# Alxaline/BraTS21

Measured on AMD Instinct MI355X. Metric: train patches/sec (4x128^3, width-48), higher is better.
Workload: dtype bf16; 1 GPU; equiunet width=48, batch=2/GPU of 4x128^3 synthetic patches, fwd + deep-supervision Dice + bwd + ranger (BASELINE.json configs[1]); global_batch=2, parallelism=dp1

## Files before the change

brats21_amd/csrc/conv_wgrad.hip:

```cpp
#include <stdlib.h>
#include "twin_begin.hpp"
#include "common.hpp"

typedef __attribute__((ext_vector_type(4))) short s16x4;

struct WgradParams {
  const void* x1; const void* x2; int c1, c2, p1, p2;
  const void* dy; int dyp;
  float* ws;
  int N, D, H, W, cin, cout;
  int tz, ty, tx, ntiles, nsplit;
  int nlane;
  int ntaps, dil;
  int seglen, nsegz;
};

constexpr int WG_TZ = 4, WG_TY = 4, WG_TX = 16, WG_VOX = 256;

template <typename T, int DIL, int COF, int CIF, int KS = 3>
struct WgGeom {
  static constexpr bool BF = std::is_same<T, bf16_t>::value;
  static constexpr int ESZ = sizeof(T);
  static constexpr int EPL = 16 / ESZ;
  static constexpr int R = KS == 3 ? DIL : 0;
  static constexpr int HY = WG_TY + 2 * R, HX = WG_TX + 2 * R;
  static constexpr int HVOX = WG_TZ * HY * HX;
  static constexpr int CI_T = 16 * CIF, CO_T = 16 * COF;
  static constexpr int XROWB = CI_T * ESZ, YROWB = CO_T * ESZ;
  static constexpr int SX = BF ? (CIF == 1 ? 32 : 96) : XROWB + 16;
  static constexpr int SY = BF ? (COF == 1 ? 32 : 96) : YROWB + 16;
  static constexpr int XPPV = XROWB / 16, YPPV = YROWB / 16;
  static constexpr int XPPR = HX * XPPV, XIPR = (XPPR + 63) / 64, XROWS = WG_TZ * HY, XRPW = (XROWS + 3) / 4;
  static constexpr int YPPR = WG_TX * YPPV, YIPR = (YPPR + 63) / 64, YROWS = WG_TZ * WG_TY, YRPW = YROWS / 4;
  static constexpr int LDS_X = HVOX * SX, LDS_Y = WG_VOX * SY;
  static constexpr int LDS = LDS_X + LDS_Y;
  static constexpr int PAIRS = (KS == 3 ? 9 : 1) * CIF;
  static constexpr int PPW = (PAIRS + 3) / 4;
  static constexpr int NB = BF ? 32 : 64;
};

DEVI bf16x8 tr_pair(const char* p0, const char* p1) {
  const s16x4 lo = __builtin_amdgcn_ds_read_tr16_b64_v4i16((__attribute__((address_space(3))) s16x4*)p0);
  const s16x4 hi = __builtin_amdgcn_ds_read_tr16_b64_v4i16((__attribute__((address_space(3))) s16x4*)p1);
  typedef __attribute__((ext_vector_type(8))) short s16x8;
  const s16x8 v = {lo[0], lo[1], lo[2], lo[3], hi[0], hi[1], hi[2], hi[3]};
  return __builtin_bit_cast(bf16x8, v);
}

template <typename T, int DIL, int COF, int CIF, int KS = 3>
__global__ __launch_bounds__(256, 2) void conv_wgrad_kernel(const WgradParams p) {
  using G = WgGeom<T, DIL, COF, CIF, KS>;
  extern __shared__ __attribute__((aligned(16))) char lds[];
  char* ldx = lds;
  char* ldy = lds + G::LDS_X;
  const int tid = threadIdx.x, lane = tid & 63;
  const int wave = __builtin_amdgcn_readfirstlane(tid >> 6);
  const int q = lane >> 4, v = lane & 15;
  const int NP = KS == 3 ? 3 : p.ntaps;
  const int lane8 = blockIdx.x % p.nlane, rr = blockIdx.x / p.nlane;
  const int tzg = rr % NP, gsub = rr / NP, g8 = gridDim.x / (NP * p.nlane);
  const int shz = (KS == 3 || p.ntaps == 1) ? 0 : (tzg / 9 - 1) * p.dil;
  const int shy = (KS == 3 || p.ntaps == 1) ? 0 : ((tzg / 3) % 3 - 1) * p.dil;
  const int shx = (KS == 3 || p.ntaps == 1) ? 0 : (tzg % 3 - 1) * p.dil;
  const int split = lane8 + p.nlane * gsub;
  const int tpx = (p.ntiles + p.nlane - 1) / p.nlane;
  const int tile_end = min(p.ntiles, (lane8 + 1) * tpx);
  const int cot = blockIdx.y, cit = blockIdx.z;
  const int co0 = cot * G::CO_T, ci0 = cit * G::CI_T;
  const T* xsrc;
  int xpitch;
  if (ci0 < p.c1) { xsrc = (const T*)p.x1 + ci0; xpitch = p.p1; }
  else { xsrc = (const T*)p.x2 + (ci0 - p.c1); xpitch = p.p2; }
  const int ci_lim = (ci0 < p.c1 ? p.c1 : p.c1 + p.c2) - ci0;
  const int co_lim = p.cout - co0;

  int xhx[G::XIPR], xlo[G::XIPR];
  int xvo[G::XRPW][G::XIPR];
#pragma unroll
  for (int j = 0; j < G::XIPR; ++j) {
    const int pc = lane + 64 * j;
    const int hx = pc / G::XPPV, part = pc % G::XPPV;
    const bool ok = pc < G::XPPR && part * G::EPL < ci_lim;
    xhx[j] = ok ? hx : -100000;
    xlo[j] = pc < G::XPPR ? wave * (G::HX * G::SX) + hx * G::SX + part * 16 : -1;
#pragma unroll
    for (int k = 0; k < G::XRPW; ++k) {
      const int row = wave + 4 * k;
      xvo[k][j] = (((row / G::HY) * p.H + row % G::HY) * p.W + hx) * xpitch * G::ESZ + part * 16;
    }
  }
  int yvx[G::YIPR], ylo[G::YIPR];
  int yvo[G::YRPW][G::YIPR];
#pragma unroll
  for (int j = 0; j < G::YIPR; ++j) {
    const int pc = lane + 64 * j;
    const int vx = pc / G::YPPV, part = pc % G::YPPV;
    const bool ok = pc < G::YPPR && part * G::EPL < co_lim;
    yvx[j] = ok ? vx : 100000;
    ylo[j] = pc < G::YPPR ? wave * (WG_TX * G::SY) + vx * G::SY + part * 16 : -1;
#pragma unroll
    for (int k = 0; k < G::YRPW; ++k) {
      const int row = wave + 4 * k;
      yvo[k][j] = (((row / WG_TY) * p.H + row % WG_TY) * p.W + vx) * p.dyp * G::ESZ + part * 16;
    }
  }
  const unsigned xsample_bytes = (unsigned)p.D * p.H * p.W * xpitch * G::ESZ;
  const unsigned ysample_bytes = (unsigned)p.D * p.H * p.W * p.dyp * G::ESZ;

  int poff[G::PPW];
#pragma unroll
  for (int jj = 0; jj < G::PPW; ++jj) {
    const int pid = wave + 4 * jj;
    const int t9 = pid / CIF, nn = pid % CIF;
    poff[jj] = pid < G::PAIRS ? (((t9 / 3) * G::R) * G::HX + (t9 % 3) * G::R) * G::SX + nn * G::NB : 0;
  }
  f32x4 acc[G::PPW][COF];
#pragma unroll
  for (int jj = 0; jj < G::PPW; ++jj)
#pragma unroll
    for (int m = 0; m < COF; ++m) acc[jj][m] = f32x4{0.f, 0.f, 0.f, 0.f};

  u32x4 rx[G::XRPW][G::XIPR], ry[G::YRPW][G::YIPR];
  auto issue_loads = [&](int tile) {
    int bt = tile;
    const int x0 = (bt % p.tx) * WG_TX; bt /= p.tx;
    const int y0 = (bt % p.ty) * WG_TY; bt /= p.ty;
    const int z0 = (bt % p.tz) * WG_TZ;
    const int n = bt / p.tz;
    const int gz0 = KS == 3 ? z0 + (tzg - 1) * DIL : z0 + shz;
    const int gy0 = KS == 3 ? y0 - DIL : y0 + shy, gx0 = KS == 3 ? x0 - DIL : x0 + shx;
    const size_t sample_vox = (size_t)n * p.D * p.H * p.W;
    const __amdgpu_buffer_rsrc_t xrs = __builtin_amdgcn_make_buffer_rsrc((void*)(xsrc + sample_vox * xpitch), (short)0,
                                                                          (int)xsample_bytes, 0x00020000);
    const __amdgpu_buffer_rsrc_t yrs = __builtin_amdgcn_make_buffer_rsrc((void*)((const T*)p.dy + sample_vox * p.dyp + co0),
                                                                          (short)0, (int)ysample_bytes, 0x00020000);
    const int xorg = ((gz0 * p.H + gy0) * p.W + gx0) * xpitch * G::ESZ;
    const int yorg = ((z0 * p.H + y0) * p.W + x0) * p.dyp * G::ESZ;
    bool xok[G::XIPR], yok[G::YIPR];
#pragma unroll
    for (int j = 0; j < G::XIPR; ++j) xok[j] = (unsigned)(gx0 + xhx[j]) < (unsigned)p.W;
#pragma unroll
    for (int j = 0; j < G::YIPR; ++j) yok[j] = x0 + yvx[j] < p.W;
#pragma unroll
    for (int k = 0; k < G::XRPW; ++k) {
      const int row = wave + 4 * k;
      const int gz = gz0 + row / G::HY, gy = gy0 + row % G::HY;
      const bool row_ok = row < G::XROWS && (unsigned)gz < (unsigned)p.D && (unsigned)gy < (unsigned)p.H;
#pragma unroll
      for (int j = 0; j < G::XIPR; ++j) {
        const int vo = (row_ok && xok[j]) ? xorg + xvo[k][j] : -1;
        rx[k][j] = __builtin_bit_cast(u32x4, __builtin_amdgcn_raw_buffer_load_b128(xrs, vo, 0, 0));
      }
    }
#pragma unroll
    for (int k = 0; k < G::YRPW; ++k) {
      const int row = wave + 4 * k;
      const bool row_ok = z0 + row / WG_TY < p.D && y0 + row % WG_TY < p.H;
#pragma unroll
      for (int j = 0; j < G::YIPR; ++j) {
        const int vo = (row_ok && yok[j]) ? yorg + yvo[k][j] : -1;
        ry[k][j] = __builtin_bit_cast(u32x4, __builtin_amdgcn_raw_buffer_load_b128(yrs, vo, 0, 0));
      }
    }
  };
  constexpr bool PREFETCH = !(G::BF && KS == 3 && DIL == 2 && COF * CIF == 9);
  const int tile_first = lane8 * tpx + gsub;
  if (PREFETCH && tile_first < tile_end) issue_loads(tile_first);
// ... 120 lines not shown
  if (ci0 < p.c1) { xsrc = (const T*)p.x1 + ci0; xpitch = p.p1; }
  else { xsrc = (const T*)p.x2 + (ci0 - p.c1); xpitch = p.p2; }

  int xcode[G::XI], ycode[G::YI];
#pragma unroll
  for (int i = 0; i < G::XI; ++i) {
    const int P = tid + 512 * i;
    const int vox = P / G::XPPV, part = P % G::XPPV;
    const int hx = vox % G::HX, hy = (vox / G::HX) % G::HY, hz = vox / (G::HX * G::HY);
    xcode[i] = (P < G::XPIECES && part * 8 < ci_lim) ? (hz | hy << 3 | hx << 6 | part << 11 | 1 << 14) : 0;
  }
#pragma unroll
  for (int i = 0; i < G::YI; ++i) {
    const int P = tid + 512 * i;
    const int vox = P / G::YPPV, part = P % G::YPPV;
    ycode[i] = (vox >> 6) | ((vox >> 4) & 3) << 3 | (vox & 15) << 6 | part << 11 | 1 << 14;
  }
  const unsigned xsample_bytes = (unsigned)p.D * p.H * p.W * xpitch * 2;
  const unsigned ysample_bytes = (unsigned)p.D * p.H * p.W * p.dyp * 2;

  int poff[G::PPW];
#pragma unroll
  for (int jj = 0; jj < G::PPW; ++jj) {
    const int pid = wave + 8 * jj;
    const int t = pid / CIF, nn = pid % CIF;
    poff[jj] = pid < G::PAIRS ? (((t / 9) * G::HY + (t / 3) % 3) * G::HX + t % 3) * G::SX + nn * 32 : 0;
  }
  f32x4 acc[G::PPW][COF];
#pragma unroll
  for (int jj = 0; jj < G::PPW; ++jj)
#pragma unroll
    for (int m = 0; m < COF; ++m) acc[jj][m] = f32x4{0.f, 0.f, 0.f, 0.f};

  u32x4 rx[G::XI], ry[G::YI];
  auto issue_loads = [&](int tile) {
    int bt = tile;
    const int x0 = (bt % p.tx) * WG_TX; bt /= p.tx;
    const int y0 = (bt % p.ty) * WG_TY; bt /= p.ty;
    const int z0 = (bt % p.tz) * WG_TZ;
    const int n = bt / p.tz;
    const size_t sample_vox = (size_t)n * p.D * p.H * p.W;
    const __amdgpu_buffer_rsrc_t xrs = __builtin_amdgcn_make_buffer_rsrc((void*)(xsrc + sample_vox * xpitch), (short)0,
                                                                          (int)xsample_bytes, 0x00020000);
    const __amdgpu_buffer_rsrc_t yrs = __builtin_amdgcn_make_buffer_rsrc((void*)((const T*)p.dy + sample_vox * p.dyp + co0),
                                                                          (short)0, (int)ysample_bytes, 0x00020000);
    unsigned zm = 0, ym = 0, xm = 0, zy = 0, yy = 0, xy = 0;
#pragma unroll
    for (int h = 0; h < G::HZ; ++h) zm |= ((unsigned)(z0 - 1 + h) < (unsigned)p.D ? 1u : 0u) << h;
#pragma unroll
    for (int h = 0; h < G::HY; ++h) ym |= ((unsigned)(y0 - 1 + h) < (unsigned)p.H ? 1u : 0u) << h;
#pragma unroll
    for (int h = 0; h < G::HX; ++h) xm |= ((unsigned)(x0 - 1 + h) < (unsigned)p.W ? 1u : 0u) << h;
    zy = zm >> 1; yy = ym >> 1; xy = xm >> 1;
    const int xorg = ((z0 - 1) * p.H + (y0 - 1)) * p.W + (x0 - 1);
    const int yorg = (z0 * p.H + y0) * p.W + x0;
    const int xpb = xpitch * 2, ypb = p.dyp * 2;
#pragma unroll
    for (int i = 0; i < G::XI; ++i) {
      int c = xcode[i];
      asm volatile("" : "+v"(c));
      const unsigned ok = (unsigned)(c >> 14) & (zm >> (c & 7)) & (ym >> ((c >> 3) & 7)) & (xm >> ((c >> 6) & 31)) & 1u;
      const int pv = ((c & 7) * p.H + ((c >> 3) & 7)) * p.W + ((c >> 6) & 31);
      const int vo = ok ? (xorg + pv) * xpb + ((c >> 11) & 7) * 16 : -1;
      rx[i] = __builtin_bit_cast(u32x4, __builtin_amdgcn_raw_buffer_load_b128(xrs, vo, 0, 0));
    }
#pragma unroll
    for (int i = 0; i < G::YI; ++i) {
      int c = ycode[i];
      asm volatile("" : "+v"(c));
      const unsigned ok = (zy >> (c & 7)) & (yy >> ((c >> 3) & 7)) & (xy >> ((c >> 6) & 31)) & 1u;
      const int pv = ((c & 7) * p.H + ((c >> 3) & 7)) * p.W + ((c >> 6) & 31);
      const int vo = ok ? (yorg + pv) * ypb + ((c >> 11) & 7) * 16 : -1;
      ry[i] = __builtin_bit_cast(u32x4, __builtin_amdgcn_raw_buffer_load_b128(yrs, vo, 0, 0));
    }
  };

  const int tile_first = lane8 * tpx + gsub;
  if (tile_first < tile_end) issue_loads(tile_first);
  for (int tile = tile_first; tile < tile_end; tile += g8) {
    __syncthreads();
#pragma unroll
    for (int i = 0; i < G::XI; ++i)
      if (tid + 512 * i < G::XPIECES) *(u32x4*)(ldx + (tid + 512 * i) * 16) = rx[i];
#pragma unroll
    for (int i = 0; i < G::YI; ++i) {
      const int P = tid + 512 * i;
      *(u32x4*)(ldy + (P / G::YPPV) * G::SY + (P % G::YPPV) * 16) = ry[i];
    }
    __syncthreads();
    if (tile + g8 < tile_end) issue_loads(tile + g8);
    __builtin_amdgcn_sched_barrier(0);
    const int qq = v >> 2, pp = v & 3;
    const int ybase = (4 * q + qq) * G::SY + pp * 8;
    const int xbase = (4 * q + qq) * G::SX + pp * 8;
    constexpr int PD = 2;
    bf16x8 a[2][COF], b[PD + 1];
    auto read_a = [&](auto s_) {
      constexpr int s = s_;
      const int yoff = ybase + (32 * s) * G::SY;
#pragma unroll
      for (int m = 0; m < COF; ++m) a[s & 1][m] = tr_pair(ldy + yoff + m * 32, ldy + yoff + 16 * G::SY + m * 32);
    };
    auto read_b = [&](auto u_) {
      constexpr int u = u_;
      constexpr int s = u / G::PPW, jj = u % G::PPW;
      const int xoff = xbase + (((s >> 1) * G::HY + 2 * (s & 1)) * G::HX) * G::SX + poff[jj];
      b[u % (PD + 1)] = tr_pair(ldx + xoff, ldx + xoff + G::HX * G::SX);
    };
    constexpr int NU = 8 * G::PPW;
    read_a(std::integral_constant<int, 0>{});
    static_for<0, PD>([&](auto u_) { read_b(u_); });
    static_for<0, NU>([&](auto u_) {
      constexpr int u = u_;
      constexpr int s = u / G::PPW, jj = u % G::PPW;
      if constexpr (u + PD < NU) read_b(std::integral_constant<int, u + PD>{});
      if constexpr (jj == 0 && s + 1 < 8) read_a(std::integral_constant<int, s + 1>{});
      __builtin_amdgcn_sched_barrier(0);
#pragma unroll
      for (int m = 0; m < COF; ++m)
        acc[jj][m] = MFMA16_16x16x32(a[s & 1][m], b[u % (PD + 1)], acc[jj][m]);
      __builtin_amdgcn_sched_barrier(0);
    });
  }

#pragma unroll
  for (int jj = 0; jj < G::PPW; ++jj) {
    const int pid = wave + 8 * jj;
    if (pid < G::PAIRS) {
      const int t = pid / CIF, nn = pid % CIF;
      float* base = p.ws + ((size_t)split * 27 + t) * p.cout * p.cin;
      const int ci = ci0 + nn * 16 + v;
      if (nn * 16 + v < ci_lim) {
#pragma unroll
        for (int m = 0; m < COF; ++m)
#pragma unroll
          for (int r = 0; r < 4; ++r) base[(size_t)(co0 + m * 16 + 4 * q + r) * p.cin + ci] = acc[jj][m][r];
      }
    }
  }
}

template <int COF, int CIF> struct Wg3b {
  static constexpr int HZ = WG_TZ + 2, HY = WG_TY + 2, HX = WG_TX + 2, HVOX = HZ * HY * HX;
  static constexpr int CO = 16 * COF, CI = 16 * CIF;
  static constexpr int SX = 2 * CI, SY = 2 * CO, XPPV = CI / 8, YPPV = CO / 8;
  static constexpr int XPIECES = HVOX * XPPV, YPIECES = WG_VOX * YPPV;
  static constexpr int XI = (XPIECES + 511) / 512, YI = YPIECES / 512;
  static constexpr int XB = XI * 512 * 16;
  static constexpr int LDS = 2 * XB + WG_VOX * SY;
  static constexpr int PAIRS = 27 * CIF, PPW = (PAIRS + 7) / 8;
  static_assert(YPIECES % 512 == 0, "");
};

template <int COF, int CIF>
__global__ __launch_bounds__(512, 1) void conv_wgrad_alltaps2_kernel(const WgradParams p) {
  typedef bf16_t T;
  using G = Wg3b<COF, CIF>;
  extern __shared__ __attribute__((aligned(16))) char lds[];
  char* ldy = lds + 2 * G::XB;
  const int tid = threadIdx.x, lane = tid & 63;
  const int wave = __builtin_amdgcn_readfirstlane(tid >> 6);
  const int q = lane >> 4, v = lane & 15;
  const int lane8 = blockIdx.x % p.nlane, gsub = blockIdx.x / p.nlane, g8 = gridDim.x / p.nlane;
  const int split = blockIdx.x;
  const int tpx = (p.ntiles + p.nlane - 1) / p.nlane;
  const int tile_end = min(p.ntiles, (lane8 + 1) * tpx);
  const int co0 = blockIdx.y * G::CO, ci0 = blockIdx.z * G::CI;
  const T* xsrc;
  int xpitch;
  if (ci0 < p.c1) { xsrc = (const T*)p.x1 + ci0; xpitch = p.p1; }
  else { xsrc = (const T*)p.x2 + (ci0 - p.c1); xpitch = p.p2; }
  const int xpb = xpitch * 2, ypb = p.dyp * 2;

  int xoffs[G::XI], xcode[G::XI];
#pragma unroll
  for (int i = 0; i < G::XI; ++i) {
    const int P = tid + 512 * i;
    const int vox = P / G::XPPV, part = P % G::XPPV;
    const int hx = vox % G::HX, hy = (vox / G::HX) % G::HY, hz = vox / (G::HX * G::HY);
    const bool ok = P < G::XPIECES && (CIF > 1 || part * 8 < p.c1);
    xoffs[i] = ok ? ((hz * p.H + hy) * p.W + hx) * xpb + part * 16 : (int)0x80000000;
    xcode[i] = ok ? (hz | hy << 3 | hx << 6 | 1 << 14) : 0;
  }
  const unsigned xsample_bytes = (unsigned)p.D * p.H * p.W * xpitch * 2;
  const unsigned ysample_bytes = (unsigned)p.D * p.H * p.W * p.dyp * 2;

  int poff[G::PPW];
#pragma unroll
  for (int jj = 0; jj < G::PPW; ++jj) {
    const int pid = wave + 8 * jj;
    const int t = pid / CIF, nn = pid % CIF;
    poff[jj] = pid < G::PAIRS ? (((t / 9) * G::HY + (t / 3) % 3) * G::HX + t % 3) * G::SX + nn * 32 : 0;
  }
  f32x4 acc[G::PPW][COF];
#pragma unroll
  for (int jj = 0; jj < G::PPW; ++jj)
#pragma unroll
    for (int m = 0; m < COF; ++m) acc[jj][m] = f32x4{0.f, 0.f, 0.f, 0.f};

  u32x4 ry[G::YI];
  struct TileLoads {
    rsrc4_t xrs;
    __amdgpu_buffer_rsrc_t yrs;
    int xorg, yorg;
    unsigned zm, ym, xm, inter;
    char* xdst;
  };
  auto setup_loads = [&](int tile, int buf) {
    TileLoads L;
    int bt = tile;
    const int x0 = (bt % p.tx) * WG_TX; bt /= p.tx;
    const int y0 = (bt % p.ty) * WG_TY; bt /= p.ty;
    const int z0 = (bt % p.tz) * WG_TZ;
    const int n = bt / p.tz;
    const size_t sample_vox = (size_t)n * p.D * p.H * p.W;
    L.xrs = make_rsrc4(xsrc + sample_vox * xpitch, xsample_bytes);
    L.yrs = __builtin_amdgcn_make_buffer_rsrc((void*)((const T*)p.dy + sample_vox * p.dyp + co0), (short)0, (int)ysample_bytes, 0x00020000);
    L.xorg = (((z0 - 1) * p.H + (y0 - 1)) * p.W + (x0 - 1)) * xpb;
    L.yorg = ((z0 * p.H + y0) * p.W + x0) * ypb;
    L.xdst = lds + buf * G::XB + wave * 1024;
    auto inside = [](int o, int size, int hn) {
      const int lo = o >= 1 ? 0 : 1 - o, hi = size - o + 1 < hn ? size - o + 1 : hn;
      return hi > lo ? ((1u << hi) - 1u) & ~((1u << lo) - 1u) : 0u;
    };
    L.zm = inside(z0, p.D, G::HZ); L.ym = inside(y0, p.H, G::HY); L.xm = inside(x0, p.W, G::HX);
    L.inter = (L.zm == (1u << G::HZ) - 1 && L.ym == (1u << G::HY) - 1 && L.xm == (1u << G::HX) - 1) ? 1u : 0u;
    return L;
  };
  auto issue_x = [&](const TileLoads& L, auto i_) {
    constexpr int i = i_;
    const int c = xcode[i];
    const unsigned ok = (unsigned)(c >> 14) & (L.inter | ((L.zm >> (c & 7)) & (L.ym >> ((c >> 3) & 7)) & (L.xm >> ((c >> 6) & 31)))) & 1u;
    lds_dma16_async(L.xrs, L.xdst + i * 8192, (L.xorg + xoffs[i]) | ((int)ok - 1));
  };
  auto issue_y = [&](const TileLoads& L, auto i_) {
    constexpr int i = i_;
    const int P = tid + 512 * i;
    const int vox = P / G::YPPV, part = P % G::YPPV;
    const int z = vox >> 6, y = (vox >> 4) & 3, x = vox & 15;
    const int yo = ((z * p.H + y) * p.W + x) * ypb + part * 16;
    const unsigned ok = (L.inter | ((L.zm >> (z + 1)) & (L.ym >> (y + 1)) & (L.xm >> (x + 1)))) & 1u;
    ry[i] = __builtin_bit_cast(u32x4, __builtin_amdgcn_raw_buffer_load_b128(L.yrs, (L.yorg + yo) | ((int)ok - 1), 0, 0));
  };

  const int tile_first = lane8 * tpx + gsub;
  const int qq = v >> 2, pp = v & 3;
  const int ybase = (4 * q + qq) * G::SY + pp * 8;
  const int xbase = (4 * q + qq) * G::SX + pp * 8;
  int cur = 0;
#ifdef BRATS_WGRAD_STAMPS
  long long tacc[5] = {0, 0, 0, 0, 0}, tlast = __builtin_amdgcn_s_memtime();
#define WG_STAMP(i) do { const long long t_ = __builtin_amdgcn_s_memtime(); tacc[i] += t_ - tlast; tlast = t_; } while (0)
#else
#define WG_STAMP(i) do { } while (0)
#endif
  if (tile_first < tile_end) {
    const TileLoads L = setup_loads(tile_first, 0);
    static_for<0, G::XI>([&](auto i_) { issue_x(L, i_); });
    static_for<0, G::YI>([&](auto i_) { issue_y(L, i_); });
  }
  for (int tile = tile_first; tile < tile_end; tile += g8, cur ^= 1) {
    WG_STAMP(4);
    asm volatile("s_waitcnt vmcnt(0)" ::: "memory");
    WG_STAMP(0);
    __syncthreads();
    WG_STAMP(1);
#pragma unroll
    for (int i = 0; i < G::YI; ++i) *(u32x4*)(ldy + (tid + 512 * i) * 16) = ry[i];
    __syncthreads();
    WG_STAMP(2);
    const bool more = tile + g8 < tile_end;
    TileLoads L = setup_loads(more ? tile + g8 : tile, cur ^ 1);
    if (!more) L.zm = L.inter = 0;
    __builtin_amdgcn_sched_barrier(0);
    WG_STAMP(3);
    const char* ldx = lds + cur * G::XB;
    constexpr int PD = 3;
    bf16x8 a[2][COF], b[PD + 1];
    auto read_a = [&](auto s_) {
      constexpr int s = s_;
      const int yoff = ybase + (32 * s) * G::SY;
#pragma unroll
      for (int m = 0; m < COF; ++m) a[s & 1][m] = tr_pair(ldy + yoff + m * 32, ldy + yoff + 16 * G::SY + m * 32);
    };
    auto read_b = [&](auto u_) {
      constexpr int u = u_;
      constexpr int s = u / G::PPW, jj = u % G::PPW;
      const int xoff = xbase + (((s >> 1) * G::HY + 2 * (s & 1)) * G::HX) * G::SX + poff[jj];
      b[u % (PD + 1)] = tr_pair(ldx + xoff, ldx + xoff + G::HX * G::SX);
    };
    constexpr int NU = 8 * G::PPW;
    static_for<0, G::XI>([&](auto i_) { issue_x(L, i_); });
    static_for<0, G::YI>([&](auto i_) { issue_y(L, i_); });
    __builtin_amdgcn_sched_barrier(0);
    read_a(std::integral_constant<int, 0>{});
    static_for<0, PD>([&](auto u_) { read_b(u_); });
    static_for<0, NU>([&](auto u_) {
      constexpr int u = u_;
      constexpr int s = u / G::PPW, jj = u % G::PPW;
      if constexpr (u + PD < NU) read_b(std::integral_constant<int, u + PD>{});
      if constexpr (jj == 0 && s + 1 < 8) read_a(std::integral_constant<int, s + 1>{});
      __builtin_amdgcn_sched_barrier(0);
#pragma unroll
      for (int m = 0; m < COF; ++m)
        acc[jj][m] = MFMA16_16x16x32(a[s & 1][m], b[u % (PD + 1)], acc[jj][m]);
      __builtin_amdgcn_sched_barrier(0);
    });
  }

#ifdef BRATS_WGRAD_STAMPS
  WG_STAMP(4);
  if (lane == 0 && blockIdx.y == 0 && blockIdx.z == 0) {
    long long* st = (long long*)(p.ws + (size_t)gridDim.x * 27 * p.cout * p.cin) + ((size_t)blockIdx.x * 8 + wave) * 5;
    for (int i = 0; i < 5; ++i) st[i] = tacc[i];
  }
#endif
#pragma unroll
  for (int jj = 0; jj < G::PPW; ++jj) {
    const int pid = wave + 8 * jj;
    if (pid < G::PAIRS) {
      const int t = pid / CIF, nn = pid % CIF;
      float* base = p.ws + ((size_t)split * 27 + t) * p.cout * p.cin;
      const int ci = ci0 + nn * 16 + v;
      if (CIF > 1 || ci < p.cin) {
#pragma unroll
        for (int m = 0; m < COF; ++m)
#pragma unroll
          for (int r = 0; r < 4; ++r) base[(size_t)(co0 + m * 16 + 4 * q + r) * p.cin + ci] = acc[jj][m][r];
      }
    }
  }
}

template <int DIL> struct Wg3n {
  static constexpr int HZ = WG_TZ + 2 * DIL, HY = WG_TY + 2 * DIL, HX = WG_TX + 2 * DIL, HVOX = HZ * HY * HX;
  static constexpr int COF = 3, CO = 48, CI = 16;
  static constexpr int SX = 2 * CI, SY = 2 * CO, XPPV = CI / 8, YPPV = CO / 8;
  static constexpr int MMA_WAVES = 8, LOAD_WAVES = 4, THREADS = 64 * (MMA_WAVES + LOAD_WAVES), LT = 64 * LOAD_WAVES;
  static constexpr int XPIECES = HVOX * XPPV, YPIECES = WG_VOX * YPPV;
  static constexpr int XI = (XPIECES + LT - 1) / LT, YI = YPIECES / LT;
  static constexpr int XB = XI * LT * 16, YB = YI * LT * 16;
  static constexpr int BUF = XB + YB;
  static constexpr int PAIRS = 27, PPW = 4;
  static constexpr int OUT_ROW = CI * 27, OUT_B = CO * OUT_ROW * 4;
  static constexpr int LDS = 2 * BUF > OUT_B ? 2 * BUF : OUT_B;
  static_assert(HZ <= 8 && HY <= 8 && HX <= 32, "packed halo coordinates: 3 + 3 + 5 bits");
  static_assert(YPIECES % LT == 0, "");
};

struct WgNoslabWalk {
  int nlane, nsplit, g8, tpx, ntiles;
  int split, tile, end;
  DEVI void enter() {
    for (;; ++split) {
      const int lane8 = split % nlane;
      tile = lane8 * tpx + split / nlane;
      end = min(ntiles, (lane8 + 1) * tpx);
      if (tile < end || split + 1 >= nsplit) return;
    }
  }
  DEVI WgNoslabWalk(const WgradParams& p) : nlane(p.nlane), nsplit(p.nsplit), g8(p.nsplit / p.nlane),
                                            tpx((p.ntiles + p.nlane - 1) / p.nlane), ntiles(p.ntiles), split(0) { enter(); }
  DEVI bool done() const { return tile >= end; }
  DEVI bool next() {
    tile += g8;
    if (tile < end) return false;
    if (split + 1 < nsplit) { ++split; enter(); }
    return true;
  }
};

template <int DIL>
__global__ __launch_bounds__(768, 1) void conv_wgrad_noslab_kernel(const WgradParams p) {
  typedef bf16_t T;
  using G = Wg3n<DIL>;
  extern __shared__ __attribute__((aligned(16))) char lds[];
  const int tid = threadIdx.x, lane = tid & 63;
  const int wave = __builtin_amdgcn_readfirstlane(tid >> 6);
  const int co0 = blockIdx.y * G::CO, ci0 = blockIdx.z * G::CI;
  f32x4 tot[G::PPW][G::COF];
#pragma unroll
  for (int jj = 0; jj < G::PPW; ++jj)
#pragma unroll
    for (int m = 0; m < G::COF; ++m) tot[jj][m] = f32x4{0.f, 0.f, 0.f, 0.f};

  WgNoslabWalk walk(p);
  if (wave >= G::MMA_WAVES) {
    const int lt = tid - 64 * G::MMA_WAVES, lw = wave - G::MMA_WAVES;
    const T* xsrc;
    int xpitch;
    if (ci0 < p.c1) { xsrc = (const T*)p.x1 + ci0; xpitch = p.p1; }
    else { xsrc = (const T*)p.x2 + (ci0 - p.c1); xpitch = p.p2; }
    const int xpb = xpitch * 2, ypb = p.dyp * 2;
    int xoffs[G::XI], xcode[G::XI], yoffs[G::YI], ycode[G::YI];
#pragma unroll
    for (int i = 0; i < G::XI; ++i) {
      const int P = lt + G::LT * i;
      const int vox = P / G::XPPV, part = P % G::XPPV;
      const int hx = vox % G::HX, hy = (vox / G::HX) % G::HY, hz = vox / (G::HX * G::HY);
      const bool ok = P < G::XPIECES;
      xoffs[i] = ok ? ((hz * p.H + hy) * p.W + hx) * xpb + part * 16 : (int)0x80000000;
      xcode[i] = ok ? (hz | hy << 3 | hx << 6 | 1 << 14) : 0;
    }
#pragma unroll
    for (int i = 0; i < G::YI; ++i) {
      const int P = lt + G::LT * i;
      const int vox = P / G::YPPV, part = P % G::YPPV;
      const int z = vox >> 6, y = (vox >> 4) & 3, x = vox & 15;
      yoffs[i] = ((z * p.H + y) * p.W + x) * ypb + part * 16;
      ycode[i] = (z + DIL) | (y + DIL) << 3 | (x + DIL) << 6;
    }
    const unsigned xsample_bytes = (unsigned)p.D * p.H * p.W * xpitch * 2;
    const unsigned ysample_bytes = (unsigned)p.D * p.H * p.W * p.dyp * 2;
    auto issue_tile = [&](int tile, int buf) {
      int bt = tile;
      const int x0 = (bt % p.tx) * WG_TX; bt /= p.tx;
      const int y0 = (bt % p.ty) * WG_TY; bt /= p.ty;
      const int z0 = (bt % p.tz) * WG_TZ;
      const int n = bt / p.tz;
      const size_t sample_vox = (size_t)n * p.D * p.H * p.W;
      const rsrc4_t xrs = make_rsrc4(xsrc + sample_vox * xpitch, xsample_bytes);
      const rsrc4_t yrs = make_rsrc4((const T*)p.dy + sample_vox * p.dyp + co0, ysample_bytes);
      const int xorg = (((z0 - DIL) * p.H + (y0 - DIL)) * p.W + (x0 - DIL)) * xpb;
      const int yorg = ((z0 * p.H + y0) * p.W + x0) * ypb;
      char* const dst = lds + buf * G::BUF + lw * 1024;
      auto inside = [](int o, int size, int hn) {
        const int lo = o >= DIL ? 0 : DIL - o, hi = size - o + DIL < hn ? size - o + DIL : hn;
        return hi > lo ? ((1u << hi) - 1u) & ~((1u << lo) - 1u) : 0u;
      };
      const unsigned zm = inside(z0, p.D, G::HZ), ym = inside(y0, p.H, G::HY), xm = inside(x0, p.W, G::HX);
      static_for<0, G::XI>([&](auto i_) {
        constexpr int i = i_;
        const int c = xcode[i];
        const unsigned ok = (unsigned)(c >> 14) & (zm >> (c & 7)) & (ym >> ((c >> 3) & 7)) & (xm >> ((c >> 6) & 31)) & 1u;
        lds_dma16_async(xrs, dst + i * (G::LT * 16), (xorg + xoffs[i]) | ((int)ok - 1));
      });
      static_for<0, G::YI>([&](auto i_) {
        constexpr int i = i_;
        const int c = ycode[i];
        const unsigned ok = (zm >> (c & 7)) & (ym >> ((c >> 3) & 7)) & (xm >> ((c >> 6) & 31)) & 1u;
        lds_dma16_async(yrs, dst + G::XB + i * (G::LT * 16), (yorg + yoffs[i]) | ((int)ok - 1));
      });
    };
    issue_tile(walk.tile, 0);
    asm volatile("s_waitcnt vmcnt(0)" ::: "memory");
    __syncthreads();
    for (int buf = 1; !walk.done(); buf ^= 1) {
      walk.next();
      if (!walk.done()) issue_tile(walk.tile, buf);
      asm volatile("s_waitcnt vmcnt(0)" ::: "memory");
      __syncthreads();
    }
  } else {
    const int q = lane >> 4, v = lane & 15;
    const bool four = wave + 24 < G::PAIRS;
    int poff[G::PPW];
#pragma unroll
    for (int jj = 0; jj < G::PPW; ++jj) {
      const int t = wave + 8 * jj;
      poff[jj] = t < G::PAIRS ? ((((t / 9) * G::HY + (t / 3) % 3) * G::HX + t % 3) * DIL) * G::SX : 0;
    }
    f32x4 acc[G::PPW][G::COF];
#pragma unroll
    for (int jj = 0; jj < G::PPW; ++jj)
#pragma unroll
      for (int m = 0; m < G::COF; ++m) acc[jj][m] = f32x4{0.f, 0.f, 0.f, 0.f};
    const int qq = v >> 2, pp = v & 3;
    const int ybase = (4 * q + qq) * G::SY + pp * 8;
    const int xbase = (4 * q + qq) * G::SX + pp * 8;
    __syncthreads();
    for (int buf = 0; !walk.done(); buf ^= 1) {
      const char* ldx = lds + buf * G::BUF;
      const char* ldy = ldx + G::XB;
      constexpr int PD = 3;
      bf16x8 a[2][G::COF], b[PD + 1];
      auto read_a = [&](auto s_) {
        constexpr int s = s_;
        const int yoff = ybase + (32 * s) * G::SY;
#pragma unroll
        for (int m = 0; m < G::COF; ++m) a[s & 1][m] = tr_pair(ldy + yoff + m * 32, ldy + yoff + 16 * G::SY + m * 32);
      };
      auto read_b = [&](auto u_) {
        constexpr int u = u_;
        constexpr int s = u / G::PPW, jj = u % G::PPW;
// ... 302 lines not shown
    f32x4 s[4];
#pragma unroll
    for (int t = 0; t < 4; ++t) s[t] = f32x4{0.f, 0.f, 0.f, 0.f};
    for (int k0 = 0; k0 < nsplit; k0 += 8) {
      f32x4 v[4][8];
#pragma unroll
      for (int t = 0; t < 4; ++t) {
        const int tap = g + 8 * t;
        const float* src = ws + ((size_t)(tap < taps ? tap : 0) * cout * cin + p4 * 4);
#pragma unroll
        for (int u = 0; u < 8; ++u)
          v[t][u] = (tap < taps && k0 + u < nsplit) ? *(const f32x4*)(src + (size_t)(k0 + u) * per) : f32x4{0.f, 0.f, 0.f, 0.f};
      }
#pragma unroll
      for (int t = 0; t < 4; ++t)
#pragma unroll
        for (int u = 0; u < 8; ++u)
          if (k0 + u < nsplit) s[t] += v[t][u];
    }
#pragma unroll
    for (int t = 0; t < 4; ++t)
      if (g + 8 * t < taps) *(f32x4*)(red_tile + (g + 8 * t) * 128 + e * 4) = s[t];
  }
  __syncthreads();
  const size_t pair0 = (size_t)blockIdx.x * 128, npairs = (size_t)cout * cin;
  float* dst = dw + pair0 * taps;
  const float isc = amax ? x3_inv_scale(x3_scale_from_amax(*amax)) : 1.f;
  for (int i = threadIdx.x; i < 128 * taps; i += blockDim.x) {
    const int pr = i / taps, tap = i % taps;
    if (pair0 + pr < npairs) dst[i] = red_tile[tap * 128 + pr] * isc;
  }
}

static void wgrad_reduce_launch(const float* ws, float* dw, int nsplit, int cout, int cin, int taps, hipStream_t st,
                                const float* amax = nullptr) {
  const size_t per = (size_t)taps * cout * cin;
  const size_t tblocks = ((size_t)cout * cin / 4 + 31) / 32;
  if (taps > 1 && taps <= 32 && tblocks >= 256)
    hipLaunchKernelGGL(wgrad_reduce_taps_kernel, dim3((unsigned)tblocks), dim3(256), (size_t)taps * 128 * sizeof(float), st, ws, dw,
                       nsplit, cout, cin, taps, amax);
  else
    hipLaunchKernelGGL(wgrad_reduce_kernel, dim3((unsigned)((per / 4 + 31) / 32)), dim3(256), 0, st, ws, dw, nsplit, cout, cin, taps, amax);
}

template <typename T>
__global__ void dbias_kernel(const T* __restrict__ dy, int pitch, float* __restrict__ db, size_t voxels, int C) {
  __shared__ float red[256];
  const int c = blockIdx.x;
  float s = 0.f;
  for (size_t v = threadIdx.x; v < voxels; v += blockDim.x) s += to_f<T>(dy[v * pitch + c]);
  red[threadIdx.x] = s;
  __syncthreads();
  for (int m = 128; m > 0; m >>= 1) {
    if ((int)threadIdx.x < m) red[threadIdx.x] += red[threadIdx.x + m];
    __syncthreads();
  }
  if (threadIdx.x == 0) db[c] = red[0];
}
static void wgrad_dbias_launch(int dtype, const void* dy, int dypitch, float* dbias, size_t vox, int cout, hipStream_t st) {
  with_storage(dtype, [&](auto t) {
    using T = typename decltype(t)::type;
    hipLaunchKernelGGL(dbias_kernel<T>, dim3(cout), dim3(256), 0, st, (const T*)dy, dypitch, dbias, vox, cout);
  });
}

struct WgradArgs {
  const void* x1; int c1, p1;
  const void* x2; int c2, p2;
  const void* dy; int dyp;
  int N, D, H, W, cout;
  int cin() const { return c1 + c2; }
  size_t vox() const { return (size_t)N * D * H * W; }
};
static WgradArgs wgrad_shape(int N, int D, int H, int W, int c1, int c2, int cout) {
  return WgradArgs{nullptr, c1, 0, nullptr, c2 > 0 ? c2 : 0, 0, nullptr, 0, N, D, H, W, cout};
}
static int wgrad_sample_overflow(const WgradArgs& a, int esize) {
  const int mp = a.p1 > a.p2 ? (a.p1 > a.dyp ? a.p1 : a.dyp) : (a.p2 > a.dyp ? a.p2 : a.dyp);
  return (double)a.D * a.H * a.W * mp * esize >= 2147483648.0 ? mp : 0;
}

struct WgradTileGrid { int tz, ty, tx, ntiles; };
static WgradTileGrid wgrad_tile_grid(const WgradArgs& a, int TZ = WG_TZ, int TY = WG_TY, int TX = WG_TX) {
  WgradTileGrid t{ceil_div(a.D, TZ), ceil_div(a.H, TY), ceil_div(a.W, TX), 0};
  t.ntiles = a.N * t.tz * t.ty * t.tx;
  return t;
}
static WgradParams wgrad_params(const WgradArgs& a, float* ws, const WgradTileGrid& t, int nlane, int nsplit, int ntaps, int dil) {
  WgradParams p{};
  p.x1 = a.x1; p.x2 = a.x2; p.c1 = a.c1; p.c2 = a.c2; p.p1 = a.p1; p.p2 = a.p2;
  p.dy = a.dy; p.dyp = a.dyp; p.ws = ws;
  p.N = a.N; p.D = a.D; p.H = a.H; p.W = a.W; p.cin = a.cin(); p.cout = a.cout;
  p.tz = t.tz; p.ty = t.ty; p.tx = t.tx; p.ntiles = t.ntiles;
  p.nlane = nlane; p.nsplit = nsplit; p.ntaps = ntaps; p.dil = dil;
  return p;
}

static int wgrad_nlane(int ntiles) {
  int nl = 8;
  while (nl > 1 && ntiles / nl < 16) nl >>= 1;
  return nl;
}
static int wgrad_split_g8(int ntiles, int nlane, int groups, int cot, int cit) {
  int g8 = ceil_div(512, groups * nlane * cot * cit);
  const int cap = ceil_div(ntiles, nlane);
  if (g8 > cap) g8 = cap;
  return g8 < 1 ? 1 : g8;
}
static bool wgrad_blocks_g8(int ntiles, int blocks, int* nlane, int* g8) {
  *nlane = wgrad_nlane(ntiles);
  *g8 = ceil_div(device_cus(), *nlane * blocks);
  if (*g8 < 1) *g8 = 1;
  return ntiles >= 4 * *nlane * *g8;
}
static void wgrad_tiles(int dtype, int c1, int c2, int cout, int* cof, int* cif) {
  const int co16 = ceil_div(cout, 16);
  *cof = co16 % 3 == 0 ? 3 : (co16 % 2 == 0 ? 2 : 1);
  if (dtype == BRATS_F32) { *cif = 1; return; }
  const int a = ceil_div(c1, 16), b = c2 > 0 ? ceil_div(c2, 16) : 0;
  auto ok = [&](int f) { return a % f == 0 && (b == 0 || b % f == 0); };
  *cif = ok(3) ? 3 : (ok(2) ? 2 : 1);
}

int g_wgrad_alltaps_mode = -1;
extern "C" int BRATS_API(brats_conv3d_set_wgrad_alltaps)(int mode) {
  const int old = g_wgrad_alltaps_mode;
  g_wgrad_alltaps_mode = mode < 0 ? -1 : (mode ? 1 : 0);
  return old;
}
static int wgrad_alltaps_mode() {
  static int env_mode = -1;
  if (env_mode < 0) {
    const char* e = getenv("BRATS_WGRAD_ALLTAPS");
    env_mode = e ? atoi(e) : 1;
  }
  return g_wgrad_alltaps_mode >= 0 ? g_wgrad_alltaps_mode : env_mode;
}

int g_wgrad_noslab_mode = -1;
extern "C" int BRATS_API(brats_conv3d_set_wgrad_noslab)(int mode) {
  const int old = g_wgrad_noslab_mode;
  g_wgrad_noslab_mode = mode < 0 ? -1 : (mode ? 1 : 0);
  return old;
}
static int wgrad_noslab_mode() {
  static int env_mode = -2;
  if (env_mode < -1) {
    const char* e = getenv("BRATS_WGRAD_NOSLAB");
    const int m = e ? atoi(e) : -1;
    env_mode = m < 0 ? -1 : (m ? 1 : 0);
  }
  return g_wgrad_noslab_mode >= 0 ? g_wgrad_noslab_mode : env_mode;
}
static bool wgrad_noslab_built(int dtype, bool shifted, int ksize, int dil, const WgradArgs& a) {
  return !shifted && ksize == 3 && dtype == BRATS_BF16 && (dil == 1 || dil == 2) && a.cout > 0 && a.cout % 48 == 0 && a.c1 > 0 &&
         a.c1 % 16 == 0 && a.c2 % 16 == 0 && a.N > 0 && a.D > 0 && a.H > 0 && a.W > 0;
}
static bool wgrad_noslab_rule(const WgradArgs& a, int dil, int ntiles) {
  const int wgs = (a.cout / 48) * (a.cin() / 16);
  return 4 * wgs >= 3 * device_cus() && ntiles <= (dil == 2 ? 64 : 32);
}

enum WgradForm {
  WG_TAP_PLANE, WG_SHIFTED_TAP,
  WG_ALLTAPS2_33, WG_ALLTAPS2_42, WG_ALLTAPS2_31,
  WG_NOSLAB,
  WG_ALLTAPS_1, WG_ALLTAPS_1_4,
  WG_F8_33, WG_F8_42
};
struct WgradPlan {
  WgradForm form;
  int cof, cif;
  int cot, cit;
  int nlane, g8, nsplit;
  int ntaps, groups;
  bool clear;
  WgradTileGrid tiles;
  size_t per;
  size_t slab_bytes() const { return nsplit * per * sizeof(float); }
};

static WgradPlan wgrad_plan(int dtype, bool shifted, int ksize, int dil, const WgradArgs& a, bool noslab = false) {
  WgradPlan pl;
  const int c1 = a.c1, c2 = a.c2, cin = a.cin(), cout = a.cout;
  pl.tiles = wgrad_tile_grid(a);
  pl.ntaps = ksize == 3 ? 27 : 1;
  pl.per = (size_t)pl.ntaps * cout * cin;
  if (noslab && wgrad_alltaps_mode() && wgrad_noslab_mode() != 0 && wgrad_noslab_built(dtype, shifted, ksize, dil, a) &&
      (wgrad_noslab_mode() == 1 || wgrad_noslab_rule(a, dil, pl.tiles.ntiles))) {
    pl.form = WG_NOSLAB;
    pl.cof = 3; pl.cif = 1;
    pl.cot = cout / 48; pl.cit = cin / 16;
    const WgradPlan slab = wgrad_plan(dtype, shifted, ksize, dil, a);
    pl.nlane = slab.nlane; pl.g8 = slab.g8; pl.nsplit = 0; pl.groups = 1;
    pl.clear = false;
    return pl;
  }
  const bool narrow = c2 == 0 && c1 <= 16;
  auto blocks_of = [&](int co, int ci) { return cout % co == 0 && (narrow || (c1 % ci == 0 && c2 % ci == 0)); };
  if (!shifted && wgrad_alltaps_mode() && dtype == BRATS_BF16 && dil == 1 && (blocks_of(48, 48) || blocks_of(64, 32))) {
    const bool wide = !blocks_of(48, 48);
    pl.cof = wide ? 4 : 3; pl.cif = narrow ? 1 : (wide ? 2 : 3);
    pl.cot = cout / (16 * pl.cof); pl.cit = narrow ? 1 : cin / (16 * pl.cif);
    if (wgrad_blocks_g8(pl.tiles.ntiles, pl.cot * pl.cit, &pl.nlane, &pl.g8)) {
      pl.form = wide ? (narrow ? WG_ALLTAPS_1_4 : WG_ALLTAPS2_42) : narrow ? (c1 % 8 == 0 ? WG_ALLTAPS2_31 : WG_ALLTAPS_1) : WG_ALLTAPS2_33;
      pl.groups = 1;
      pl.clear = false;
      pl.nsplit = pl.nlane * pl.g8;
      return pl;
    }
  }
  pl.form = shifted ? WG_SHIFTED_TAP : WG_TAP_PLANE;
  wgrad_tiles(dtype, c1, c2, cout, &pl.cof, &pl.cif);
  pl.cot = ceil_div(cout, 16 * pl.cof);
  pl.cit = ceil_div(c1, 16 * pl.cif) + (c2 > 0 ? ceil_div(c2, 16 * pl.cif) : 0);
  pl.groups = shifted ? pl.ntaps : 3;
  pl.nlane = wgrad_nlane(pl.tiles.ntiles);
  pl.g8 = wgrad_split_g8(pl.tiles.ntiles, pl.nlane, pl.groups, pl.cot, pl.cit);
  pl.nsplit = pl.nlane * pl.g8;
  pl.clear = cin % 16 || cout % 16;
  return pl;
}
static size_t wgrad_slab_room(int dtype, bool shifted, int ksize, const WgradArgs& a) {
  const size_t d1 = wgrad_plan(dtype, shifted, ksize, 1, a).slab_bytes();
  const size_t d2 = shifted ? 0 : wgrad_plan(dtype, shifted, ksize, 2, a).slab_bytes();
  return d1 > d2 ? d1 : d2;
}

template <typename T, int DIL, int COF, int CIF, int KS = 3>
static int wgrad_launch(const WgradParams& p, dim3 grid, hipStream_t st) {
  using G = WgGeom<T, DIL, COF, CIF, KS>;
  auto kern = conv_wgrad_kernel<T, DIL, COF, CIF, KS>;
  static std::atomic<uint64_t> attr_done{0};
  BRATS_ENSURE_LDS_ATTR(kern, G::LDS, attr_done);
  hipLaunchKernelGGL(kern, grid, dim3(256), G::LDS, st, p);
  BRATS_CHECK_LAUNCH();
  return 0;
}

template <typename T, int DIL, int KS = 3>
static int wgrad_dispatch(const WgradParams& p, int cof, int cif, dim3 grid, hipStream_t st) {
#define WG_CASE(A, B) if (cof == A && cif == B) return wgrad_launch<T, DIL, A, B, KS>(p, grid, st);
  WG_CASE(3, 1) WG_CASE(2, 1) WG_CASE(1, 1)
  if constexpr (std::is_same<T, bf16_t>::value) {
    WG_CASE(3, 3) WG_CASE(3, 2) WG_CASE(2, 3) WG_CASE(2, 2) WG_CASE(1, 3) WG_CASE(1, 2)
  }
#undef WG_CASE
  BRATS_FAIL(BRATS_E_UNSUPPORTED, "wgrad: unsupported tile %dx%d", cof, cif);
}

template <auto KERN, int LDS, int THREADS = 512>
static int wgrad_alltaps_launch(const WgradParams& p, dim3 grid, hipStream_t st) {
  static std::atomic<uint64_t> attr_done{0};
  BRATS_ENSURE_LDS_ATTR(KERN, LDS, attr_done);
  hipLaunchKernelGGL(KERN, grid, dim3(THREADS), LDS, st, p);
  BRATS_CHECK_LAUNCH();
  return 0;
}

static int wgrad_run(const WgradPlan& pl, int dtype, int dil, const WgradArgs& a, float* ws, size_t room, hipStream_t st) {
  const char* who = pl.form == WG_SHIFTED_TAP ? "wgrad_shift" : "wgrad";
  if (a.c2 > 0 && a.c1 % (16 * pl.cif)) BRATS_FAIL(BRATS_E_UNSUPPORTED, "wgrad: c1=%d must be a multiple of the ci tile %d", a.c1, 16 * pl.cif);
  if (pl.slab_bytes() > room) BRATS_FAIL(BRATS_E_ARG, "%s: the plan's %zu bytes of slabs exceed the workspace size %zu", who, pl.slab_bytes(), room);
  const WgradParams p = wgrad_params(a, ws, pl.tiles, pl.nlane, pl.nsplit, pl.ntaps, dil);
  if (pl.clear) {
    hipError_t e = hipMemsetAsync(ws, 0, pl.slab_bytes(), st);
    if (e != hipSuccess) BRATS_FAIL(BRATS_E_HIP, "%s: memset: %s", who, hipGetErrorString(e));
  }
  const dim3 grid(pl.groups * pl.nsplit, pl.cot, pl.cit);
  const bool bf = dtype == BRATS_BF16;
  switch (pl.form) {
    case WG_NOSLAB: {
      const dim3 g1(1, pl.cot, pl.cit);
      WgradParams pn = p;
      pn.nsplit = pl.nlane * pl.g8;
      return dil == 1 ? wgrad_alltaps_launch<conv_wgrad_noslab_kernel<1>, Wg3n<1>::LDS, Wg3n<1>::THREADS>(pn, g1, st)
                      : wgrad_alltaps_launch<conv_wgrad_noslab_kernel<2>, Wg3n<2>::LDS, Wg3n<2>::THREADS>(pn, g1, st);
    }
    case WG_TAP_PLANE:
      if (bf) return dil == 1 ? wgrad_dispatch<bf16_t, 1>(p, pl.cof, pl.cif, grid, st) : wgrad_dispatch<bf16_t, 2>(p, pl.cof, pl.cif, grid, st);
      return dil == 1 ? wgrad_dispatch<float, 1>(p, pl.cof, pl.cif, grid, st) : wgrad_dispatch<float, 2>(p, pl.cof, pl.cif, grid, st);
    case WG_SHIFTED_TAP:
      return bf ? wgrad_dispatch<bf16_t, 1, 1>(p, pl.cof, pl.cif, grid, st) : wgrad_dispatch<float, 1, 1>(p, pl.cof, pl.cif, grid, st);
    case WG_ALLTAPS2_33: return wgrad_alltaps_launch<conv_wgrad_alltaps2_kernel<3, 3>, Wg3b<3, 3>::LDS>(p, grid, st);
    case WG_ALLTAPS2_42: return wgrad_alltaps_launch<conv_wgrad_alltaps2_kernel<4, 2>, Wg3b<4, 2>::LDS>(p, grid, st);
    case WG_ALLTAPS2_31: return wgrad_alltaps_launch<conv_wgrad_alltaps2_kernel<3, 1>, Wg3b<3, 1>::LDS>(p, grid, st);
    case WG_ALLTAPS_1: return wgrad_alltaps_launch<conv_wgrad_alltaps_kernel<1>, Wg3<1>::LDS>(p, grid, st);
    case WG_ALLTAPS_1_4: return wgrad_alltaps_launch<conv_wgrad_alltaps_kernel<1, 4>, Wg3<1, 4>::LDS>(p, grid, st);
    default: BRATS_FAIL(BRATS_E_UNSUPPORTED, "wgrad: form %d is not a 16-bit / f32 kernel", (int)pl.form);
  }
}

template <int V>
__global__ void __launch_bounds__(256) x3_split_kernel(const float* __restrict__ src, int pitch, bf16_t* __restrict__ hi,
                                                       bf16_t* __restrict__ lo, size_t voxels, int C, const float* __restrict__ amax) {
  const float sc = amax ? x3_scale_from_amax(*amax) : 1.f;
  const int cv = C / 8;
  const size_t total = voxels * cv;
  const size_t stride = (size_t)gridDim.x * 256;
  auto load = [&](size_t i, u32x4& a, u32x4& b) {
    const float* p = src + (i / cv) * pitch + (i % cv) * 8;
    a = __builtin_nontemporal_load((const u32x4*)p);
    b = __builtin_nontemporal_load((const u32x4*)(p + 4));
  };
  auto emit = [&](size_t i, const u32x4& a, const u32x4& b) {
    const uint32_t w[8] = {a[0], a[1], a[2], a[3], b[0], b[1], b[2], b[3]};
    uint32_t h[4], l[4];
#pragma unroll
    for (int e = 0; e < 4; ++e) {
      const float x0 = __uint_as_float(w[2 * e]) * sc, x1 = __uint_as_float(w[2 * e + 1]) * sc;
      x3_split2(x0, x1, h[e], l[e]);
    }
    const size_t o = (i / cv) * C + (i % cv) * 8;
    __builtin_nontemporal_store(u32x4{h[0], h[1], h[2], h[3]}, (u32x4*)(hi + o));
    __builtin_nontemporal_store(u32x4{l[0], l[1], l[2], l[3]}, (u32x4*)(lo + o));
  };
  size_t i = (size_t)blockIdx.x * 256 + threadIdx.x;
  for (; i + stride < total; i += 2 * stride) {
    u32x4 a0, b0, a1, b1;
    load(i, a0, b0);
    load(i + stride, a1, b1);
    emit(i, a0, b0);
    emit(i + stride, a1, b1);
  }
  if (i < total) {
    u32x4 a0, b0;
    load(i, a0, b0);
    emit(i, a0, b0);
  }
}
static size_t x3_align(size_t b) { return (b + 255) / 256 * 256; }
static void x3_split_launch(const float* src, int pitch, bf16_t* hi, bf16_t* lo, size_t vox, int c, const float* amax, hipStream_t st) {
  const size_t total = vox * (c / 8);
  size_t nb = (total + 511) / 512;
  const unsigned blocks = (unsigned)(nb < 1 ? 1 : (nb > 262144 ? 262144 : nb));
  hipLaunchKernelGGL(x3_split_kernel<0>, dim3(blocks), dim3(256), 0, st, src, pitch, hi, lo, vox, c, amax);
}

struct X3Carve {
  size_t off[7];
  X3Carve(size_t room16, const WgradArgs& a) {
    const int c[3] = {a.c1, a.c2, a.cout};
    size_t b = x3_align(3 * room16);
    for (int i = 0; i < 6; ++i) {
      off[i] = b;
      b += c[i / 2] > 0 ? x3_align(a.vox() * c[i / 2] * 2) : 0;
    }
    off[6] = b;
  }
  size_t bytes() const { return off[6]; }
  bf16_t* at(float* ws, int i) const { return (bf16_t*)((char*)ws + off[i]); }
};

static int wgrad_x3(const WgradPlan& pl, int dil, const WgradArgs& a, const float* amax_dy, float* ws, float* dw, size_t room16,
                          hipStream_t st) {
  const X3Carve cv(room16, a);
  bf16_t *h1 = cv.at(ws, 0), *l1 = cv.at(ws, 1), *h2 = cv.at(ws, 2), *l2 = cv.at(ws, 3), *hy = cv.at(ws, 4), *ly = cv.at(ws, 5);
  x3_split_launch((const float*)a.x1, a.p1, h1, l1, a.vox(), a.c1, nullptr, st);
  if (a.c2 > 0) x3_split_launch((const float*)a.x2, a.p2, h2, l2, a.vox(), a.c2, nullptr, st);
  x3_split_launch((const float*)a.dy, a.dyp, hy, ly, a.vox(), a.cout, amax_dy, st);
  BRATS_CHECK_LAUNCH();
  WgradArgs t = a;
  t.p1 = a.c1; t.p2 = a.c2; t.dyp = a.cout;
  const bool xlo[3] = {true, false, false}, ylo[3] = {false, true, false};
  for (int k = 0; k < 3; ++k) {
    t.x1 = xlo[k] ? l1 : h1;
    t.x2 = a.c2 > 0 ? (xlo[k] ? l2 : h2) : nullptr;
    t.dy = ylo[k] ? ly : hy;
    const int rc = wgrad_run(pl, BRATS_BF16, dil, t, ws + (size_t)k * pl.nsplit * pl.per, room16, st);
    if (rc) return rc;
  }
  wgrad_reduce_launch((const float*)ws, dw, 3 * pl.nsplit, a.cout, a.cin(), pl.ntaps, st, amax_dy);
  return 0;
}

#include "conv_wgrad_x3.hpp"
extern "C" int BRATS_API(brats_conv3d_set_x3_wgrad_fused)(int mode) {
  const int old = g_x3_wgrad_fused_mode;
  g_x3_wgrad_fused_mode = mode < 0 ? -1 : (mode > 2 ? 2 : mode);
  return old;
}

static size_t wgrad_ws_bytes(int dtype, bool shifted, int ksize, const WgradArgs& a) {
  if (dtype != BRATS_X3_BF16) return wgrad_slab_room(dtype, shifted, ksize, a);
  const size_t three = X3Carve(wgrad_slab_room(BRATS_BF16, shifted, ksize, a), a).bytes();
  const size_t fused = shifted ? 0 : wgrad_x3_fused_ws_bytes(a);
  return three > fused ? three : fused;
}
extern "C" size_t BRATS_API(brats_conv3d_wgrad_ws_bytes)(int dtype, int ksize, int N, int D, int H, int W, int c1, int c2, int cout) {
  return ksize == 3 ? wgrad_ws_bytes(dtype, false, 3, wgrad_shape(N, D, H, W, c1, c2, cout)) : 0;
}
extern "C" size_t BRATS_API(brats_conv3d_wgrad_shift_ws_bytes)(int dtype, int ksize, int N, int D, int H, int W, int cin, int cout) {
  return ksize == 1 || ksize == 3 ? wgrad_ws_bytes(dtype, true, ksize, wgrad_shape(N, D, H, W, cin, 0, cout)) : 0;
}

extern "C" int BRATS_API(brats_conv3d_wgrad_noslab_taken)(int dtype, int dil, int N, int D, int H, int W, int c1, int c2, int cout) {
  if (dtype != BRATS_BF16 || c1 <= 0 || cout <= 0 || N <= 0 || D <= 0 || H <= 0 || W <= 0) return 0;
  return wgrad_plan(dtype, false, 3, dil, wgrad_shape(N, D, H, W, c1, c2, cout), true).form == WG_NOSLAB ? 1 : 0;
}

static int wgrad_impl(bool shifted, WgradArgs a, const float* amax_dy, float* ws, float* dw, float* dbias, int dtype, int ksize, int dil,
                      brats_stream_t s) {
  const char* who = shifted ? "wgrad_shift" : "wgrad";
  if (!a.x1 || !a.dy || !ws || !dw || a.c1 <= 0 || a.cout <= 0 || (shifted && (a.N <= 0 || a.D <= 0 || a.H <= 0 || a.W <= 0)))
    BRATS_FAIL(BRATS_E_ARG, "%s: null pointer / bad size", who);
  if (shifted ? (ksize != 1 && ksize != 3) || dil < 1 : ksize != 3 || (dil != 1 && dil != 2))
    BRATS_FAIL(BRATS_E_UNSUPPORTED, "%s: ksize=%d dil=%d unsupported", who, ksize, dil);
  if (shifted && dtype != BRATS_BF16 && dtype != BRATS_F32 && dtype != BRATS_X3_BF16) BRATS_FAIL(BRATS_E_UNSUPPORTED, "wgrad_shift: dtype %d", dtype);
  if (a.c2 < 0) a.c2 = 0;
  if (a.c2 > 0 && !a.x2) BRATS_FAIL(BRATS_E_ARG, "wgrad: c2 > 0 but x2 NULL");
  const bool x3 = dtype == BRATS_X3_BF16;
  const int epl = vec_width(dtype);
  if (a.p1 % epl || (a.c2 && a.p2 % epl) || a.dyp % epl || a.c1 % epl || a.c2 % epl || a.cout % epl)
    BRATS_FAIL(BRATS_E_ARG, "%s: channel counts / pitches must be multiples of %d", who, epl);
  if (x3 && (a.c1 % 8 || a.c2 % 8 || a.cout % 8)) BRATS_FAIL(BRATS_E_ARG, "%s (split precision): channel counts must be multiples of 8", who);
  if (const int mp = wgrad_sample_overflow(a, dtype == BRATS_BF16 ? 2 : 4))
    BRATS_FAIL(BRATS_E_UNSUPPORTED, "%s: one sample of %dx%dx%d x pitch %d exceeds the 2 GiB buffer-offset range", who, a.D, a.H, a.W, mp);
  hipStream_t st = (hipStream_t)s;
  int rc = x3 && !shifted ? wgrad_x3_fused(a, amax_dy, ws, dw, dil, st) : 1;
  if (rc == 1) {
    const int dt = x3 ? BRATS_BF16 : dtype;
    const WgradPlan pl = wgrad_plan(dt, shifted, ksize, dil, a, !x3);
    const size_t room = wgrad_slab_room(dt, shifted, ksize, a);
    if (x3) rc = wgrad_x3(pl, dil, a, amax_dy, ws, dw, room, st);
    else if (pl.form == WG_NOSLAB) rc = wgrad_run(pl, dtype, dil, a, dw, room, st);
    else if (!(rc = wgrad_run(pl, dtype, dil, a, ws, room, st))) wgrad_reduce_launch((const float*)ws, dw, pl.nsplit, a.cout, a.cin(), pl.ntaps, st);
  }
  if (rc) return rc;
  if (dbias) wgrad_dbias_launch(dtype, a.dy, a.dyp, dbias, a.vox(), a.cout, st);
  BRATS_CHECK_LAUNCH();
  return 0;
}

extern "C" int BRATS_API(brats_conv3d_wgrad)(const void* x1, int c1, int pitch1, const void* x2, int c2, int pitch2, const void* dy,
                                  int dypitch, float* ws, float* dw, float* dbias, int dtype, int ksize, int dil, int N,
                                  int D, int H, int W, int cout, brats_stream_t s) {
  return wgrad_impl(false, WgradArgs{x1, c1, pitch1, x2, c2, pitch2, dy, dypitch, N, D, H, W, cout}, nullptr, ws, dw, dbias, dtype, ksize, dil, s);
}
extern "C" int BRATS_API(brats_conv3d_x3_wgrad)(const void* x1, int c1, int pitch1, const void* x2, int c2, int pitch2, const void* dy,
                                     int dypitch, const float* amax_dy, float* ws, float* dw, float* dbias, int dtype, int dil,
                                     int N, int D, int H, int W, int cout, brats_stream_t s) {
  if (dtype != BRATS_X3_BF16) BRATS_FAIL(BRATS_E_ARG, "conv3d_x3_wgrad: dtype must be BRATS_X3_F16 or BRATS_X3_BF16");
  return wgrad_impl(false, WgradArgs{x1, c1, pitch1, x2, c2, pitch2, dy, dypitch, N, D, H, W, cout}, amax_dy, ws, dw, dbias, dtype, 3, dil, s);
}
extern "C" int BRATS_API(brats_conv3d_wgrad_shift)(const void* x, int cin, int xpitch, const void* dy, int dypitch, float* ws, float* dw,
                                        float* dbias, int dtype, int ksize, int dil, int N, int D, int H, int W, int cout,
                                        brats_stream_t s) {
  return wgrad_impl(true, WgradArgs{x, cin, xpitch, nullptr, 0, 0, dy, dypitch, N, D, H, W, cout}, nullptr, ws, dw, dbias, dtype, ksize, dil, s);
}
extern "C" int BRATS_API(brats_conv3d_x3_wgrad_shift)(const void* x, int cin, int xpitch, const void* dy, int dypitch, const float* amax_dy,
                                           float* ws, float* dw, float* dbias, int dtype, int ksize, int dil, int N, int D, int H,
                                           int W, int cout, brats_stream_t s) {
  if (dtype != BRATS_X3_BF16) BRATS_FAIL(BRATS_E_ARG, "conv3d_x3_wgrad_shift: dtype must be BRATS_X3_F16 or BRATS_X3_BF16");
  return wgrad_impl(true, WgradArgs{x, cin, xpitch, nullptr, 0, 0, dy, dypitch, N, D, H, W, cout}, amax_dy, ws, dw, dbias, dtype, ksize, dil, s);
}

static bool wgrad_f8_plan(const WgradArgs& a, WgradPlan* pl) {
  const int c1 = a.c1, c2 = a.c2, cout = a.cout;
  if (c1 <= 0 || cout <= 0) return false;
  if (cout % 48 == 0 && c1 % 48 == 0 && c2 % 48 == 0) { pl->form = WG_F8_33; pl->cof = 3; pl->cif = 3; }
  else if (cout % 64 == 0 && c1 % 32 == 0 && c2 % 32 == 0) { pl->form = WG_F8_42; pl->cof = 4; pl->cif = 2; }
  else return false;
  pl->tiles = wgrad_tile_grid(a);
  pl->cot = cout / (16 * pl->cof); pl->cit = a.cin() / (16 * pl->cif);
  if (!wgrad_blocks_g8(pl->tiles.ntiles, pl->cot * pl->cit, &pl->nlane, &pl->g8)) return false;
  pl->nsplit = pl->nlane * pl->g8;
  pl->ntaps = 27; pl->groups = 1; pl->clear = false;
  pl->per = (size_t)27 * cout * a.cin();
  return true;
}

extern "C" size_t BRATS_API(brats_conv3d_wgrad_f8_ws_bytes)(int N, int D, int H, int W, int c1, int c2, int cout) {
  WgradPlan pl;
  return wgrad_f8_plan(wgrad_shape(N, D, H, W, c1, c2, cout), &pl) ? pl.slab_bytes() : 0;
}

template <int COF, int CIF>
static int wgrad_f8_launch(const WgradF8Params& pp, dim3 grid, hipStream_t st) {
  using G = Wg3f<COF, CIF>;
  auto kern = conv_wgrad_alltaps_f8_kernel<COF, CIF>;
  static std::atomic<uint64_t> attr_done{0};
  BRATS_ENSURE_LDS_ATTR(kern, G::LDS, attr_done);
  hipLaunchKernelGGL(kern, grid, dim3(512), G::LDS, st, pp);
  BRATS_CHECK_LAUNCH();
  return 0;
}

extern "C" int BRATS_API(brats_conv3d_wgrad_f8)(const void* x1, int c1, int pitch1, const float* amax1, const void* x2, int c2, int pitch2,
                                     const float* amax2, const void* dy, int dypitch, const float* amax_dy, float* ws, float* dw,
                                     int N, int D, int H, int W, int cout, brats_stream_t s) {
  if (!x1 || !dy || !ws || !dw || !amax1 || !amax_dy || c1 <= 0 || cout <= 0) BRATS_FAIL(BRATS_E_ARG, "wgrad_f8: null pointer / bad size");
  if (c2 < 0) c2 = 0;
  if (c2 > 0 && (!x2 || !amax2)) BRATS_FAIL(BRATS_E_ARG, "wgrad_f8: c2 > 0 needs x2 and its |max|");
  const WgradArgs a{x1, c1, pitch1, x2, c2, pitch2, dy, dypitch, N, D, H, W, cout};
  WgradPlan pl;
  if (!wgrad_f8_plan(a, &pl))
    BRATS_FAIL(BRATS_E_UNSUPPORTED, "wgrad_f8: built for 48 x 48 / 64 x 32 channel blocks of layers with enough tiles "
               "(brats_conv3d_wgrad_f8_ws_bytes() == 0 otherwise): use brats_conv3d_wgrad");
  if (pitch1 % 8 || (c2 && pitch2 % 8) || dypitch % 8) BRATS_FAIL(BRATS_E_ARG, "wgrad_f8: pitches must be multiples of 8");
  if (wgrad_sample_overflow(a, 2)) BRATS_FAIL(BRATS_E_UNSUPPORTED, "wgrad_f8: sample exceeds the 2 GiB buffer-offset range");
  const WgradF8Params pp{wgrad_params(a, ws, pl.tiles, pl.nlane, pl.nsplit, 27, 1), amax1, c2 ? amax2 : nullptr, amax_dy};
  hipStream_t st = (hipStream_t)s;
  const dim3 grid(pl.nsplit, pl.cot, pl.cit);
  const int rc = pl.form == WG_F8_33 ? wgrad_f8_launch<3, 3>(pp, grid, st) : wgrad_f8_launch<4, 2>(pp, grid, st);
  if (rc) return rc;
  wgrad_reduce_launch((const float*)ws, dw, pl.nsplit, cout, a.cin(), 27, st);
  BRATS_CHECK_LAUNCH();
  return 0;
}
#include "twin_end.hpp"
```

brats21_amd/csrc/gen_twin_dispatch.py:

```python
#!/usr/bin/env python3
import re
import sys

BOTH = {"brats_conv3d_set_vs8", "brats_conv3d_set_kp", "brats_conv3d_set_wgrad_alltaps", "brats_conv3d_set_wgrad_noslab",
        "brats_conv3d_set_x3_wgrad_fused", "brats_upsample_bwd_set_fused"}
DATA = {"brats_conv3d_f8_fwd", "brats_conv3d_wgrad_f8", "brats_conv3d_pack_weights_multi"}

txt = re.sub(r"/\*.*?\*/", " ", open(sys.argv[1]).read(), flags=re.S)
protos = {}
for m in re.finditer(r"(const char\s*\*|size_t|int)\s+(brats_[a-z0-9_]+)\s*\(([^)]*)\)\s*;", txt):
    protos[m.group(2)] = (" ".join(m.group(1).split()), " ".join(m.group(3).split()))
names = []
for path in sys.argv[2:]:
    for m in re.finditer(r'extern "C" [a-z_ \*]+?BRATS_API\((brats_[a-z0-9_]+)\)\(', open(path).read()):
        names.append(m.group(1))
print("// GENERATED by gen_twin_dispatch.py from include/brats_hip.h -- do not edit")
print('#include "../../include/brats_hip.h"')
print('extern "C" {')
for n in names:
    if n not in protos:
        raise SystemExit(f"{n} is defined in a twinned translation unit but not declared in brats_hip.h")
    ret, args = protos[n]
    arglist = [] if args in ("", "void") else [a.strip() for a in args.split(",")]
    argnames = [re.search(r"([A-Za-z_][A-Za-z0-9_]*)$", a).group(1) for a in arglist]
    call = ", ".join(argnames)
    sig = args if arglist else "void"
    print(f"{ret} {n}_bf16({sig});")
    print(f"{ret} {n}_f16({sig});")
    if n in DATA:
        if n + "_f16" not in protos:
            raise SystemExit(f"{n}_f16 must be declared in brats_hip.h (16-bit data, no dtype argument)")
        print(f"{ret} {n}({sig}) {{ return {n}_bf16({call}); }}")
    elif n in BOTH:
        print(f"{ret} {n}({sig}) {{ {n}_f16({call}); return {n}_bf16({call}); }}")
    elif "dtype" in argnames:
        call16 = ", ".join("BRATS_BF16" if a == "dtype" else a for a in argnames)
        callx3 = ", ".join("BRATS_X3_BF16" if a == "dtype" else a for a in argnames)
        print(f"{ret} {n}({sig}) {{ return dtype == BRATS_F16 ? {n}_f16({call16}) : dtype == BRATS_X3_F16 ? {n}_f16({callx3}) : {n}_bf16({call}); }}")
    else:
        print(f"{ret} {n}({sig}) {{ return {n}_bf16({call}); }}")
print("}")
```

brats21_amd/csrc/norm.hip:

```cpp
#include "twin_begin.hpp"
#include "common.hpp"

#include "act.hpp"
#include "se.hpp"

constexpr int GN_MAX_SPLITS = 64;
__global__ void gn_chan_reduce_kernel(const float* __restrict__ stats, int tps, int C, double* __restrict__ part) {
  const int n = blockIdx.y, c0 = blockIdx.x * 16;
  const int cl = threadIdx.x & 15, tl = threadIdx.x >> 4;
  const int c = c0 + cl;
  const int per = (tps + gridDim.z - 1) / gridDim.z;
  const int t0 = blockIdx.z * per, t1 = min(tps, t0 + per);
  double s1 = 0.0, s2 = 0.0;
  if (c < C) {
    for (int t = t0 + tl; t < t1; t += 16) {
      const f32x2 v = *(const f32x2*)(stats + (((size_t)n * tps + t) * C + c) * 2);
      s1 += v[0];
      s2 += v[1];
    }
  }
  __shared__ double r1[256], r2[256];
  r1[threadIdx.x] = s1;
  r2[threadIdx.x] = s2;
  __syncthreads();
  for (int m = 128; m >= 16; m >>= 1) {
    if ((int)threadIdx.x < m) { r1[threadIdx.x] += r1[threadIdx.x + m]; r2[threadIdx.x] += r2[threadIdx.x + m]; }
    __syncthreads();
  }
  if (threadIdx.x < 16 && c < C) {
    double* dst = part + (((size_t)blockIdx.z * gridDim.y + n) * C + c) * 2;
    dst[0] = r1[threadIdx.x];
    dst[1] = r2[threadIdx.x];
  }
}

static int gn_splits(int tps) {
  int splits = tps / 64;
  return splits < 1 ? 1 : (splits > GN_MAX_SPLITS ? GN_MAX_SPLITS : splits);
}

static int chan_reduce_launch(const float* stats, int tps, int N, int C, double* chan_ws, hipStream_t st) {
  hipLaunchKernelGGL(gn_chan_reduce_kernel, dim3((C + 15) / 16, N, gn_splits(tps)), dim3(256), 0, st, stats, tps, C,
                     chan_ws + (size_t)N * C * 2);
  return 0;
}

__global__ void gn_finalize_kernel(double* __restrict__ chan, int splits, int N, int C, int groups, double count_per_channel,
                                   float eps, int unbiased, const float* __restrict__ gamma, const float* __restrict__ beta,
                                   float* __restrict__ mean_rstd, float* __restrict__ scale_shift) {
  const int n = blockIdx.x / groups, g = blockIdx.x % groups;
  const int cpg = C / groups;
  __shared__ double r1[256], r2[256];
  double s1 = 0.0, s2 = 0.0;
  {
    const int ZL = 256 / cpg;
    const int cl = threadIdx.x % cpg, zl = threadIdx.x / cpg;
    const double* part = chan + (size_t)N * C * 2;
    double p1 = 0.0, p2 = 0.0;
    if (zl < ZL) {
      const int c = g * cpg + cl;
      for (int z = zl; z < splits; z += ZL) {
        p1 += part[(((size_t)z * N + n) * C + c) * 2];
        p2 += part[(((size_t)z * N + n) * C + c) * 2 + 1];
      }
    }
    r1[threadIdx.x] = p1;
    r2[threadIdx.x] = p2;
    __syncthreads();
    if ((int)threadIdx.x < cpg) {
      for (int z = 0; z < ZL; ++z) { s1 += r1[z * cpg + threadIdx.x]; s2 += r2[z * cpg + threadIdx.x]; }
      const int c = g * cpg + threadIdx.x;
      chan[((size_t)n * C + c) * 2] = s1;
      chan[((size_t)n * C + c) * 2 + 1] = s2;
    }
    __syncthreads();
  }
  r1[threadIdx.x] = s1;
  r2[threadIdx.x] = s2;
  __syncthreads();
  for (int m = blockDim.x / 2; m > 0; m >>= 1) {
    if ((int)threadIdx.x < m) { r1[threadIdx.x] += r1[threadIdx.x + m]; r2[threadIdx.x] += r2[threadIdx.x + m]; }
    __syncthreads();
  }
  const double M = count_per_channel * cpg;
  const double mean = r1[0] / M;
  double var = r2[0] / M - mean * mean;
  if (unbiased) var = var * M / (M - 1.0);
  if (var < 0.0) var = 0.0;
  const float rstd = (float)(1.0 / sqrt(var + (double)eps));
  if (threadIdx.x == 0) {
    mean_rstd[(n * groups + g) * 2] = (float)mean;
    mean_rstd[(n * groups + g) * 2 + 1] = rstd;
  }
  if (scale_shift && (int)threadIdx.x < cpg) {
    const int c = g * cpg + threadIdx.x;
    const float sc = rstd * gamma[c];
    scale_shift[((size_t)n * C + c) * 2] = sc;
    scale_shift[((size_t)n * C + c) * 2 + 1] = beta[c] - (float)mean * sc;
  }
}

__global__ void __launch_bounds__(1024) gn_finalize_direct_kernel(const float* __restrict__ stats, int tps, double* __restrict__ chan,
                                                                  int N, int C, int groups, double count_per_channel, float eps,
                                                                  int unbiased, const float* __restrict__ gamma,
                                                                  const float* __restrict__ beta, float* __restrict__ mean_rstd,
                                                                  float* __restrict__ scale_shift) {
  const int n = blockIdx.x / groups, g = blockIdx.x % groups;
  const int cpg = C / groups;
  __shared__ double r1[1024], r2[1024];
  const int TL = 1024 / cpg;
  const int cl = threadIdx.x % cpg, tl = threadIdx.x / cpg;
  double p1 = 0.0, p2 = 0.0;
  if (tl < TL) {
    const float* src = stats + (((size_t)n * tps) * C + g * cpg + cl) * 2;
    int t = tl;
    for (; t + 7 * TL < tps; t += 8 * TL) {
      f32x2 v[8];
#pragma unroll
      for (int u = 0; u < 8; ++u) v[u] = *(const f32x2*)(src + (size_t)(t + u * TL) * C * 2);
#pragma unroll
      for (int u = 0; u < 8; ++u) { p1 += v[u][0]; p2 += v[u][1]; }
    }
    for (; t < tps; t += TL) {
      const f32x2 v = *(const f32x2*)(src + (size_t)t * C * 2);
      p1 += v[0];
      p2 += v[1];
    }
  }
  r1[threadIdx.x] = p1;
  r2[threadIdx.x] = p2;
  __syncthreads();
  double s1 = 0.0, s2 = 0.0;
  if ((int)threadIdx.x < cpg) {
    for (int z = 0; z < TL; ++z) { s1 += r1[z * cpg + threadIdx.x]; s2 += r2[z * cpg + threadIdx.x]; }
    const int c = g * cpg + threadIdx.x;
    chan[((size_t)n * C + c) * 2] = s1;
    chan[((size_t)n * C + c) * 2 + 1] = s2;
  }
  __syncthreads();
  r1[threadIdx.x] = s1;
  r2[threadIdx.x] = s2;
  __syncthreads();
  for (int m = 128; m > 0; m >>= 1) {
    if ((int)threadIdx.x < m) { r1[threadIdx.x] += r1[threadIdx.x + m]; r2[threadIdx.x] += r2[threadIdx.x + m]; }
    __syncthreads();
  }
  const double M = count_per_channel * cpg;
  const double mean = r1[0] / M;
  double var = r2[0] / M - mean * mean;
  if (unbiased) var = var * M / (M - 1.0);
  if (var < 0.0) var = 0.0;
  const float rstd = (float)(1.0 / sqrt(var + (double)eps));
  if (threadIdx.x == 0) {
    mean_rstd[(n * groups + g) * 2] = (float)mean;
    mean_rstd[(n * groups + g) * 2 + 1] = rstd;
  }
// ... 593 lines not shown
#pragma unroll
      for (int k = 0; k < HK; ++k)
#pragma unroll
        for (int j = 0; j < VW; ++j) wr[k][j] = hf.w[k * C + c0 + j];
      const float* dl = hf.dl + (size_t)n * HK * voxels;
      const float nslope = act == BRATS_ACT_RELU ? 0.f : slope;
      auto hbody = [&](const float* g, const float* yy) {
#pragma unroll
        for (int j = 0; j < VW; ++j) {
          float d = 0.f;
#pragma unroll
          for (int k = 0; k < HK; ++k) d += g[k] * wr[k][j];
          const float pre = yy[j] * sc[j] + sh[j];
          const bool pos = pre > 0.f;
          const float u = d * (pos ? 1.f : nslope);
          a1[j] += u;
          a2[j] += u * yy[j];
          const float z = pos ? pre : pre * nslope;
#pragma unroll
          for (int k = 0; k < HK; ++k) aw[k][j] += g[k] * z;
        }
#pragma unroll
        for (int k = 0; k < HK; ++k) ab[k] += g[k];
      };
      auto step = [&](size_t v0, auto cnt) {
        constexpr int NV = decltype(cnt)::value;
        typename Raw16<T>::type yr[NV];
        float gq[NV][HKA];
#pragma unroll
        for (int i = 0; i < NV; ++i) yr[i] = Raw16<T>::template load<NT>(yb + (v0 + i * stride) * ypitch);
#pragma unroll
        for (int i = 0; i < NV; ++i)
#pragma unroll
          for (int k = 0; k < HK; ++k) gq[i][k] = dl[(size_t)k * voxels + v0 + i * stride];
#pragma unroll
        for (int i = 0; i < NV; ++i) {
          float yy[VW];
          Raw16<T>::unpack(yr[i], yy);
          hbody(gq[i], yy);
        }
      };
      for (; vox + 3 * stride < (size_t)voxels; vox += 4 * stride) step(vox, std::integral_constant<int, 4>{});
      for (; vox < (size_t)voxels; vox += stride) step(vox, std::integral_constant<int, 1>{});
#pragma unroll
      for (int j = 0; j < VW; ++j) a2[j] = a2[j] * rs[j] + mo[j] * a1[j];
    } else {
    auto body = [&](const float* g, const float* yy) {
#pragma unroll
      for (int j = 0; j < VW; ++j) {
        const float u = g[j] * act_grad<HEAVY>(yy[j] * sc[j] + sh[j], act, slope);
        a1[j] += u;
        a2[j] += u * (yy[j] * rs[j] + mo[j]);
      }
    };
    for (; vox + 3 * stride < (size_t)voxels; vox += 4 * stride) {
      float g0[VW], y0[VW], g1[VW], y1[VW], g2[VW], y2[VW], g3[VW], y3[VW];
      vload<T, VW, NT>(dzb + vox * dzpitch, g0);
      vload<T, VW, NT>(yb + vox * ypitch, y0);
      vload<T, VW, NT>(dzb + (vox + stride) * dzpitch, g1);
      vload<T, VW, NT>(yb + (vox + stride) * ypitch, y1);
      vload<T, VW, NT>(dzb + (vox + 2 * stride) * dzpitch, g2);
      vload<T, VW, NT>(yb + (vox + 2 * stride) * ypitch, y2);
      vload<T, VW, NT>(dzb + (vox + 3 * stride) * dzpitch, g3);
      vload<T, VW, NT>(yb + (vox + 3 * stride) * ypitch, y3);
      body(g0, y0);
      body(g1, y1);
      body(g2, y2);
      body(g3, y3);
    }
    for (; vox < (size_t)voxels; vox += stride) {
      float g0[VW], y0[VW];
      vload<T, VW, NT>(dzb + vox * dzpitch, g0);
      vload<T, VW, NT>(yb + vox * ypitch, y0);
      body(g0, y0);
    }
    }
  }
  float* scr = sm;
  if (myvl < vl_n) {
#pragma unroll
    for (int j = 0; j < VW; ++j) {
      scr[(myvl * C + c0 + j) * 2] = a1[j];
      scr[(myvl * C + c0 + j) * 2 + 1] = a2[j];
    }
  }
  __syncthreads();
  float* part = red + (size_t)gridDim.y * C * 2 + ((size_t)blockIdx.x * gridDim.y + n) * C * 2;
  for (int i = threadIdx.x; i < 2 * C; i += blockDim.x) {
    float t = 0.f;
    for (int l = 0; l < vl_n; ++l) t += scr[l * C * 2 + i];
    part[i] = t;
  }
  if constexpr (HK > 0) {
    const bool live = myvl < vl_n;
    float* hb = sm + vl_n * C * 2;
    if (live && mycv == 0) {
#pragma unroll
      for (int k = 0; k < HK; ++k) hb[myvl * HK + k] = ab[k];
    }
    float* hp = hf.hpart + ((size_t)n * gridDim.x + blockIdx.x) * (HK * C + HK);
#pragma unroll
    for (int k = 0; k < HK; ++k)
      lane_reduce_plane<VW>(sm, aw[k], live, myvl, vl_n, C, c0, [&](int c, float t) { hp[k * C + c] = t; });
    if ((int)threadIdx.x < HK) {
      float t = 0.f;
      for (int l = 0; l < vl_n; ++l) t += hb[l * HK + threadIdx.x];
      hp[HK * C + threadIdx.x] = t;
    }
  }
}

__global__ void __launch_bounds__(256) gn_bwd_finish_kernel(float* __restrict__ red, int nb, int total ) {
  const int e = threadIdx.x & 7, g = threadIdx.x >> 3;
  const int i = blockIdx.x * 8 + e;
  const float* part = red + total;
  float s = 0.f;
  if (i < total) {
    const float* src = part + i;
    int b = g;
    for (; b + 7 * 32 < nb; b += 8 * 32) {
      float v[8];
#pragma unroll
      for (int u = 0; u < 8; ++u) v[u] = src[(size_t)(b + 32 * u) * total];
#pragma unroll
      for (int u = 0; u < 8; ++u) s += v[u];
    }
    for (; b < nb; b += 32) s += src[(size_t)b * total];
  }
  __shared__ float sm[32][8];
  sm[g][e] = s;
  __syncthreads();
  if (g == 0 && i < total) {
#pragma unroll
    for (int k = 1; k < 32; ++k) s += sm[k][e];
    red[i] = s;
  }
}

template <typename T, bool HEAVY, bool NT = false, int HK = 0>
__global__ void __launch_bounds__(256) gn_bwd_apply_kernel(const T* __restrict__ dz, int dzpitch, const T* __restrict__ y,
                                                           int ypitch, const float* __restrict__ scale_shift,
                                                           const float* __restrict__ mean_rstd, const float* __restrict__ gamma,
                                                           const float* __restrict__ red, T* __restrict__ dy, int dypitch,
                                                           float* __restrict__ dgamma, float* __restrict__ dbeta, int act,
                                                           SlopeArg sl, int N, int voxels, int C, int groups,
                                                           uint32_t* __restrict__ amax, HeadFold hf) {
  constexpr int VW = 16 / sizeof(T);
  constexpr int HKA = HK > 0 ? HK : 1;
  const float slope = sl.p ? *sl.p : sl.v;
  extern __shared__ float sm[];
  float* m12 = sm;
  const int n = blockIdx.y;
  const int cpg = C / groups;
  const float invM = 1.f / ((float)cpg * (float)voxels);
  for (int g = threadIdx.x; g < groups; g += blockDim.x) {
    float t1 = 0.f, t2 = 0.f;
    for (int j = 0; j < cpg; ++j) {
      const int c = g * cpg + j;
      t1 += gamma[c] * red[((size_t)n * C + c) * 2];
      t2 += gamma[c] * red[((size_t)n * C + c) * 2 + 1];
    }
    m12[g * 2] = t1 * invM;
    m12[g * 2 + 1] = t2 * invM;
  }
  if (blockIdx.x == 0 && blockIdx.y == 0 && dgamma) {
    for (int c = threadIdx.x; c < C; c += blockDim.x) {
      float b = 0.f, g = 0.f;
      for (int m = 0; m < N; ++m) { b += red[((size_t)m * C + c) * 2]; g += red[((size_t)m * C + c) * 2 + 1]; }
      dbeta[c] = b;
      dgamma[c] = g;
    }
  }
  __syncthreads();
  const int cv = C / VW;
  const int vl_n = blockDim.x / cv;
  const int mycv = threadIdx.x % cv, myvl = threadIdx.x / cv;
  const bool live = myvl < vl_n;
  const int c0 = mycv * VW;
  float sc[VW], sh[VW], ca[VW], cb[VW], ck[VW];
#pragma unroll
  for (int j = 0; j < VW; ++j) {
    const int c = c0 + j, g = c / cpg;
    sc[j] = scale_shift[((size_t)n * C + c) * 2];
    sh[j] = scale_shift[((size_t)n * C + c) * 2 + 1];
    const float mean = mean_rstd[(n * groups + g) * 2], rstd = mean_rstd[(n * groups + g) * 2 + 1];
    const float m1 = m12[g * 2], m2 = m12[g * 2 + 1];
    ca[j] = rstd * gamma[c];
    cb[j] = -rstd * rstd * m2;
    ck[j] = rstd * (mean * rstd * m2 - m1);
  }
  const T* dzb = dz + (size_t)n * voxels * dzpitch + c0;
  const T* yb = y + (size_t)n * voxels * ypitch + c0;
  T* dyb = dy + (size_t)n * voxels * dypitch + c0;
  const size_t stride = (size_t)gridDim.x * vl_n;
  size_t vox = live ? (size_t)blockIdx.x * vl_n + myvl : (size_t)voxels;
  float mx = 0.f;
  auto body = [&](const float* g, const float* yy, float* o) {
#pragma unroll
    for (int j = 0; j < VW; ++j) {
      const float u = g[j] * act_grad<HEAVY>(yy[j] * sc[j] + sh[j], act, slope);
      o[j] = u * ca[j] + (yy[j] * cb[j] + ck[j]);
    }
    if (amax) {
#pragma unroll
      for (int j = 0; j < VW; j += 2) mx = __builtin_fmaxf(__builtin_fmaxf(mx, __builtin_fabsf(o[j])), __builtin_fabsf(o[j + 1]));
    }
  };
  if constexpr (HK < 0) {
    const float nslope = act == BRATS_ACT_RELU ? 0.f : slope;
    auto step = [&](size_t v0, auto cnt) {
      constexpr int NVX = decltype(cnt)::value;
      typename Raw16<T>::type yr[NVX], skr[NVX], dpr[NVX], avr[NVX];
      uint32_t aw[NVX][VW / 4];
      int kk[NVX];
#pragma unroll
      for (int i = 0; i < NVX; ++i) {
        yr[i] = Raw16<T>::template load<NT>(yb + (v0 + i * stride) * ypitch);
        pool_dz<T, VW>(hf, n, v0 + i * stride, c0, C, skr[i], dpr[i], avr[i], aw[i], kk[i]);
      }
#pragma unroll
      for (int i = 0; i < NVX; ++i) {
        float yy[VW], g[VW], o[VW];
        Raw16<T>::unpack(yr[i], yy);
        pool_dz_finish<T, VW>(skr[i], dpr[i], avr[i], hf.with_avg, aw[i], kk[i], g);
#pragma unroll
        for (int j = 0; j < VW; ++j) {
          const float u = g[j] * (yy[j] * sc[j] + sh[j] > 0.f ? 1.f : nslope);
          o[j] = u * ca[j] + (yy[j] * cb[j] + ck[j]);
        }
        if (amax) {
#pragma unroll
          for (int j = 0; j < VW; j += 2) mx = __builtin_fmaxf(__builtin_fmaxf(mx, __builtin_fabsf(o[j])), __builtin_fabsf(o[j + 1]));
        }
        vstore<T, VW, NT>(dyb + (v0 + i * stride) * dypitch, o);
      }
    };
    for (; vox + stride < (size_t)voxels; vox += 2 * stride) step(vox, std::integral_constant<int, 2>{});
    for (; vox < (size_t)voxels; vox += stride) step(vox, std::integral_constant<int, 1>{});
  } else if constexpr (HK > 0) {
    float wr[HKA][VW];
#pragma unroll
    for (int k = 0; k < HK; ++k)
#pragma unroll
      for (int j = 0; j < VW; ++j) wr[k][j] = hf.w[k * C + c0 + j];
    const float* dl = hf.dl + (size_t)n * HK * voxels;
    const float nslope = act == BRATS_ACT_RELU ? 0.f : slope;
    auto step = [&](size_t v0, auto cnt) {
      constexpr int NV = decltype(cnt)::value;
      typename Raw16<T>::type yr[NV];
      float gq[NV][HKA];
#pragma unroll
      for (int i = 0; i < NV; ++i) yr[i] = Raw16<T>::template load<NT>(yb + (v0 + i * stride) * ypitch);
#pragma unroll
      for (int i = 0; i < NV; ++i)
#pragma unroll
        for (int k = 0; k < HK; ++k) gq[i][k] = dl[(size_t)k * voxels + v0 + i * stride];
#pragma unroll
      for (int i = 0; i < NV; ++i) {
        float yy[VW], o[VW];
        Raw16<T>::unpack(yr[i], yy);
#pragma unroll
        for (int j = 0; j < VW; ++j) {
          float d = 0.f;
#pragma unroll
          for (int k = 0; k < HK; ++k) d += gq[i][k] * wr[k][j];
          const float u = d * (yy[j] * sc[j] + sh[j] > 0.f ? 1.f : nslope);
          o[j] = u * ca[j] + (yy[j] * cb[j] + ck[j]);
        }
        if (amax) {
#pragma unroll
          for (int j = 0; j < VW; j += 2) mx = __builtin_fmaxf(__builtin_fmaxf(mx, __builtin_fabsf(o[j])), __builtin_fabsf(o[j + 1]));
        }
        vstore<T, VW, NT>(dyb + (v0 + i * stride) * dypitch, o);
      }
    };
    for (; vox + 3 * stride < (size_t)voxels; vox += 4 * stride) step(vox, std::integral_constant<int, 4>{});
    for (; vox < (size_t)voxels; vox += stride) step(vox, std::integral_constant<int, 1>{});
  } else {
  for (; vox + stride < (size_t)voxels; vox += 2 * stride) {
    float g0[VW], y0[VW], g1[VW], y1[VW], o0[VW], o1[VW];
    vload<T, VW, NT>(dzb + vox * dzpitch, g0);
    vload<T, VW, NT>(yb + vox * ypitch, y0);
    vload<T, VW, NT>(dzb + (vox + stride) * dzpitch, g1);
    vload<T, VW, NT>(yb + (vox + stride) * ypitch, y1);
    body(g0, y0, o0);
    body(g1, y1, o1);
    vstore<T, VW, NT>(dyb + vox * dypitch, o0);
    vstore<T, VW, NT>(dyb + (vox + stride) * dypitch, o1);
  }
  if (vox < (size_t)voxels) {
    float g0[VW], y0[VW], o0[VW];
    vload<T, VW, NT>(dzb + vox * dzpitch, g0);
    vload<T, VW, NT>(yb + vox * ypitch, y0);
    body(g0, y0, o0);
    vstore<T, VW, NT>(dyb + vox * dypitch, o0);
  }
  }
  if (amax) record_absmax<T>(mx, amax);
}

constexpr int GN_BWD_MAX_BLOCKS = 2048;
extern "C" size_t BRATS_API(brats_gn_bwd_ws_floats)(int N, int C) { return (size_t)(1 + GN_BWD_MAX_BLOCKS) * N * C * 2; }

template <typename F> static inline void with_fold(int fold, F&& f) {
  if (fold > 0) f(std::integral_constant<int, 3>{});
  else if (fold < 0) f(std::integral_constant<int, -1>{});
  else f(std::integral_constant<int, 0>{});
}

static int gn_act_bwd_impl(const void* dz, int dzpitch, const void* y, int ypitch, const float* scale_shift, const float* mean_rstd,
                           const float* gamma, void* dy, int dypitch, float* red, float* dgamma, float* dbeta, int dtype, int act,
                           SlopeArg slope, int N, int voxels, int C, int groups, float* amax, HeadFold hf, int K, hipStream_t st) {
  const int vw = vec_width(dtype);
  if (C % vw || C % groups || dzpitch % vw || ypitch % vw || dypitch % vw || C / vw > 256)
    BRATS_FAIL(BRATS_E_ARG, "gn_act_bwd: C=%d / pitches must be multiples of %d", C, vw);
  const Walk w = voxel_walk(vw, voxels, C);
  const bool big = big_tensor(dtype, (size_t)N * voxels * C);
  dim3 g1(w.grid(big ? GN_BWD_MAX_BLOCKS : 512), N), g2(w.grid(big ? 8192 : 2048), N);
  const size_t lds1 = (size_t)(w.vl * C * 2 + (K > 0 ? w.vl * K : 0)) * sizeof(float);
  const size_t lds2 = (size_t)2 * groups * sizeof(float);
  auto go = [&](auto t, auto heavy, auto nt, auto hk) {
    using T = typename decltype(t)::type;
    constexpr bool HEAVY = decltype(heavy)::value, NT = decltype(nt)::value;
    constexpr int HK = decltype(hk)::value;
    hipLaunchKernelGGL((gn_bwd_reduce_kernel<T, HEAVY, NT, HK>), g1, dim3(256), lds1, st, (const T*)dz, dzpitch, (const T*)y, ypitch,
                       scale_shift, mean_rstd, red, act, slope, voxels, C, groups, hf);
    hipLaunchKernelGGL(gn_bwd_finish_kernel, dim3((N * C * 2 + 7) / 8), dim3(256), 0, st, red, (int)g1.x, N * C * 2);
    hipLaunchKernelGGL((gn_bwd_apply_kernel<T, HEAVY, NT, HK>), g2, dim3(256), lds2, st, (const T*)dz, dzpitch, (const T*)y, ypitch,
                       scale_shift, mean_rstd, gamma, red, (T*)dy, dypitch, dgamma, dbeta, act, slope, N, voxels, C, groups,
                       (uint32_t*)amax, hf);
  };
  with_fold(K, [&](auto hk) {
    if constexpr (decltype(hk)::value != 0)
      with_stream(dtype, big, [&](auto t, auto nt) { go(t, std::false_type{}, nt, hk); });
    else
      with_act_stream(dtype, act > BRATS_ACT_LEAKY, big, [&](auto t, auto heavy, auto nt) { go(t, heavy, nt, hk); });
  });
  BRATS_CHECK_LAUNCH();
  return (int)g1.x;
}

extern "C" int BRATS_API(brats_gn_act_bwd)(const void* dz, int dzpitch, const void* y, int ypitch, const float* scale_shift,
                                const float* mean_rstd, const float* gamma, void* dy, int dypitch, float* red,
                                float* dgamma, float* dbeta, int dtype, int act, float slope_value, const float* slope_dev,
                                int N, int voxels, int C, int groups, float* amax, brats_stream_t s) {
  if (!dz || !y || !dy || !red || !scale_shift || !mean_rstd || !gamma) BRATS_FAIL(BRATS_E_ARG, "gn_act_bwd: null pointer");
  const int rc = gn_act_bwd_impl(dz, dzpitch, y, ypitch, scale_shift, mean_rstd, gamma, dy, dypitch, red, dgamma, dbeta, dtype, act,
                                 SlopeArg{slope_value, slope_dev}, N, voxels, C, groups, amax, HeadFold{}, 0, (hipStream_t)s);
  return rc < 0 ? rc : 0;
}

__global__ void __launch_bounds__(256) gn_bwd_tiles_finish_kernel(const double* __restrict__ part, int splits, int N, int C, int groups,
                                                                  const float* __restrict__ mean_rstd, float* __restrict__ red) {
  const int i = blockIdx.x * blockDim.x + threadIdx.x;
  if (i >= N * C) return;
  const int n = i / C, c = i % C;
  double s1 = 0.0, s2 = 0.0;
  const double* src = part + ((size_t)n * C + c) * 2;
  const size_t zs = (size_t)N * C * 2;
  int z = 0;
  for (; z + 8 <= splits; z += 8) {
    double v1[8], v2[8];
#pragma unroll
    for (int u = 0; u < 8; ++u) { v1[u] = src[(z + u) * zs]; v2[u] = src[(z + u) * zs + 1]; }
#pragma unroll
    for (int u = 0; u < 8; ++u) { s1 += v1[u]; s2 += v2[u]; }
  }
  for (; z < splits; ++z) { s1 += src[z * zs]; s2 += src[z * zs + 1]; }
  const int g = c / (C / groups);
  const double mean = mean_rstd[(n * groups + g) * 2], rstd = mean_rstd[(n * groups + g) * 2 + 1];
  red[(size_t)i * 2] = (float)s1;
  red[(size_t)i * 2 + 1] = (float)(rstd * (s2 - mean * s1));
}

extern "C" int BRATS_API(brats_gn_act_bwd_tiles)(const float* tile_stats, int tiles_per_sample, const void* dz, int dzpitch, const void* y,
                                      int ypitch, const float* scale_shift, const float* mean_rstd, const float* gamma, void* dy,
                                      int dypitch, float* red, float* dgamma, float* dbeta, int dtype, int act, float slope,
                                      int N, int voxels, int C, int groups, float* amax, brats_stream_t s) {
  if (!tile_stats || !dz || !y || !dy || !red || !scale_shift || !mean_rstd || !gamma || tiles_per_sample <= 0)
    BRATS_FAIL(BRATS_E_ARG, "gn_act_bwd_tiles: null pointer");
  if (dtype != BRATS_BF16 && dtype != BRATS_F32) BRATS_FAIL(BRATS_E_UNSUPPORTED, "gn_act_bwd_tiles: 16-bit or f32 (split-precision mode) activations");
  if (act != BRATS_ACT_RELU && act != BRATS_ACT_LEAKY) BRATS_FAIL(BRATS_E_UNSUPPORTED, "gn_act_bwd_tiles: relu / leakyrelu only (act %d)", act);
  const int vw = vec_width(dtype);
  if (C % vw || C % groups || dzpitch % vw || ypitch % vw || dypitch % vw || C / vw > 256)
    BRATS_FAIL(BRATS_E_ARG, "gn_act_bwd_tiles: C=%d / pitches must be multiples of %d", C, vw);
  hipStream_t st = (hipStream_t)s;
  double* part = (double*)(red + (((size_t)N * C * 2 + 1) / 2) * 2);
  const int splits = gn_splits(tiles_per_sample);
  hipLaunchKernelGGL(gn_chan_reduce_kernel, dim3((C + 15) / 16, N, splits), dim3(256), 0, st, tile_stats, tiles_per_sample, C, part);
  hipLaunchKernelGGL(gn_bwd_tiles_finish_kernel, dim3((N * C + 255) / 256), dim3(256), 0, st, part, splits, N, C, groups, mean_rstd, red);
  const bool big = big_tensor(dtype, (size_t)N * voxels * C);
  dim3 g2(voxel_walk(vw, voxels, C).grid(big ? 8192 : 2048), N);
  const size_t lds2 = (size_t)2 * groups * sizeof(float);
  with_stream(dtype, big, [&](auto t, auto nt) {
    using T = typename decltype(t)::type;
    hipLaunchKernelGGL((gn_bwd_apply_kernel<T, false, decltype(nt)::value, 0>), g2, dim3(256), lds2, st, (const T*)dz, dzpitch, (const T*)y,
                       ypitch, scale_shift, mean_rstd, gamma, red, (T*)dy, dypitch, dgamma, dbeta, act, SlopeArg{slope, nullptr}, N, voxels,
                       C, groups, (uint32_t*)amax, HeadFold{});
  });
  BRATS_CHECK_LAUNCH();
  return 0;
}

extern "C" size_t BRATS_API(brats_gn_bwd_head_ws_floats)(int N, int C, int K) { return (size_t)N * GN_BWD_MAX_BLOCKS * (K * C + K); }
extern "C" int BRATS_API(brats_gn_act_bwd_head)(const float* dlogits, const float* hw, int K, const void* y, int ypitch,
                                     const float* scale_shift, const float* mean_rstd, const float* gamma, void* dy, int dypitch,
                                     float* red, float* hws, float* dgamma, float* dbeta, float* dhw, float* dhb, int dtype,
                                     int act, float slope_value, int N, int voxels, int C, int groups, float* amax,
                                     brats_stream_t s) {
  if (!dlogits || !hw || !y || !dy || !red || !hws || !scale_shift || !mean_rstd || !gamma || !dhw || !dhb)
    BRATS_FAIL(BRATS_E_ARG, "gn_act_bwd_head: null pointer");
  if (K != 3 || act > BRATS_ACT_LEAKY)
    BRATS_FAIL(BRATS_E_UNSUPPORTED, "gn_act_bwd_head: built for K = 3 logit planes and relu / leakyrelu (K=%d, act=%d)", K, act);
  HeadFold hf;
  hf.dl = dlogits; hf.w = hw; hf.hpart = hws;
  const int nb = gn_act_bwd_impl(nullptr, 8, y, ypitch, scale_shift, mean_rstd, gamma, dy, dypitch, red, dgamma, dbeta, dtype, act,
                                 SlopeArg{slope_value, nullptr}, N, voxels, C, groups, amax, hf, K, (hipStream_t)s);
  if (nb < 0) return nb;
  return brats_ordered_sum2(hws, dhw, K * C, dhb, N * nb, K * C + K, (hipStream_t)s);
}

extern "C" int BRATS_API(brats_gn_act_bwd_pool)(const void* dskip, int dskip_pitch, const void* dpool, int dpool_pitch,
                                     const unsigned char* argmax, const void* y, int ypitch, const float* scale_shift,
                                     const float* mean_rstd, const float* gamma, void* dy, int dypitch, float* red, float* dgamma,
                                     float* dbeta, int dtype, int act, float slope_value, int N, int D, int H, int W, int C,
                                     int groups, float* amax, brats_stream_t s) {
  const int vw = vec_width(dtype);
  if (!dskip || !dpool || !argmax || !y || !dy || !red || !scale_shift || !mean_rstd || !gamma)
    BRATS_FAIL(BRATS_E_ARG, "gn_act_bwd_pool: null pointer");
  if (act > BRATS_ACT_LEAKY || ((D | H | W) & 1) || dskip_pitch % vw || dpool_pitch % vw)
    BRATS_FAIL(BRATS_E_UNSUPPORTED, "gn_act_bwd_pool: relu / leakyrelu, even spatial dims, pitches multiples of %d (act=%d)", vw, act);
  HeadFold hf;
  hf.dskip = dskip; hf.dpool = dpool; hf.argmax = argmax; hf.dskip_pitch = dskip_pitch; hf.dpool_pitch = dpool_pitch;
  hf.D = D; hf.H = H; hf.W = W;
  const int rc = gn_act_bwd_impl(nullptr, vw, y, ypitch, scale_shift, mean_rstd, gamma, dy, dypitch, red, dgamma, dbeta, dtype, act,
                                 SlopeArg{slope_value, nullptr}, N, D * H * W, C, groups, amax, hf, -1, (hipStream_t)s);
  return rc < 0 ? rc : 0;
}

template <typename T>
__global__ void __launch_bounds__(256) prelu_slope_grad_kernel(const T* __restrict__ dz, int dzpitch, const T* __restrict__ y, int ypitch,
                                                               const float* __restrict__ scale_shift, float* __restrict__ part,
                                                               int voxels, int C) {
  constexpr int VW = 16 / sizeof(T);
  const int n = blockIdx.y;
  const int cv = C / VW, vl_n = blockDim.x / cv;
  const int mycv = threadIdx.x % cv, myvl = threadIdx.x / cv, c0 = mycv * VW;
  float acc = 0.f;
  if (myvl < vl_n) {
    float sc[VW], sh[VW];
#pragma unroll
    for (int j = 0; j < VW; ++j) { sc[j] = scale_shift[((size_t)n * C + c0 + j) * 2]; sh[j] = scale_shift[((size_t)n * C + c0 + j) * 2 + 1]; }
    const T* dzb = dz + (size_t)n * voxels * dzpitch + c0;
    const T* yb = y + (size_t)n * voxels * ypitch + c0;
    for (size_t vox = (size_t)blockIdx.x * vl_n + myvl; vox < (size_t)voxels; vox += (size_t)gridDim.x * vl_n) {
      float g[VW], yy[VW];
      Vec<T, VW>::load(dzb + vox * dzpitch, g);
      Vec<T, VW>::load(yb + vox * ypitch, yy);
#pragma unroll
      for (int j = 0; j < VW; ++j) acc += g[j] * fminf(yy[j] * sc[j] + sh[j], 0.f);
    }
  }
  __shared__ float r[256];
  r[threadIdx.x] = acc;
  __syncthreads();
  for (int m = 128; m > 0; m >>= 1) {
    if ((int)threadIdx.x < m) r[threadIdx.x] += r[threadIdx.x + m];
    __syncthreads();
  }
  if (threadIdx.x == 0) part[(size_t)n * gridDim.x + blockIdx.x] = r[0];
}

constexpr int PRELU_MAX_BLOCKS = 1024;
extern "C" size_t BRATS_API(brats_prelu_ws_floats)(int N) { return (size_t)N * PRELU_MAX_BLOCKS; }
extern "C" int BRATS_API(brats_prelu_slope_grad)(const void* dz, int dzpitch, const void* y, int ypitch, const float* scale_shift, float* ws,
                                      float* dslope, int dtype, int N, int voxels, int C, brats_stream_t s) {
  const int vw = vec_width(dtype);
  if (!dz || !y || !scale_shift || !ws || !dslope || C % vw || dzpitch % vw || ypitch % vw || C / vw > 256)
    BRATS_FAIL(BRATS_E_ARG, "prelu_slope_grad: bad argument");
  hipStream_t st = (hipStream_t)s;
  const unsigned gx = voxel_walk(vw, voxels, C).grid(PRELU_MAX_BLOCKS);
  with_storage(dtype, [&](auto t) {
    using T = typename decltype(t)::type;
    hipLaunchKernelGGL(prelu_slope_grad_kernel<T>, dim3(gx, N), dim3(256), 0, st, (const T*)dz, dzpitch, (const T*)y, ypitch, scale_shift,
                       ws, voxels, C);
  });
  BRATS_CHECK_LAUNCH();
  return brats_ordered_sum(ws, dslope, N * (int)gx, 1, st);
}

extern "C" int BRATS_API(brats_evonorm_finalize)(const float* stats, int tiles_per_sample, int N, int C, int groups,
                                      double count_per_channel, float eps, float* mean_rstd, double* chan_ws,
                                      brats_stream_t s) {
  if (!stats || !mean_rstd || !chan_ws || C % groups || C / groups > 256) BRATS_FAIL(BRATS_E_ARG, "evonorm_finalize: bad argument");
  return gn_finalize_launch(stats, tiles_per_sample, N, C, groups, count_per_channel, eps, 1, nullptr, nullptr, mean_rstd, nullptr, chan_ws,
                            (hipStream_t)s);
}

DEVI float sigmoidf_(float x) { return __builtin_amdgcn_rcpf(1.f + __expf(-x)); }

template <typename T, bool NT = false>
__global__ void __launch_bounds__(256) evonorm_fwd_kernel(const T* __restrict__ x, int xpitch, const float* __restrict__ mean_rstd,
                                   const float* __restrict__ gamma, const float* __restrict__ beta, T* __restrict__ z,
                                   int zpitch, float* __restrict__ chansum, int voxels, int C, int groups,
                                   uint32_t* __restrict__ amax, const float* __restrict__ gscale) {
  constexpr int VW = 16 / sizeof(T);
  extern __shared__ float sm[];
  float* sc = sm;
  float* be = sm + C;
  const int n = blockIdx.y, cpg = C / groups;
  for (int c = threadIdx.x; c < C; c += blockDim.x) {
    const float gs = gscale ? gscale[(size_t)n * C + c] : 1.f;
    sc[c] = mean_rstd[(n * groups + c / cpg) * 2 + 1] * gamma[c] * gs;
    be[c] = beta[c] * gs;
  }
  __syncthreads();
  const int cv = C / VW, vl_n = blockDim.x / cv;
  const int mycv = threadIdx.x % cv, myvl = threadIdx.x / cv, c0 = mycv * VW;
  float acc[VW];
  float mx = 0.f;
#pragma unroll
  for (int j = 0; j < VW; ++j) acc[j] = 0.f;
  if (myvl < vl_n) {
    const T* xb = x + (size_t)n * voxels * xpitch;
    T* zb = z + (size_t)n * voxels * zpitch;
    for (size_t vox = (size_t)blockIdx.x * vl_n + myvl; vox < (size_t)voxels; vox += (size_t)gridDim.x * vl_n) {
      float a[VW];
      vload<T, VW, NT>(xb + vox * xpitch + c0, a);
#pragma unroll
      for (int j = 0; j < VW; ++j) {
        a[j] = a[j] * sigmoidf_(a[j]) * sc[c0 + j] + be[c0 + j];
        acc[j] += a[j];
      }
      if (amax) {
#pragma unroll
        for (int j = 0; j < VW; j += 2) mx = __builtin_fmaxf(__builtin_fmaxf(mx, __builtin_fabsf(a[j])), __builtin_fabsf(a[j + 1]));
      }
      vstore<T, VW, NT>(zb + vox * zpitch + c0, a);
    }
  }
  if (amax) record_absmax<T>(mx, amax);
  if (chansum) {
    float* scr = sm + 2 * C;
// ... 858 lines not shown
```

brats21_amd/networks/_program.py:

```python
import os

import torch
import torch.nn as nn

from .. import ops
from .._lib import BratsHipError


class _PackedWeightsModule(nn.Module):

    PRECISIONS = ("auto", "bf16", "fp16", "fp32", "x3", "fp16x3", "bf16x3", "x3fwd", "x3bwd")
    _cpu_hint = ""

    @property
    def precision(self):
        return self._precision

    @precision.setter
    def precision(self, value):
        if value not in self.PRECISIONS:
            raise ValueError(f"model.precision / BRATS_PRECISION must be one of {self.PRECISIONS}, got {value!r}")
        self._precision = value

    def train(self, mode=True):
        if mode != self.training:
            ops.invalidate_packed_weights()
        return super().train(mode)

    def _init_switches(self, pack_plan):
        self.precision = os.environ.get("BRATS_PRECISION", "auto")
        self.conv_fp8 = None
        self.skip_deep_heads_in_eval = False
        self._grad_sink = None
        self._grad_dest = None
        self.pack_plan = os.environ.get("BRATS_PACK_PLAN", pack_plan) != "0"
        self.fold_head_bwd = os.environ.get("BRATS_FOLD_HEAD", "1") != "0"
        self.fold_pool_bwd = os.environ.get("BRATS_FOLD_POOL", "1") != "0"
        self.fold_bwd_stats = os.environ.get("BRATS_FOLD_BWD_STATS", "1") != "0"
        self.fold_head_fwd = os.environ.get("BRATS_FOLD_HEAD_FWD", os.environ.get("BRATS_FOLD_HEAD", "1")) != "0"

    def _init_dropout(self, p):
        if not 0.0 <= float(p) < 1.0:
            raise ValueError(f"dropout probability has to be in [0, 1), got {p}")
        self.dropout_p = float(p)
        seed = 0
        if self.dropout_p > 0.0:
            seed = int(torch.randint(0, 2 ** 62, (1,), generator=torch.Generator().manual_seed(torch.initial_seed())))
        self._dropout_seed_base, self._dropout_rank_mixed = seed, self.dropout_p == 0.0
        self.register_buffer("_dropout_state", torch.tensor([seed, 0], dtype=torch.int64), persistent=False)

    def _advance_dropout(self, device):
        if self._dropout_state.device != device:
            raise BratsHipError("brats21_amd: module and input are on different devices")
        if not self._dropout_rank_mixed:
            rank = os.environ.get("RANK")
            if rank is None:
                import torch.distributed as dist
                rank = dist.get_rank() if dist.is_available() and dist.is_initialized() else 0
            self._dropout_state[0] = (self._dropout_seed_base + 0x9E3779B97F4A7C15 * int(rank)) % (2 ** 63)
            self._dropout_rank_mixed = True
        self._dropout_state[1] += 1
        return self._dropout_state.clone()

    def _weights_may_have_changed(self):
        if torch.is_grad_enabled():
            ops.invalidate_packed_weights()

    def _dtype(self):
        if self.precision == "bf16":
            return torch.bfloat16
        if self.precision == "fp16":
            return torch.float16
        if self.precision in ("fp32", "x3", "fp16x3", "bf16x3", "x3fwd", "x3bwd"):
            return torch.float32
        if torch.is_autocast_enabled():
            return torch.float16 if torch.get_autocast_dtype("cuda") == torch.float16 else torch.bfloat16
        return torch.float32

    def _x3_modes(self):
        if self.precision in ("x3", "fp16x3"):
            return ops.X3F, ops.X3F
        if self.precision == "bf16x3":
            return ops.X3B, ops.X3B
        if self.precision in ("x3fwd", "x3bwd"):
            return (ops.X3F, None) if self.precision == "x3fwd" else (None, ops.X3F)
        return None, None

    MAX_INPLANES = MAX_CLASSES = 16

    def _check_shape_limits(self, inplanes, num_classes, features, width_multiple):
        if int(inplanes) != inplanes or int(num_classes) != num_classes or inplanes < 1 or num_classes < 1:
            raise ValueError(f"{self.name}: inplanes and num_classes must be positive integers (got {inplanes!r}, {num_classes!r})")
        if inplanes > self.MAX_INPLANES:
            raise NotImplementedError(f"{self.name}: the input layer is built for inplanes <= {self.MAX_INPLANES} (got {inplanes})")
        if num_classes > self.MAX_CLASSES:
            raise NotImplementedError(f"{self.name}: the head kernels are built for num_classes <= {self.MAX_CLASSES} (got {num_classes})")
        if any(c % width_multiple for c in features):
            raise NotImplementedError(f"{self.name}: the convolution kernels need widths that are multiples of {width_multiple} "
                                      f"(got {list(features)})")
        self.inplanes = int(inplanes)

    def _run(self, fn, x):
        if not x.is_cuda:
            raise BratsHipError(f"brats21_amd.{self.name} runs on the GPU only (no CPU fallback){self._cpu_hint}")
        if x.dim() != 5 or x.shape[1] != self.inplanes or any(s % 8 for s in x.shape[2:]):
            raise ValueError(f"expected input [N, {self.inplanes}, D, H, W] with D, H, W divisible by 8")
        refinement = getattr(self, "refinement", False)
        if refinement and any(s % 16 for s in x.shape[2:]):
            raise ValueError(f"refinement=True: expected input [N, {self.inplanes}, D, H, W] with D, H, W divisible by 16")
        if refinement and self.conv_fp8:
            raise NotImplementedError("refinement=True with the e4m3 convolution path (conv_fp8) is not implemented")
        self._fwd_grad = torch.is_grad_enabled()
        self._weights_may_have_changed()
        if self.training and self.pack_plan and torch.is_grad_enabled():
            ops.plan_for(self, x.device)
        outs = fn.apply(self, x.float(), self._dtype(), *self.parameters())
        if refinement:
            return ([outs[0], outs[1]], list(outs[2:])) if self.deep_supervision else [outs[0], outs[1]]
        if self.deep_supervision:
            return outs[0], list(outs[1:])
        return outs[0]


class _AmaxSlots:

    def __init__(self, n, device):
        self.buf = torch.zeros(n, dtype=torch.float32, device=device)
        self.i = 0

    def take(self):
        s = self.buf[self.i:self.i + 1]
        self.i += 1
        return s


def _inherit_amax(dst, src):
    a = getattr(src, "_amax", None)
    if a is not None:
        dst._amax = a
    return dst


def douts_device(douts):
    return next(d.device for d in douts if d is not None)


class _Ctx:

    def __init__(self, model, dtype, will_bwd=False):
        self.m, self.dtype = model, dtype
        self.fp8 = getattr(model, "conv_fp8", None) if ops.is16(dtype) else None
        self.x3s = ops.x3_mode() == ops.X3F and dtype == torch.float32
        self.slots = None
        self._names = None
        self.grads = {}
        self.recs = {}
        self.drop = None
        self.act, self.training = getattr(model, "act", None), model.training
        self.will_bwd = will_bwd
        self.lazy_ok = (not will_bwd and not torch.is_grad_enabled() and getattr(model, "norm_on_load", False)
                        and ops.is16(dtype))

    @property
    def names(self):
        if self._names is None:
            self._names = {p: i for i, p in enumerate(self.m.parameters())}
        return self._names

    def start_dropout(self, device):
        m = self.m
        if m.training and m.dropout_p > 0.0:
            if self.fp8:
                raise NotImplementedError("--dropout > 0 with the e4m3 convolution path is not implemented")
            self.drop = (m.dropout_p, m._advance_dropout(device))

    def drop_of(self, unit):
        return self.m._unit_ids[unit] if self.drop is not None else None

    def dropped(self, t, uid, out=None):
        if self.drop is None or uid is None:
            return t
        return ops.dropout(t, self.drop[0], self.drop[1], uid, out=out)

    def slot(self, device, force=False):
        if not self.fp8 and not force:
            return None
        if self.slots is None or self.slots.i >= self.slots.buf.numel():
            self.slots = _AmaxSlots(64, device)
        return self.slots.take()

    def identity_ss(self, n, c, device):
# ... 65 lines not shown
```

brats21_amd/networks/equiunet.py:

```python
import contextlib
import functools
import math
import os

import torch
import torch.nn as nn

from .. import ops
from .._lib import PACK_DGRAD, PACK_FWD, BratsHipError
from ._program import _PackedWeightsModule, _fn_backward, _fn_forward, _heads_bwd, _inherit_amax, input_cpad


class _ConvParams(nn.Module):

    def __init__(self, cin, cout, k, bias):
        super().__init__()
        self.weight = nn.Parameter(torch.empty(cout, cin, k, k, k))
        self.bias = nn.Parameter(torch.empty(cout)) if bias else None
        nn.init.kaiming_uniform_(self.weight, a=math.sqrt(5))
        if bias:
            bound = 1.0 / math.sqrt(cin * k * k * k)
            nn.init.uniform_(self.bias, -bound, bound)


# ... 93 lines not shown
        self.conv0 = _ConvParams(in_ch, inc_ch, 3, bias=True)
        for name in ("hx1", "hx2", "hx3", "hx4", "hx5"):
            setattr(self, name, ConvBnRelu(inc_ch, inc_ch, 1, norm, act))
        for name in ("d4", "d3", "d2", "d1"):
            setattr(self, name, ConvBnRelu(inc_ch * 2, inc_ch, 1, norm, act))
        self.conv_d0 = _ConvParams(inc_ch, in_ch, 3, bias=True)


def _head(cin, k):
    return nn.ModuleList([_ConvParams(cin, k, 1, bias=True)])


def _f8_ok(fp8, dtype, x, x2=None):
    return (bool(fp8) and ops.is16(dtype) and not getattr(x, "_net_input", False) and x.shape[1] >= ops.F8_MIN_SIZE and
            ops.conv_f8_chunk(x.shape[-1], x2.shape[-1] if x2 is not None else 0) > 0)


def _unit_act(unit, act):
    if act == "prelu":
        return "leakyrelu", unit.prelu.weight.detach()
    return act, None


def _one_sample(t):
    n, d, h, w, c = t.shape
    if not t.is_contiguous():
        raise BratsHipError("--norm batch needs dense activations")
    return t.view(1, n * d, h, w, c)


def _blk(b):
    return b.ConvBnRelu1, b.ConvBnRelu2


def _bn_fwd_tail(cx, unit, x, x2, y, stats, pool):
    n, d, h, wd, c = y.shape
    bn = unit.bn
    if cx.training:
        mean_rstd, scale_shift = ops.gn_finalize(stats.view(1, -1, c, 2), 1, c, c, n * d * h * wd, bn.weight.detach(), bn.bias.detach())
        with torch.no_grad():
            cnt = float(n * d * h * wd)
            mean = mean_rstd[0, :, 0]
            var = (1.0 / mean_rstd[0, :, 1].double() ** 2 - 1e-5).clamp_min(0).float()
            bn.running_mean.mul_(0.9).add_(mean, alpha=0.1)
            bn.running_var.mul_(0.9).add_(var, alpha=0.1 * cnt / max(cnt - 1.0, 1.0))
            bn.num_batches_tracked += 1
    else:
        mean_rstd = None
        scale = bn.weight.detach() * torch.rsqrt(bn.running_var + 1e-5)
        scale_shift = torch.stack([scale, bn.bias.detach() - bn.running_mean * scale], -1).reshape(1, c, 2).contiguous().float()
    kact, slope_t = _unit_act(unit, cx.act)
    z = ops.affine_act(_one_sample(y), scale_shift, kact, slope_t=slope_t).view(n, d, h, wd, c)
    cx.dropped(z, cx.drop_of(unit), out=z)
    cx.recs[unit] = (unit, x, x2, y, mean_rstd, scale_shift)
    if pool:
        return z, ops.maxpool2(z, want_argmax=pool == "argmax")
    return z


def _cgr_fwd(cx, unit, x, x2=None, *, no_act=False, pool=False, lazy=False):
    dtype, fp8 = cx.dtype, cx.fp8
    uid = cx.drop_of(unit)
    lazy = lazy and cx.lazy_ok and uid is None
    if pool:
        pool = "argmax" if cx.will_bwd else True
    w = unit.conv.weight
    cbias, gamma_c, beta_c = None, unit.bn.weight.detach(), unit.bn.bias.detach()
    if unit.bcn:
        if torch.is_grad_enabled():
            a_c, cbias, gamma_c, beta_c = unit.bn.tables()
            w = w.detach() * a_c.view(-1, 1, 1, 1, 1)
        else:
            srcs = (unit.conv.weight, unit.bn.weight, unit.bn.bias, unit.bn.bn.weight, unit.bn.bn.bias, unit.bn.bn.running_var,
                    unit.bn.bn.running_mean)
            key = (ops.pack_generation(),) + tuple((t._version, t.data_ptr()) for t in srcs)
            hit = getattr(unit, "_bcn_fold", None)
            if hit is None or hit[0] != key:
                a_c, cbias, gamma_c, beta_c = unit.bn.tables()
                hit = unit._bcn_fold = (key, (w.detach() * a_c.view(-1, 1, 1, 1, 1), cbias, gamma_c, beta_c))
            w, cbias, gamma_c, beta_c = hit[1]
        fp8, lazy = None, False
    elif unit.conv.bias is not None:
        cbias, fp8 = unit.conv.bias.detach(), None
    cout = w.shape[0]
    cin_pad = x.shape[-1] + (x2.shape[-1] if x2 is not None else 0)
    c1 = x.shape[-1] if x2 is not None else None
    if isinstance(x, ops.Pending) or isinstance(x2, ops.Pending):
        if fp8 or not ops.conv_pre_ok(dtype, 3, unit.dilation, x.shape[-1], x2.shape[-1] if x2 is not None else 0, cout):
            x = x.materialize() if isinstance(x, ops.Pending) else x
            x2 = x2.materialize() if isinstance(x2, ops.Pending) else x2
    if _f8_ok(fp8, dtype, x, x2):
        wpk = ops.pack_weights_f8(w, PACK_FWD, cin_pad=cin_pad, c1=c1)
        y, stats = ops.conv3d_f8(x, wpk, cout, unit.dilation, want_stats=True, x2=x2, amax=getattr(x, "_amax", None),
                                 amax2=getattr(x2, "_amax", None) if x2 is not None else None)
    else:
        with ops.use_plan(None) if unit.bcn else contextlib.nullcontext():
            wpk = ops.pack_weights(w, dtype, PACK_FWD, cin_pad=cin_pad, dil=unit.dilation, c1=c1)
        y, stats = ops.conv3d(x, wpk, cout, 3, unit.dilation, want_stats=True, x2=x2, amax=getattr(x, "_x3amax", None), bias=cbias)
    n, d, h, wd, _ = y.shape
    if unit.batch_norm:
        return _bn_fwd_tail(cx, unit, x, x2, y, stats, pool)
    mean_rstd, scale_shift = ops.gn_finalize(stats, n, cout, unit.groups, d * h * wd, gamma_c, beta_c)
    rec = (unit, x, x2, y, mean_rstd, scale_shift)
    if no_act:
        cx.recs[unit] = rec
        return y
    amax = cx.slot(y.device)
    kact, slope_t = _unit_act(unit, cx.act)
    if lazy and slope_t is None and kact in ("relu", "leakyrelu") and amax is None and not pool:
        return ops.Pending(y, scale_shift, kact)
    cx.recs[unit] = rec
    if pool and uid is None and kact in ("relu", "leakyrelu") and y.numel() * y.element_size() >= (256 << 20):
        z, pooled = ops.affine_act_pool(y, scale_shift, kact, amax=amax, slope_t=slope_t, want_argmax=pool == "argmax")
        if amax is not None:
            z._amax = pooled._amax = amax
        return z, pooled
    z = ops.affine_act(y, scale_shift, kact, amax=amax, slope_t=slope_t)
    if amax is not None:
        z._amax = amax
    cx.dropped(z, uid, out=z)
    if pool:
        return z, _inherit_amax(ops.maxpool2(z, want_argmax=pool == "argmax"), z)
    return z


def _cgr_bwd(cx, unit, dz, *, need_dx=True, head=None, pool=None, bst=None):
    _, x, x2, y, mean_rstd, scale_shift = cx.recs[unit]
    dtype, fp8 = cx.dtype, cx.fp8
    if bst is not None:
        bst = cx.recs[bst] if (cx.m.fold_bwd_stats and cx.drop is None) else None
    cin = unit.conv.weight.shape[1]
    gamma_c = unit.bn.weight.detach()
    w_bwd = unit.conv.weight
    if unit.bcn:
        a_c, _, gamma_c, _ = unit.bn.tables()
        w_bwd = unit.conv.weight.detach() * a_c.view(-1, 1, 1, 1, 1)
        fp8 = None
    elif unit.conv.bias is not None:
        fp8 = None
    tiles = None
    if isinstance(dz, tuple):
        dz, tiles = dz
    dz = cx.dropped(dz, cx.drop_of(unit))
    all8 = fp8 == "all" and ops.is16(dtype)
    f8 = all8 and need_dx and ops.conv_f8_chunk(y.shape[-1]) > 0
    ax, ax2 = getattr(x, "_amax", None), (getattr(x2, "_amax", None) if x2 is not None else None)
    w8 = (all8 and unit.dilation == 1 and ax is not None and (x2 is None or ax2 is not None) and ops.is16(y.dtype)
          and ops.conv3d_wgrad_f8_ok(x, y, x2))
    x3s = cx.x3s
    amax = cx.slot(y.device, True) if (f8 or w8 or x3s) else None
    kact, slope_t = _unit_act(unit, cx.act)
    if slope_t is not None:
        cx.put(unit.prelu.weight, ops.prelu_slope_grad(dz, y, scale_shift))
    if unit.batch_norm:
        if mean_rstd is None:
            raise NotImplementedError("--norm batch: backward through an eval-mode forward (running statistics) is not implemented")
        n_, d_, h_, w_, c_ = y.shape
        dy, dgamma, dbeta = ops.gn_act_bwd(_one_sample(dz), _one_sample(y), scale_shift, mean_rstd, gamma_c, c_, kact,
                                           amax=amax, slope_t=slope_t)
        dy = dy.view(n_, d_, h_, w_, c_)
        if amax is not None:
            dy._amax = amax
    elif head is not None:
        hd, dout = head
        dy, dgamma, dbeta, dhw, dhb = ops.gn_act_bwd_head(dout, hd.weight, y, scale_shift, mean_rstd, gamma_c,
                                                          unit.groups, kact, amax=amax)
        cx.put(hd.weight, dhw)
        cx.put(hd.bias, dhb)
    elif pool is not None:
        dy, dgamma, dbeta = ops.gn_act_bwd_pool(pool[0], pool[1], pool[2], y, scale_shift, mean_rstd, gamma_c,
                                                unit.groups, kact, amax=amax)
    elif tiles is not None:
        dy, dgamma, dbeta = ops.gn_act_bwd_tiles(tiles, dz, y, scale_shift, mean_rstd, gamma_c, unit.groups, kact,
                                                 amax=amax)
    else:
        dy, dgamma, dbeta = ops.gn_act_bwd(dz, y, scale_shift, mean_rstd, gamma_c, unit.groups, kact, amax=amax,
                                           slope_t=slope_t)
    wdst = cx.dest(unit.conv.weight)
    if w8 and amax is not None:
        dw = ops.conv3d_wgrad_f8(x, dy, ax, amax, x2=x2, amax2=ax2, out=wdst)
    elif x2 is not None and x.shape[-1] % 16:
        dw, db = ops.conv3d_wgrad(torch.cat([x, x2], -1), dy, 3, unit.dilation, amax_dy=amax if x3s else None, want_dbias=unit.bcn)
    else:
        dw, db = ops.conv3d_wgrad(x, dy, 3, unit.dilation, x2=x2, out=None if unit.bcn else wdst, amax_dy=amax if x3s else None,
                                  want_dbias=unit.bcn)
    dw = dw[:, :cin].contiguous() if dw.shape[1] != cin else dw
    if unit.bcn:
        pg = _bcn_param_grads(unit, dw, db, dgamma, dbeta)
    else:
        pg = {unit.conv.weight: dw, unit.bn.weight: dgamma, unit.bn.bias: dbeta}
        if unit.conv.bias is not None:
            pg[unit.conv.bias] = ops.channel_dot(dy).sum(0)
    for prm, g in pg.items():
        cx.put(prm, g)
    if not need_dx:
        return None
    if f8:
        wpk = ops.pack_weights_f8(unit.conv.weight, PACK_DGRAD)

        def dgrad(**kw):
            return ops.conv3d_f8(dy, wpk, cin, unit.dilation, amax=amax, **kw)
    else:
        with ops.use_plan(None) if unit.bcn else contextlib.nullcontext():
            wpk = ops.pack_weights(w_bwd, dtype, PACK_DGRAD, dil=unit.dilation)

        def dgrad(**kw):
            return ops.conv3d(dy, wpk, cin, 3, unit.dilation, amax=amax if x3s else None, **kw)
    if x2 is None:
        if bst is not None and not f8:
            u1, _, _, y1, mr1, ss1 = bst
            kact1, slope1 = _unit_act(u1, cx.act)
            if (not u1.batch_norm and not u1.bcn and not unit.bcn and mr1 is not None and y1.shape[-1] == cin and y1.dtype == dy.dtype
                    and ops.conv_bstats_ok(dtype, unit.dilation, dy.shape[-1], cin, kact1, slope1)):
                return ops.conv3d_bstats(dy, wpk, cin, unit.dilation, y1, ss1, kact1, amax=amax if x3s else None)
        dx, _ = dgrad()
        return dx
    c1 = x.shape[-1]
    if c1 % ops.split_granule(cin) == 0:
        dx, _ = dgrad(split=c1)
        return dx
    dx, _ = dgrad()
    return dx[..., :c1], dx[..., c1:]


def _level_bwd(cx, unit, down, d_pooled, d_skip, need_dx=True, bst=None):
    idx = getattr(down, "_pool_argmax", None)
    kact, slope_t = _unit_act(unit, cx.act)
    if (idx is not None and cx.m.fold_pool_bwd and cx.drop is None and not unit.batch_norm and slope_t is None
            and kact in ("relu", "leakyrelu")):
        return _cgr_bwd(cx, unit, None, need_dx=need_dx, pool=(d_skip, d_pooled, idx), bst=bst)
    return _cgr_bwd(cx, unit, ops.maxpool2_bwd(down, d_pooled, dx_skip=d_skip), need_dx=need_dx, bst=bst)


def _ref_cpad(k):
    return 8 if k <= 8 else 16


def _ref_amax(cx, t):
    return ops.absmax(t) if cx.x3s else None


def _ref_fwd(ctx, cx, out):
    r, dtype = cx.m.refunet, cx.dtype
    cgr = functools.partial(_cgr_fwd, cx)
    k, f0 = out.shape[1], r.conv0.weight.shape[0]
    x0 = ops.ncdhw_to_ndhwc(out, dtype, cpad=input_cpad(k, dtype))
    x0._net_input = True
    amax0 = ops.absmax(x0) if ops.x3_mode() == ops.X3F else None
    wpk = ops.pack_weights(r.conv0.weight, dtype, PACK_FWD, cin_pad=x0.shape[-1])
    hx, _ = ops.conv3d(x0, wpk, f0, 3, 1, bias=r.conv0.bias.detach(), amax=amax0)
    hx1, p = cgr(r.hx1, hx, pool=True)
    hx2, p = cgr(r.hx2, p, pool=True)
    hx3, p = cgr(r.hx3, p, pool=True)
    hx4, p = cgr(r.hx4, p, pool=True)
    d = cgr(r.hx5, p)
    for unit, skip in ((r.d4, hx4), (r.d3, hx3), (r.d2, hx2), (r.d1, hx1)):
        d = cgr(unit, ops.upsample(d, 2), x2=skip)
    ctx.ref = (x0, hx1, hx2, hx3, hx4, d)
    return ops.conv3d_narrow(d, ops.pack_weights_narrow(r.conv_d0.weight, PACK_FWD), k, bias=r.conv_d0.bias.detach(), add=out)


def _ref_bwd(ctx, cx, d_ref, d_out):
    r, dtype = cx.m.refunet, cx.dtype
    cbw = functools.partial(_cgr_bwd, cx)
    x0, hx1, hx2, hx3, hx4, d1 = ctx.ref
    ctx.ref = None
    if d_ref is None:
        d_ref = torch.zeros(ctx.out_shape, dtype=torch.float32, device=d1.device)
    d_ref = d_ref.contiguous().float()
    k, f0 = d_ref.shape[1], d1.shape[-1]
    dy = ops.ncdhw_to_ndhwc(d_ref, dtype, cpad=_ref_cpad(k))
    amax = _ref_amax(cx, dy)
    dw, _ = ops.conv3d_wgrad(d1, dy, 3, 1, amax_dy=amax)
    cx.put(r.conv_d0.weight, dw[:k].contiguous())
    cx.put(r.conv_d0.bias, ops.channel_dot(dy).sum(0)[:k].contiguous())
    wpad = torch.zeros((dy.shape[-1],) + tuple(r.conv_d0.weight.shape[1:]), dtype=torch.float32, device=d1.device)
    wpad[:k] = r.conv_d0.weight.detach()
    with ops.use_plan(None):
        wpk = ops.pack_weights(wpad, dtype, PACK_DGRAD)
    g, _ = ops.conv3d(dy, wpk, f0, 3, 1, amax=amax)
    skips = []
    for unit in (r.d1, r.d2, r.d3, r.d4):
        g_up, g_skip = cbw(unit, g)
        skips.append(g_skip)
        g = ops.upsample_bwd(g_up, 2)
    g = cbw(r.hx5, g)
    for unit, down in ((r.hx4, hx4), (r.hx3, hx3), (r.hx2, hx2), (r.hx1, hx1)):
        g = _level_bwd(cx, unit, down, g, skips.pop())
    dw0, _ = ops.conv3d_wgrad(x0, g, 3, 1, amax_dy=_ref_amax(cx, g))
    cx.put(r.conv0.weight, dw0[:, :k].contiguous())
    cx.put(r.conv0.bias, ops.channel_dot(g).sum(0))
    rest = d_ref if d_out is None else d_ref + d_out.float()
    return ops.conv3d_narrow(g, ops.pack_weights_narrow(r.conv0.weight, PACK_DGRAD), k, add=rest)


def _deep_heads_on(m):
    return m.deep_supervision and not (m.skip_deep_heads_in_eval and not m.training)


def _plus(a, b):
    return a if b is None else a + b


def _decoder_fwd(ctx, cx, down1, down2, down3, down4, bottom, bottom_2):
    m = cx.m
    cgr = functools.partial(_cgr_fwd, cx)

    def up(t):
        return _inherit_amax(ops.upsample(t, 2), t)

    up3 = cgr(m.decoder3.ConvBnRelu2, cgr(m.decoder3.ConvBnRelu1, down3, x2=up(bottom_2), lazy=True))
    up2 = cgr(m.decoder2.ConvBnRelu2, cgr(m.decoder2.ConvBnRelu1, down2, x2=up(up3), lazy=True))
    u1 = cgr(m.decoder1.ConvBnRelu1, down1, x2=up(up2), lazy=True)
    last = m.decoder1.ConvBnRelu2
    kact, slope_t = _unit_act(last, cx.act)
    nk = m.outconv.weight.shape[0]
    fuse_top = (m.fold_head_fwd and cx.drop is None and not last.batch_norm and slope_t is None and kact in ("relu", "leakyrelu")
                and nk <= 4 and (not cx.will_bwd or (m.fold_head_bwd and ops.head_fold_ok(m.outconv.weight, kact, slope_t))))
    if fuse_top:
        y1 = cgr(last, u1, no_act=True)
        up1 = None
        outs = [ops.gn_head(y1, cx.recs[last][5], m.outconv.weight, m.outconv.bias, kact)]
    else:
        up1 = cgr(last, u1)
        outs = [ops.head(up1, m.outconv.weight, m.outconv.bias, 1)]
    ctx.top_fused = fuse_top
    ctx.out_shape = tuple(outs[0].shape)
    ctx.heads = [(m.outconv, up1, 1)]
    if _deep_heads_on(m):
        for hd, src, sc in ((m.deep_bottom[0], bottom, 8), (m.deep_bottom2[0], bottom_2, 8), (m.deep3[0], up3, 4),
                            (m.deep2[0], up2, 2)):
            outs.append(ops.head(src, hd.weight, hd.bias, sc))
# ... 129 lines not shown
```

brats21_amd/ops.py:

```python
import contextlib
import weakref

import numpy as np
import torch

from . import _lib
from ._lib import ACT_LEAKY, ACT_NONE, ACT_RELU, BF16, F16, F32, PACK_DGRAD, PACK_FWD, X3_BF16, X3_F16

from ._tensors import (X3B, X3F, _NO_ACT, _SIZES, _act, _act2, _code, _conv_packed, _desc, _desc2, _even, _f32, _finalize_in,
                       _groups, _head_weight, _out, _packed, _planes, _tile_stats, _vec)

ACTS = {"none": ACT_NONE, "relu": ACT_RELU, "leakyrelu": ACT_LEAKY, "elu": _lib.ACT_ELU, "swish": _lib.ACT_SWISH,
        "mish": _lib.ACT_MISH}


class KernelTimer:

    def __init__(self):
        self.records = {}

    def span(self, key):
        return _Span(self, key)

    def summary(self):
# ... 1563 lines not shown
POOL_FUSED_MIN_BYTES = 256 << 20


def rrcnn_fwd(x, x2, params, groups=8, act="relu", t=2, save=True, pool=False):
    if x3_active():
        raise NotImplementedError("rrcnn_fwd: the split-precision modes are not built for the recurrent block")
    a, a2 = _conv_sources(x, x2, "rrcnn_fwd")
    ps, c, cin = _rrcnn_params(params, a)
    if t < 1:
        raise _lib.BratsHipError(f"rrcnn_fwd: t = {t} (t >= 1)")
    if pool:
        _even(a, "rrcnn_fwd(pool=True)")
    (n, d, h, w, c1), c2 = a.shape, a2.c
    if (x2 is not None and c1 + c2 != cin) or (x2 is None and c1 < cin):
        raise _lib.BratsHipError(f"rrcnn_fwd: the block is built for {cin} input channels, the tensors have {c1} + {c2}")
    if c % groups:
        raise _lib.BratsHipError(f"rrcnn_fwd: {c} channels in {groups} groups")
    dtype, dev, vox = x.dtype, x.device, d * h * w
    sv = RrcnnSaved()
    sv.x, sv.x2, sv.groups, sv.act, sv.t, sv.n = x, x2, groups, act, t, n
    sv.S, sv.Y, sv.ss, sv.mr = [], [], [[], []], [[], []]
    if save:
        for _ in range(4):
            (sv.S if len(sv.S) < 2 else sv.Y).append(new_act((t + 1) * n, d, h, w, c, dtype, dev))
        x0 = sv.S[0][:n]
    else:
        x0 = new_act(n, d, h, w, c, dtype, dev)
        ybuf, ping = new_act(n, d, h, w, c, dtype, dev), [new_act(n, d, h, w, c, dtype, dev) for _ in range(2)]
    wpk = pack_weights(params[8], dtype, PACK_FWD, cin_pad=c1 + c2, c1=c1 if x2 is not None else None)
    conv3d(x, wpk, c, 1, 1, bias=ps[9], out=x0, x2=x2)
    xb = x0
    for b in (0, 1):
        _, bias, gamma, beta = ps[4 * b:4 * b + 4]
        wpk = pack_weights(params[4 * b], dtype, PACK_FWD)
        cur = xb
        for k in range(t + 1):
            yk = sv.Y[b][k * n:(k + 1) * n] if save else ybuf
            _, stats = conv3d(cur, wpk, c, 3, 1, bias=bias, out=yk, want_stats=True)
            mean_rstd, scale_shift = gn_finalize(stats, n, c, groups, vox, gamma, beta)
            if save:
                sv.ss[b].append(scale_shift)
                sv.mr[b].append(mean_rstd)
            if k < t:
                nxt = sv.S[b][(k + 1) * n:(k + 2) * n] if save else ping[b]
                cur = affine_act_add(yk, scale_shift, xb, act, out=nxt)
            elif b == 0:
                xb = affine_act(yk, scale_shift, act, out=sv.S[1][:n] if save else ping[0])
            elif not pool:
                out = affine_act_add(yk, scale_shift, x0, act, out=None if save else ping[1])
            elif yk.numel() * yk.element_size() >= POOL_FUSED_MIN_BYTES:
                out = affine_act_add(yk, scale_shift, x0, act, out=None if save else ping[1], pool=True, want_argmax=save)
            else:
                out = affine_act_add(yk, scale_shift, x0, act, out=None if save else ping[1])
                out = out, maxpool2(out, want_argmax=save)
    return out, (sv if save else None)


def rrcnn_bwd(dout, saved, params, need_dx=True):
    sv = saved
    if not isinstance(sv, RrcnnSaved):
        raise _lib.BratsHipError("rrcnn_bwd: saved must come from rrcnn_fwd(save=True)")
    if x3_active():
        raise NotImplementedError("rrcnn_bwd: the split-precision modes are not built for the recurrent block")
    ps, c, cin = _rrcnn_params(params, sv.x)
    _rrcnn_saved(sv, c, cin, dout)
    n, t, x, x2 = sv.n, sv.t, sv.x, sv.x2
    dtype = x.dtype
    grads = [None] * 10
    dz = dout
    for b in (1, 0):
        gamma = ps[4 * b + 2]
        S, Y = sv.S[b], sv.Y[b]
        DY = torch.empty_like(Y)
        wpk = pack_weights(params[4 * b], dtype, PACK_DGRAD)
        ds, small = [None] * (t + 1), []
        for k in range(t, -1, -1):
            sl = slice(k * n, (k + 1) * n)
            _, dgamma, dbeta = gn_act_bwd(dz, Y[sl], sv.ss[b][k], sv.mr[b][k], gamma, sv.groups, sv.act, out=DY[sl])
            small.append((dgamma, dbeta))
            ds[k], _ = conv3d(DY[sl], wpk, c, 3, 1)
            dz = ds[k]
        dz = grad_sum(*(ds + ([dout] if b == 0 else [])))
        grads[4 * b], _ = conv3d_wgrad(S, DY, 3, 1)
        grads[4 * b + 1] = channel_dot(DY).sum(0)
        gb = torch.stack([g for g, _ in small] + [g for _, g in small]).view(2, t + 1, c).sum(1)
        grads[4 * b + 2], grads[4 * b + 3] = gb[0], gb[1]
    d_x0 = dz
    c1 = x.shape[-1]
    dws = [conv3d_wgrad_shift(s, d_x0, 1)[0] for s in ((x,) if x2 is None else (x, x2))]
    dw1 = dws[0] if x2 is None else torch.cat(dws, 1)
    grads[8] = dw1[:, :cin].contiguous() if dw1.shape[1] != cin else dw1
    grads[9] = channel_dot(d_x0).sum(0)
    if not need_dx:
        return None, None, grads
    wpk = pack_weights(params[8], dtype, PACK_DGRAD, cin_pad=c1 if x2 is None else None)
    if x2 is None:
        dx, _ = conv3d(d_x0, wpk, c1, 1, 1)
        return dx, None, grads
    if c1 % split_granule(cin) == 0:
        (dx, dx2), _ = conv3d(d_x0, wpk, cin, 1, 1, split=c1)
        return dx, dx2, grads
    dx, _ = conv3d(d_x0, wpk, cin, 1, 1)
    return dx[..., :c1], dx[..., c1:], grads


def probe_box(device=None, mfma_ms=50.0, stream_bytes=403 << 20, modes=(0, 1)):
    dev = torch.device("cuda", torch.cuda.current_device()) if device is None else torch.device(device)
    l = _lib.lib()
    ncu = torch.cuda.get_device_properties(dev).multi_processor_count
    blocks = 2 * ncu
    out = torch.empty(blocks, dtype=torch.float32, device=dev)
    ev = [torch.cuda.Event(enable_timing=True) for _ in range(4)]

    def mfma(iters, mode):
        ev[0].record()
        _lib.check(l.brats_probe_mfma(out.data_ptr(), blocks, iters, mode, _stream()), "probe_mfma")
        ev[1].record()
        ev[1].synchronize()
        return ev[0].elapsed_time(ev[1])

    res = {}
    for mode in modes:
        mfma(2000, mode)
        t0 = mfma(20000, mode)
        iters = max(20000, int(20000 * mfma_ms / max(t0, 1e-3)))
        ms = mfma(iters, mode)
        tf = blocks * 4.0 * iters * 8 * 16384 / (ms * 1e-3) / 1e12
        res[mode] = (tf, ms, iters)
    src = torch.empty(stream_bytes, dtype=torch.uint8, device=dev)
    src.view(torch.int16).fill_(0x3c00)
    dst = torch.empty_like(src)
    for _ in range(2):
        _lib.check(l.brats_probe_stream(src.data_ptr(), dst.data_ptr(), stream_bytes, _stream()), "probe_stream")
    reps = 8
    ev[2].record()
    for _ in range(reps):
        _lib.check(l.brats_probe_stream(src.data_ptr(), dst.data_ptr(), stream_bytes, _stream()), "probe_stream")
    ev[3].record()
    ev[3].synchronize()
    sms = ev[2].elapsed_time(ev[3]) / reps
    rec = {"stream_TBps": round(2.0 * stream_bytes / (sms * 1e-3) / 1e12, 3)}
    names = {0: "mfma", 1: "mfma_zeros", 2: "mfma_duty_dense", 3: "mfma_duty"}
    for mode, (tf, ms, iters) in res.items():
        rec[names[mode] + "_TFLOPs"] = round(tf, 1)
    if 0 in res:
        rec["sclk_MHz"] = round(2.0 * res[0][2] * 8 * 16 / (res[0][1] * 1e-3) / 1e6, 0)
    rec["probe"] = (f"csrc/probe.hip: {blocks} x 4 waves issuing v_mfma_f32_16x16x32_bf16 back to back, ~{mfma_ms:.0f} ms per mode (mfma = dense "
                    f"random operands: the sustained matrix rate, sclk = the clock behind it at 16 cycles per MFMA and SIMD; mfma_zeros = "
                    f"every second value zero); bf16 read + write stream over {stream_bytes >> 20} MiB, {sms * 1e3:.0f} us per pass")
    return rec


from ._attgate import AttGateSaved, attgate_bwd, attgate_fwd
```

include/brats_hip.h:

```cpp
#ifndef BRATS_HIP_H
#define BRATS_HIP_H
#include <stddef.h>
#include <stdint.h>

#ifdef __cplusplus
extern "C" {
#endif

typedef void* brats_stream_t;

enum { BRATS_F32 = 0, BRATS_BF16 = 1, BRATS_F16 = 2, BRATS_X3_BF16 = 3, BRATS_X3_F16 = 4 };
enum { BRATS_E_ARG = -1, BRATS_E_UNSUPPORTED = -2, BRATS_E_HIP = -3 };
enum { BRATS_ACT_NONE = 0, BRATS_ACT_RELU = 1, BRATS_ACT_LEAKY = 2, BRATS_ACT_ELU = 3, BRATS_ACT_SWISH = 4, BRATS_ACT_MISH = 5 };

#define BRATS_ABI_VERSION 7
int brats_abi_version(void);
const char* brats_last_error(void);

int brats_dropout(const void* x, int xpitch, void* out, int opitch, int dtype, size_t voxels, int C, float p,
                  const void* state, int unit, brats_stream_t s);

int brats_ncdhw_to_ndhwc(const float* src, void* dst, int dtype, int N, int C, int cpad, int dst_pitch,
                         int D, int H, int W, brats_stream_t s);
int brats_ndhwc_to_ncdhw(const void* src, int src_pitch, float* dst, int dtype, int N, int C,
                         int D, int H, int W, brats_stream_t s);

enum { BRATS_PACK_FWD = 0, BRATS_PACK_DGRAD = 1 };
size_t brats_conv3d_packed_bytes(int dtype, int ksize, int cin, int cout, int ck);
int brats_conv3d_chunk(int dtype, int ksize, int dil, int c1, int c2, int cout);
int brats_conv3d_pack_weights(const float* w, void* packed, int dtype, int mode, int ksize,
                              int cout_w, int cin_w, int cin_off, int cin_cnt, int ck, brats_stream_t s);
typedef struct {
  const float* w;
  void* out;
  int dtype, mode, taps, cin_w, cin_real, cin_off, rows, rows16, kdim, ck, ms_n, reserved;
  unsigned long long total;
} brats_pack_job;
int brats_conv3d_pack_blocks(int kdim, int ck, int rows);
int brats_conv3d_pack_weights_multi(const brats_pack_job* jobs, const int* blocks , int nblocks,
                                    brats_stream_t s);
int brats_conv3d_pack_weights_multi_f16(const brats_pack_job* jobs, const int* blocks , int nblocks,
                                    brats_stream_t s);
int brats_conv3d_tiles_per_sample(int D, int H, int W);
int brats_conv3d_split_granule(int cout);
int brats_conv3d_set_vs8(int mode);
int brats_conv3d_set_kp(int mode);
int brats_conv3d_fwd(const void* x1, int c1, int pitch1, const void* x2, int c2, int pitch2,
                     const void* packed_w, const float* bias, void* y, int ypitch,
                     void* y2, int y2pitch, int ysplit, float* stats,
                     int dtype, int ksize, int dil, int N, int D, int H, int W, int cout,
                     brats_stream_t s);
int brats_conv3d_pre_ok(int dtype, int ksize, int dil, int c1, int c2, int cout);
int brats_conv3d_fwd_pre(const void* x1, int c1, int pitch1, const float* ss1, const void* x2, int c2, int pitch2,
                         const float* ss2, int act, float slope, const void* packed_w, const float* bias, void* y, int ypitch,
                         float* stats, int dtype, int dil, int N, int D, int H, int W, int cout, brats_stream_t s);
int brats_conv3d_bstats_ok(int dtype, int ksize, int dil, int c1, int cout);
int brats_conv3d_fwd_bstats(const void* x1, int c1, int pitch1, const void* packed_w, void* y, int ypitch,
                            const void* fwd_y, int fwd_pitch, const float* scale_shift, int act, float slope,
                            float* tile_stats, int dtype, int dil, int N, int D, int H, int W, int cout, brats_stream_t s);
int brats_conv3d_x3_fwd(const void* x1, int c1, int pitch1, const void* x2, int c2, int pitch2, const float* xamax,
                        const void* packed_w, const float* bias, void* y, int ypitch, void* y2, int y2pitch, int ysplit,
                        float* stats, int dtype, int dil, int N, int D, int H, int W, int cout, brats_stream_t s);
int brats_conv3d_x3_fwd_bstats(const void* x1, int c1, int pitch1, const float* xamax, const void* packed_w, void* y, int ypitch,
                               const void* fwd_y, int fwd_pitch, const float* scale_shift, int act, float slope,
                               float* tile_stats, int dtype, int dil, int N, int D, int H, int W, int cout, brats_stream_t s);
int brats_conv3d_f8_chunk(int c1, int c2);
size_t brats_conv3d_f8_packed_bytes(int cin, int cout, int ck);
int brats_conv3d_f8_pack_weights(const float* w, void* packed, int mode, int cout_w, int cin_w, int cin_off,
                                 int cin_cnt, int ck, brats_stream_t s);
int brats_conv3d_f8_fwd(const void* x1, int c1, int pitch1, const float* amax1, const void* x2, int c2, int pitch2,
                        const float* amax2, float xscale, const void* packed_w, const float* bias, void* y, int ypitch,
                        void* y2, int y2pitch, int ysplit, float* stats, int dil, int N, int D, int H, int W, int cout,
                        brats_stream_t s);
int brats_conv3d_f8_fwd_f16(const void* x1, int c1, int pitch1, const float* amax1, const void* x2, int c2, int pitch2,
                        const float* amax2, float xscale, const void* packed_w, const float* bias, void* y, int ypitch,
                        void* y2, int y2pitch, int ysplit, float* stats, int dil, int N, int D, int H, int W, int cout,
                        brats_stream_t s);
int brats_absmax(const void* x, int pitch, int dtype, size_t rows, int C, float* out, brats_stream_t s);
size_t brats_conv3d_wgrad_ws_bytes(int dtype, int ksize, int N, int D, int H, int W, int c1, int c2, int cout);
int brats_conv3d_set_wgrad_alltaps(int mode);
int brats_conv3d_set_wgrad_noslab(int mode);
int brats_conv3d_wgrad_noslab_taken(int dtype, int dil, int N, int D, int H, int W, int c1, int c2, int cout);
int brats_conv3d_set_x3_wgrad_fused(int mode);
int brats_conv3d_wgrad(const void* x1, int c1, int pitch1, const void* x2, int c2, int pitch2,
                       const void* dy, int dypitch, float* ws, float* dw, float* dbias,
                       int dtype, int ksize, int dil, int N, int D, int H, int W, int cout,
                       brats_stream_t s);
int brats_conv3d_x3_wgrad(const void* x1, int c1, int pitch1, const void* x2, int c2, int pitch2, const void* dy, int dypitch,
                          const float* amax_dy, float* ws, float* dw, float* dbias, int dtype, int dil, int N, int D, int H,
                          int W, int cout, brats_stream_t s);
size_t brats_conv3d_wgrad_f8_ws_bytes(int N, int D, int H, int W, int c1, int c2, int cout);
int brats_conv3d_wgrad_f8(const void* x1, int c1, int pitch1, const float* amax1, const void* x2, int c2, int pitch2,
                          const float* amax2, const void* dy, int dypitch, const float* amax_dy, float* ws, float* dw,
                          int N, int D, int H, int W, int cout, brats_stream_t s);
int brats_conv3d_wgrad_f8_f16(const void* x1, int c1, int pitch1, const float* amax1, const void* x2, int c2, int pitch2,
                          const float* amax2, const void* dy, int dypitch, const float* amax_dy, float* ws, float* dw,
                          int N, int D, int H, int W, int cout, brats_stream_t s);
size_t brats_conv3d_wgrad_shift_ws_bytes(int dtype, int ksize, int N, int D, int H, int W, int cin, int cout);
int brats_conv3d_wgrad_shift(const void* x, int cin, int xpitch, const void* dy, int dypitch, float* ws, float* dw,
                             float* dbias, int dtype, int ksize, int dil, int N, int D, int H, int W, int cout,
                             brats_stream_t s);
int brats_conv3d_x3_wgrad_shift(const void* x, int cin, int xpitch, const void* dy, int dypitch, const float* amax_dy,
                                float* ws, float* dw, float* dbias, int dtype, int ksize, int dil, int N, int D, int H, int W,
                                int cout, brats_stream_t s);

size_t brats_gn_ws_doubles(int N, int C);
int brats_gn_finalize(const float* stats, int tiles_per_sample, int N, int C, int groups,
                      double count_per_channel, float eps, const float* gamma, const float* beta,
                      float* mean_rstd , float* scale_shift ,
                      double* chan_ws , brats_stream_t s);
int brats_affine_act_fwd(const void* y, int ypitch, const float* scale_shift, void* z, int zpitch,
                         int dtype, int act, float slope, const float* slope_dev, int N, int voxels, int C, float* amax,
                         brats_stream_t s);
int brats_affine_act_add_fwd(const void* y, int ypitch, const float* scale_shift, const void* add, int addpitch, void* s,
                             int spitch, int dtype, int act, float slope, const float* slope_dev, int N, int voxels, int C,
                             brats_stream_t stream);
int brats_grad_sum(const void* src0, int pitch0, const void* src1, int pitch1, const void* src2, int pitch2, const void* src3,
                   int pitch3, int nsrc, void* dst, int dpitch, int dtype, int N, int voxels, int C, brats_stream_t stream);
int brats_affine_act_pool_fwd(const void* y, int ypitch, const float* scale_shift, void* z, int zpitch, void* pooled,
                              int ppitch, unsigned char* argmax ,
                              int dtype, int act, float slope, const float* slope_dev, int N, int D, int H, int W, int C,
                              int with_avg, float* amax, brats_stream_t s);
int brats_affine_act_add_pool_fwd(const void* y, int ypitch, const float* scale_shift, const void* add, int addpitch, void* s,
                                  int spitch, void* pooled, int ppitch, unsigned char* argmax, int dtype, int act, float slope,
                                  const float* slope_dev, int N, int D, int H, int W, int C, brats_stream_t stream);
size_t brats_gn_bwd_ws_floats(int N, int C);
int brats_gn_act_bwd(const void* dz, int dzpitch, const void* y, int ypitch, const float* scale_shift,
                     const float* mean_rstd, const float* gamma, void* dy, int dypitch,
                     float* red , float* dgamma, float* dbeta,
                     int dtype, int act, float slope, const float* slope_dev, int N, int voxels, int C, int groups,
                     float* amax , brats_stream_t s);
int brats_gn_act_bwd_tiles(const float* tile_stats, int tiles_per_sample, const void* dz, int dzpitch, const void* y,
                           int ypitch, const float* scale_shift, const float* mean_rstd, const float* gamma, void* dy,
                           int dypitch, float* red , float* dgamma, float* dbeta, int dtype, int act,
                           float slope, int N, int voxels, int C, int groups,
                           float* amax , brats_stream_t s);
size_t brats_gn_bwd_head_ws_floats(int N, int C, int K);
int brats_gn_act_bwd_head(const float* dlogits, const float* hw, int K, const void* y, int ypitch, const float* scale_shift,
                          const float* mean_rstd, const float* gamma, void* dy, int dypitch, float* red ,
                          float* hws, float* dgamma, float* dbeta, float* dhw, float* dhb, int dtype, int act, float slope,
                          int N, int voxels, int C, int groups, float* amax, brats_stream_t s);
int brats_gn_act_bwd_pool(const void* dskip, int dskip_pitch, const void* dpool, int dpool_pitch, const unsigned char* argmax,
                          const void* y, int ypitch, const float* scale_shift, const float* mean_rstd, const float* gamma,
                          void* dy, int dypitch, float* red, float* dgamma, float* dbeta, int dtype, int act, float slope,
                          int N, int D, int H, int W, int C, int groups, float* amax, brats_stream_t s);
size_t brats_prelu_ws_floats(int N);
int brats_prelu_slope_grad(const void* dz, int dzpitch, const void* y, int ypitch, const float* scale_shift, float* ws,
                           float* dslope, int dtype, int N, int voxels, int C, brats_stream_t s);

size_t brats_chan_ws_floats(int N, int C, int vals);
int brats_evonorm_finalize(const float* stats, int tiles_per_sample, int N, int C, int groups,
                           double count_per_channel, float eps, float* mean_rstd, double* chan_ws,
                           brats_stream_t s);
int brats_evonorm_fwd(const void* x, int xpitch, const float* mean_rstd, const float* gamma,
                      const float* beta, void* z, int zpitch, float* chansum, int dtype, int N,
                      int voxels, int C, int groups,
                      float* amax , brats_stream_t s);
int brats_evonorm_bwd(const void* dz, int dzpitch, const void* x, int xpitch, const float* mean_rstd,
                      const float* gamma, void* dx, int dxpitch, float* red ,
                      float* dgamma, float* dbeta, const double* chan_sums, float* dconvbias,
                      int dtype, int N, int voxels, int C, int groups,
                      float* amax ,
                      const float* gscale, const float* gadd ,
                      brats_stream_t s);
size_t brats_evonorm_bwd_tiles_ws_floats(int N, int C);
int brats_evonorm_bwd_tiles(const float* tile_stats, int tiles_per_sample, const void* dz, int dzpitch, const void* x,
                            int xpitch, const float* mean_rstd, const float* gamma, const float* beta, void* dx, int dxpitch,
                            float* red, float* dgamma, float* dbeta, const double* chan_sums, float* dconvbias, int dtype,
                            int N, int voxels, int C, int groups, float* amax, brats_stream_t s);
int brats_se_fwd(const float* chansum, float inv_vox, const float* w1, const float* b1, const float* w2, const float* b2,
                 float* gate1p , float* hidden , int N, int C, int Ch, brats_stream_t s);
int brats_se_bwd(const float* dgate, const float* chansum, float inv_vox, const float* hidden, const float* gate1p,
                 const float* w1, const float* w2, float* gadd , float* dw1, float* db1, float* dw2, float* db2,
                 int N, int C, int Ch, brats_stream_t s);
int brats_evonorm_se_bwd(const void* dout, int dopitch, const void* x, int xpitch, const float* mean_rstd, const float* gamma,
                         const float* beta, void* dx, int dxpitch, float* ws, float* dgamma, float* dbeta,
                         const double* chan_sums, float* dconvbias, const float* se_chansum, const float* hidden,
                         const float* gate1p, const float* w1, const float* w2, float* gadd, float* dw1, float* db1,
                         float* dw2, float* db2, int Ch,
                         const float* dlogits ,
                         const float* hw , int K, float* hws ,
                         float* dhw , float* dhb ,
                         int dtype, int N, int voxels, int C, int groups, float* amax, brats_stream_t s);
int brats_evonorm_se_bwd_pool(const void* dskip, int dskip_pitch, const void* dpool, int dpool_pitch, const unsigned char* argmax,
                              int with_avg, int D, int H, int W, const void* x, int xpitch, const float* mean_rstd,
                              const float* gamma, const float* beta, void* dx, int dxpitch, float* ws, float* dgamma,
                              float* dbeta, const double* chan_sums, float* dconvbias, const float* se_chansum,
                              const float* hidden, const float* gate1p, const float* w1, const float* w2, float* gadd,
                              float* dw1, float* db1, float* dw2, float* db2, int Ch, int dtype, int N, int C, int groups,
                              float* amax, brats_stream_t s);
int brats_evonorm_se_fwd(const void* x, int xpitch, const float* mean_rstd, const float* gamma, const float* beta,
                         const float* w1, const float* b1, const float* w2, const float* b2, void* out, int opitch,
                         float* ws, float* chansum_out, float* gate1p, float* hidden, int Ch, int dtype, int N, int voxels,
                         int C, int groups, float* amax ,
                         brats_stream_t s);
int brats_channel_dot(const void* a, int apitch, const void* b , int bpitch, float* out ,
                      int dtype, int N, int voxels, int C, brats_stream_t s);
int brats_channel_scale(const void* a, int apitch, const float* scale , const float* add ,
                        void* dst, int dpitch, int dtype, int N, int voxels, int C,
                        float* amax , brats_stream_t s);
typedef struct { const void* x; const void* w; int xpitch, cin, ksize, dil; } brats_dconv_term;
typedef struct { brats_dconv_term term[4]; int nterms, rows; const float* bias; void* y; int ypitch, reserved; } brats_dconv_job;
size_t brats_dconv_packed_bytes(int dtype, int ksize, int kdim, int rows);
int brats_dconv_pack_weights(const float* w, void* packed, int dtype, int mode, int ksize, int cout_w, int cin_w,
                             int cin_off, int cin_cnt, brats_stream_t s);
int brats_dconv_run(const brats_dconv_job* jobs, int njobs, int dtype, int N, int D, int H, int W, brats_stream_t s);

int brats_maxpool2_fwd(const void* x, int xpitch, void* y, int ypitch,
                       unsigned char* argmax ,
                       int dtype, int N, int C, int D, int H, int W, int with_avg, brats_stream_t s);
int brats_maxpool2_bwd(const void* x, int xpitch, const void* y, int ypitch, const void* dy, int dypitch,
                       const void* dx_skip, int dxskip_pitch, void* dx, int dxpitch, int dtype,
                       int N, int C, int D, int H, int W, int with_avg, brats_stream_t s);
int brats_maxpool2_bwd_idx(const unsigned char* argmax, const void* dy, int dypitch, const void* dx_skip ,
                           int dxskip_pitch, void* dx, int dxpitch, int dtype, int N, int C, int D, int H, int W,
                           int with_avg, brats_stream_t s);

int brats_upsample_fwd(const void* x, int xpitch, void* y, int ypitch, int dtype, int N, int C,
                       int D, int H, int W, int scale, brats_stream_t s);
size_t brats_upsample_bwd_ws_bytes(int dtype, int N, int C, int D, int H, int W, int scale);
int brats_upsample_bwd(const void* dy, int dypitch, void* dx, int dxpitch, void* tmp, int dtype,
                       int N, int C, int D, int H, int W, int scale, brats_stream_t s);
int brats_upsample_bwd_add(const void* dy, int dypitch, const void* add, int addpitch, void* dx, int dxpitch, void* tmp,
                           int dtype, int N, int C, int D, int H, int W, int scale, brats_stream_t s);
int brats_upsample_bwd_set_fused(int mode);

int brats_upsample_nearest_fwd(const void* x, int xpitch, void* y, int ypitch, int dtype, int N, int C,
                               int D, int H, int W, int scale, brats_stream_t s);
int brats_upsample_nearest_bwd(const void* dy, int dypitch, const void* add , int addpitch, void* dx, int dxpitch,
                               int dtype, int N, int C, int D, int H, int W, int scale, brats_stream_t s);
int brats_planes_nearest_fwd(const float* low, float* out, int planes, int D, int H, int W, int scale, brats_stream_t s);
int brats_planes_nearest_bwd(const float* dout, float* dlow, int planes, int D, int H, int W, int scale, brats_stream_t s);

size_t brats_conv3d_narrow_packed_bytes(int C, int K);
int brats_conv3d_narrow_pack(const float* w, float* packed, int mode, int cout_w, int cin_w, brats_stream_t s);
// ... 238 lines not shown
```

Baseline: 141.4 patches/s.

## Fuse GroupNorm+activation backward into the first conv's weight-gradient kernel

Result: no change. 142.1 patches/s (median of 6 runs) (+0.5%).

```diff
diff --git a/brats21_amd/_first_bwd.py b/brats21_amd/_first_bwd.py
--- /dev/null
+++ b/brats21_amd/_first_bwd.py
@@ -0,0 +1,28 @@
+import torch
+
+from . import _lib, ops
+from ._tensors import _act, _tile_stats
+
+
+def conv3d_wgrad_gn_bwd_tiles(x, tile_stats, dz, y, scale_shift, mean_rstd, gamma, groups=8, act="relu", slope=0.01, out=None):
+    what = "conv3d_wgrad_gn_bwd_tiles"
+    a = _act(y, (what, "y"))
+    g = _act(dz, (what, "dz"), a)
+    xa = _act(x, (what, "x"), a, anyc=True)
+    ts = _tile_stats(tile_stats, a, a.c, (what, "tile_stats"))
+    ss, mr, gm = ops._gn_bwd_args(a, scale_shift, mean_rstd, gamma, groups, what)
+    n, d, h, w, c, cout = a.n, a.d, a.h, a.w, xa.c, a.c
+    if not (ops.is16(a.dtype) and act in ("relu", "leakyrelu") and gm is not None and
+            _lib.lib().brats_conv3d_wgrad_gn_bwd_taken(a.code, n, d, h, w, c, xa.pitch, cout, g.pitch, a.pitch, groups, ops.ACTS[act])):
+        return None
+    f32 = dict(dtype=torch.float32, device=a.device)
+    red = torch.empty(_lib.lib().brats_gn_bwd_ws_floats(n, cout), **f32)
+    dgamma, dbeta = torch.empty(cout, **f32), torch.empty(cout, **f32)
+    ws = torch.empty(max(_lib.lib().brats_conv3d_wgrad_ws_bytes(a.code, 3, n, d, h, w, c, 0, cout), 4) // 4, **f32)
+    dw = ops._grad_out(out, (cout, c, 3, 3, 3), a.device)
+    with ops._span("conv_wgrad", c, cout, 3, 1, n, d, h, w, str(a.dtype)):
+        _lib.check(_lib.lib().brats_conv3d_wgrad_gn_bwd_tiles(xa.ptr, c, xa.pitch, ts, tile_stats.shape[1], g.ptr, g.pitch, a.ptr, a.pitch,
+                                                              ss, mr, gm, red.data_ptr(), dgamma.data_ptr(), dbeta.data_ptr(),
+                                                              ws.data_ptr(), dw.data_ptr(), a.code, ops.ACTS[act], float(slope), groups,
+                                                              n, d, h, w, cout, ops._stream()), what)
+    return dw, dgamma, dbeta
diff --git a/brats21_amd/csrc/conv_wgrad.hip b/brats21_amd/csrc/conv_wgrad.hip
--- a/brats21_amd/csrc/conv_wgrad.hip
+++ b/brats21_amd/csrc/conv_wgrad.hip
@@ -1,6 +1,7 @@
 #include <stdlib.h>
 #include "twin_begin.hpp"
 #include "common.hpp"
+#include "gn_bwd_apply.hpp"
 
 typedef __attribute__((ext_vector_type(4))) short s16x4;
 
@@ -13,6 +14,13 @@
   int nlane;
   int ntaps, dil;
   int seglen, nsegz;
+};
+struct WgradGnFold {
+  const void* dz; const void* y; int dzp, yp;
+  const float* scale_shift; const float* mean_rstd; const float* gamma; const float* red;
+  float* dgamma; float* dbeta;
+  int act, groups;
+  float slope;
 };
 
 constexpr int WG_TZ = 4, WG_TY = 4, WG_TX = 16, WG_VOX = 256;
@@ -439,184 +447,29 @@
   static_assert(YPIECES % 512 == 0, "");
 };
 
+template <bool GNB> struct WgGnbState {
+  u32x4 rz[4];
+  unsigned yokm = 0;
+  int n_pend = -1, n_coef = -1;
+  float sc[8], sh[8], ca[8], cb[8], ck[8];
+};
+template <> struct WgGnbState<false> {};
+template <bool GNB> struct WgGnbLoads { __amdgpu_buffer_rsrc_t zrs; int zorg, n; };
+template <> struct WgGnbLoads<false> {};
+DEVI int wg_gnb_piece(int tid, int i) { return i < 3 ? tid + 510 * i : (WG_VOX - 1) * 6 + tid; }
+DEVI bool wg_gnb_mine(int tid, int i) { return i < 3 ? tid < 510 : tid < 6; }
+
 template <int COF, int CIF>
 __global__ __launch_bounds__(512, 1) void conv_wgrad_alltaps2_kernel(const WgradParams p) {
-  typedef bf16_t T;
-  using G = Wg3b<COF, CIF>;
-  extern __shared__ __attribute__((aligned(16))) char lds[];
-  char* ldy = lds + 2 * G::XB;
-  const int tid = threadIdx.x, lane = tid & 63;
-  const int wave = __builtin_amdgcn_readfirstlane(tid >> 6);
-  const int q = lane >> 4, v = lane & 15;
-  const int lane8 = blockIdx.x % p.nlane, gsub = blockIdx.x / p.nlane, g8 = gridDim.x / p.nlane;
-  const int split = blockIdx.x;
-  const int tpx = (p.ntiles + p.nlane - 1) / p.nlane;
-  const int tile_end = min(p.ntiles, (lane8 + 1) * tpx);
-  const int co0 = blockIdx.y * G::CO, ci0 = blockIdx.z * G::CI;
-  const T* xsrc;
-  int xpitch;
-  if (ci0 < p.c1) { xsrc = (const T*)p.x1 + ci0; xpitch = p.p1; }
-  else { xsrc = (const T*)p.x2 + (ci0 - p.c1); xpitch = p.p2; }
-  const int xpb = xpitch * 2, ypb = p.dyp * 2;
-
-  int xoffs[G::XI], xcode[G::XI];
-#pragma unroll
-  for (int i = 0; i < G::XI; ++i) {
-    const int P = tid + 512 * i;
-    const int vox = P / G::XPPV, part = P % G::XPPV;
-    const int hx = vox % G::HX, hy = (vox / G::HX) % G::HY, hz = vox / (G::HX * G::HY);
-    const bool ok = P < G::XPIECES && (CIF > 1 || part * 8 < p.c1);
-    xoffs[i] = ok ? ((hz * p.H + hy) * p.W + hx) * xpb + part * 16 : (int)0x80000000;
-    xcode[i] = ok ? (hz | hy << 3 | hx << 6 | 1 << 14) : 0;
-  }
-  const unsigned xsample_bytes = (unsigned)p.D * p.H * p.W * xpitch * 2;
-  const unsigned ysample_bytes = (unsigned)p.D * p.H * p.W * p.dyp * 2;
-
-  int poff[G::PPW];
-#pragma unroll
-  for (int jj = 0; jj < G::PPW; ++jj) {
-    const int pid = wave + 8 * jj;
-    const int t = pid / CIF, nn = pid % CIF;
-    poff[jj] = pid < G::PAIRS ? (((t / 9) * G::HY + (t / 3) % 3) * G::HX + t % 3) * G::SX + nn * 32 : 0;
-  }
-  f32x4 acc[G::PPW][COF];
-#pragma unroll
-  for (int jj = 0; jj < G::PPW; ++jj)
-#pragma unroll
-    for (int m = 0; m < COF; ++m) acc[jj][m] = f32x4{0.f, 0.f, 0.f, 0.f};
-
-  u32x4 ry[G::YI];
-  struct TileLoads {
-    rsrc4_t xrs;
-    __amdgpu_buffer_rsrc_t yrs;
-    int xorg, yorg;
-    unsigned zm, ym, xm, inter;
-    char* xdst;
-  };
-  auto setup_loads = [&](int tile, int buf) {
-    TileLoads L;
-    int bt = tile;
-    const int x0 = (bt % p.tx) * WG_TX; bt /= p.tx;
-    const int y0 = (bt % p.ty) * WG_TY; bt /= p.ty;
-    const int z0 = (bt % p.tz) * WG_TZ;
-    const int n = bt / p.tz;
-    const size_t sample_vox = (size_t)n * p.D * p.H * p.W;
-    L.xrs = make_rsrc4(xsrc + sample_vox * xpitch, xsample_bytes);
-    L.yrs = __builtin_amdgcn_make_buffer_rsrc((void*)((const T*)p.dy + sample_vox * p.dyp + co0), (short)0, (int)ysample_bytes, 0x00020000);
-    L.xorg = (((z0 - 1) * p.H + (y0 - 1)) * p.W + (x0 - 1)) * xpb;
-    L.yorg = ((z0 * p.H + y0) * p.W + x0) * ypb;
-    L.xdst = lds + buf * G::XB + wave * 1024;
-    auto inside = [](int o, int size, int hn) {
-      const int lo = o >= 1 ? 0 : 1 - o, hi = size - o + 1 < hn ? size - o + 1 : hn;
-      return hi > lo ? ((1u << hi) - 1u) & ~((1u << lo) - 1u) : 0u;
-    };
-    L.zm = inside(z0, p.D, G::HZ); L.ym = inside(y0, p.H, G::HY); L.xm = inside(x0, p.W, G::HX);
-    L.inter = (L.zm == (1u << G::HZ) - 1 && L.ym == (1u << G::HY) - 1 && L.xm == (1u << G::HX) - 1) ? 1u : 0u;
-    return L;
-  };
-  auto issue_x = [&](const TileLoads& L, auto i_) {
-    constexpr int i = i_;
-    const int c = xcode[i];
-    const unsigned ok = (unsigned)(c >> 14) & (L.inter | ((L.zm >> (c & 7)) & (L.ym >> ((c >> 3) & 7)) & (L.xm >> ((c >> 6) & 31)))) & 1u;
-    lds_dma16_async(L.xrs, L.xdst + i * 8192, (L.xorg + xoffs[i]) | ((int)ok - 1));
-  };
-  auto issue_y = [&](const TileLoads& L, auto i_) {
-    constexpr int i = i_;
-    const int P = tid + 512 * i;
-    const int vox = P / G::YPPV, part = P % G::YPPV;
-    const int z = vox >> 6, y = (vox >> 4) & 3, x = vox & 15;
-    const int yo = ((z * p.H + y) * p.W + x) * ypb + part * 16;
-    const unsigned ok = (L.inter | ((L.zm >> (z + 1)) & (L.ym >> (y + 1)) & (L.xm >> (x + 1)))) & 1u;
-    ry[i] = __builtin_bit_cast(u32x4, __builtin_amdgcn_raw_buffer_load_b128(L.yrs, (L.yorg + yo) | ((int)ok - 1), 0, 0));
-  };
-
-  const int tile_first = lane8 * tpx + gsub;
-  const int qq = v >> 2, pp = v & 3;
-  const int ybase = (4 * q + qq) * G::SY + pp * 8;
-  const int xbase = (4 * q + qq) * G::SX + pp * 8;
-  int cur = 0;
-#ifdef BRATS_WGRAD_STAMPS
-  long long tacc[5] = {0, 0, 0, 0, 0}, tlast = __builtin_amdgcn_s_memtime();
-#define WG_STAMP(i) do { const long long t_ = __builtin_amdgcn_s_memtime(); tacc[i] += t_ - tlast; tlast = t_; } while (0)
-#else
-#define WG_STAMP(i) do { } while (0)
-#endif
-  if (tile_first < tile_end) {
-    const TileLoads L = setup_loads(tile_first, 0);
-    static_for<0, G::XI>([&](auto i_) { issue_x(L, i_); });
-    static_for<0, G::YI>([&](auto i_) { issue_y(L, i_); });
-  }
-  for (int tile = tile_first; tile < tile_end; tile += g8, cur ^= 1) {
-    WG_STAMP(4);
-    asm volatile("s_waitcnt vmcnt(0)" ::: "memory");
-    WG_STAMP(0);
-    __syncthreads();
-    WG_STAMP(1);
-#pragma unroll
-    for (int i = 0; i < G::YI; ++i) *(u32x4*)(ldy + (tid + 512 * i) * 16) = ry[i];
-    __syncthreads();
-    WG_STAMP(2);
-    const bool more = tile + g8 < tile_end;
-    TileLoads L = setup_loads(more ? tile + g8 : tile, cur ^ 1);
-    if (!more) L.zm = L.inter = 0;
-    __builtin_amdgcn_sched_barrier(0);
-    WG_STAMP(3);
-    const char* ldx = lds + cur * G::XB;
-    constexpr int PD = 3;
-    bf16x8 a[2][COF], b[PD + 1];
-    auto read_a = [&](auto s_) {
-      constexpr int s = s_;
-      const int yoff = ybase + (32 * s) * G::SY;
-#pragma unroll
-      for (int m = 0; m < COF; ++m) a[s & 1][m] = tr_pair(ldy + yoff + m * 32, ldy + yoff + 16 * G::SY + m * 32);
-    };
-    auto read_b = [&](auto u_) {
-      constexpr int u = u_;
-      constexpr int s = u / G::PPW, jj = u % G::PPW;
-      const int xoff = xbase + (((s >> 1) * G::HY + 2 * (s & 1)) * G::HX) * G::SX + poff[jj];
-      b[u % (PD + 1)] = tr_pair(ldx + xoff, ldx + xoff + G::HX * G::SX);
-    };
-    constexpr int NU = 8 * G::PPW;
-    static_for<0, G::XI>([&](auto i_) { issue_x(L, i_); });
-    static_for<0, G::YI>([&](auto i_) { issue_y(L, i_); });
-    __builtin_amdgcn_sched_barrier(0);
-    read_a(std::integral_constant<int, 0>{});
-    static_for<0, PD>([&](auto u_) { read_b(u_); });
-    static_for<0, NU>([&](auto u_) {
-      constexpr int u = u_;
-      constexpr int s = u / G::PPW, jj = u % G::PPW;
-      if constexpr (u + PD < NU) read_b(std::integral_constant<int, u + PD>{});
-      if constexpr (jj == 0 && s + 1 < 8) read_a(std::integral_constant<int, s + 1>{});
-      __builtin_amdgcn_sched_barrier(0);
-#pragma unroll
-      for (int m = 0; m < COF; ++m)
-        acc[jj][m] = MFMA16_16x16x32(a[s & 1][m], b[u % (PD + 1)], acc[jj][m]);
-      __builtin_amdgcn_sched_barrier(0);
-    });
-  }
-
-#ifdef BRATS_WGRAD_STAMPS
-  WG_STAMP(4);
-  if (lane == 0 && blockIdx.y == 0 && blockIdx.z == 0) {
-    long long* st = (long long*)(p.ws + (size_t)gridDim.x * 27 * p.cout * p.cin) + ((size_t)blockIdx.x * 8 + wave) * 5;
-    for (int i = 0; i < 5; ++i) st[i] = tacc[i];
-  }
-#endif
-#pragma unroll
-  for (int jj = 0; jj < G::PPW; ++jj) {
-    const int pid = wave + 8 * jj;
-    if (pid < G::PAIRS) {
-      const int t = pid / CIF, nn = pid % CIF;
-      float* base = p.ws + ((size_t)split * 27 + t) * p.cout * p.cin;
-      const int ci = ci0 + nn * 16 + v;
-      if (CIF > 1 || ci < p.cin) {
-#pragma unroll
-        for (int m = 0; m < COF; ++m)
-#pragma unroll
-          for (int r = 0; r < 4; ++r) base[(size_t)(co0 + m * 16 + 4 * q + r) * p.cin + ci] = acc[jj][m][r];
-      }
-    }
-  }
+  constexpr bool GNB = COF < 0;
+  const WgradGnFold f{};
+#include "conv_wgrad_alltaps2_body.inc"
+}
+constexpr int WG_GNB_TAB = 5 * 48 * (int)sizeof(float);
+template <int COF, int CIF>
+__global__ __launch_bounds__(512, 1) void conv_wgrad_alltaps2_gnb_kernel(const WgradParams p, const WgradGnFold f) {
+  constexpr bool GNB = COF > 0;
+#include "conv_wgrad_alltaps2_body.inc"
 }
 
 template <int DIL> struct Wg3n {
@@ -1225,6 +1078,20 @@
   }
   return g_wgrad_noslab_mode >= 0 ? g_wgrad_noslab_mode : env_mode;
 }
+int g_wgrad_gn_bwd_mode = -1;
+extern "C" int BRATS_API(brats_conv3d_set_wgrad_gn_bwd)(int mode) {
+  const int old = g_wgrad_gn_bwd_mode;
+  g_wgrad_gn_bwd_mode = mode < 0 ? -1 : (mode ? 1 : 0);
+  return old;
+}
+static int wgrad_gn_bwd_mode() {
+  static int env_mode = -1;
+  if (env_mode < 0) {
+    const char* e = getenv("BRATS_WGRAD_GN_BWD");
+    env_mode = e ? (atoi(e) ? 1 : 0) : 1;
+  }
+  return g_wgrad_gn_bwd_mode >= 0 ? g_wgrad_gn_bwd_mode : env_mode;
+}
 static bool wgrad_noslab_built(int dtype, bool shifted, int ksize, int dil, const WgradArgs& a) {
   return !shifted && ksize == 3 && dtype == BRATS_BF16 && (dil == 1 || dil == 2) && a.cout > 0 && a.cout % 48 == 0 && a.c1 > 0 &&
          a.c1 % 16 == 0 && a.c2 % 16 == 0 && a.N > 0 && a.D > 0 && a.H > 0 && a.W > 0;
@@ -1510,6 +1377,46 @@
                                   int D, int H, int W, int cout, brats_stream_t s) {
   return wgrad_impl(false, WgradArgs{x1, c1, pitch1, x2, c2, pitch2, dy, dypitch, N, D, H, W, cout}, nullptr, ws, dw, dbias, dtype, ksize, dil, s);
 }
+static bool wgrad_gn_bwd_rule(int dtype, const WgradArgs& a, int dzpitch, int ypitch, int groups, int act) {
+  if (!wgrad_gn_bwd_mode() || dtype != BRATS_BF16 || (act != BRATS_ACT_RELU && act != BRATS_ACT_LEAKY)) return false;
+  if (a.c1 <= 0 || a.c2 != 0 || a.cout <= 0 || a.N <= 0 || a.D <= 0 || a.H <= 0 || a.W <= 0 || groups <= 0 || a.cout % groups) return false;
+  if (a.p1 % 8 || dzpitch % 8 || ypitch % 8 || a.c1 % 8 || a.cout % 8 || a.p1 < a.c1 || dzpitch < a.cout || ypitch < a.cout) return false;
+  WgradArgs b = a;
+  b.dyp = dzpitch > ypitch ? dzpitch : ypitch;
+  if (wgrad_sample_overflow(b, 2)) return false;
+  return wgrad_plan(dtype, false, 3, 1, a, true).form == WG_ALLTAPS2_31;
+}
+extern "C" int BRATS_API(brats_conv3d_wgrad_gn_bwd_taken)(int dtype, int N, int D, int H, int W, int c1, int xpitch, int cout, int dzpitch,
+                                               int ypitch, int groups, int act) {
+  return wgrad_gn_bwd_rule(dtype, WgradArgs{nullptr, c1, xpitch, nullptr, 0, 0, nullptr, 0, N, D, H, W, cout}, dzpitch, ypitch, groups, act) ? 1 : 0;
+}
+extern "C" int BRATS_API(brats_conv3d_wgrad_gn_bwd_tiles)(const void* x, int c1, int xpitch, const float* tile_stats, int tiles_per_sample,
+                                               const void* dz, int dzpitch, const void* y, int ypitch, const float* scale_shift,
+                                               const float* mean_rstd, const float* gamma, float* red, float* dgamma, float* dbeta,
+                                               float* ws, float* dw, int dtype, int act, float slope, int groups, int N, int D, int H,
+                                               int W, int cout, brats_stream_t s) {
+  if (!x || !tile_stats || !dz || !y || !scale_shift || !mean_rstd || !gamma || !red || !dgamma || !dbeta || !ws || !dw || tiles_per_sample <= 0)
+    BRATS_FAIL(BRATS_E_ARG, "wgrad_gn_bwd_tiles: null pointer");
+  const WgradArgs a{x, c1, xpitch, nullptr, 0, 0, nullptr, 0, N, D, H, W, cout};
+  if (!wgrad_gn_bwd_rule(dtype, a, dzpitch, ypitch, groups, act))
+    BRATS_FAIL(BRATS_E_UNSUPPORTED, "wgrad_gn_bwd_tiles: not a problem of the fused form (ask brats_conv3d_wgrad_gn_bwd_taken first)");
+  hipStream_t st = (hipStream_t)s;
+  const WgradPlan pl = wgrad_plan(dtype, false, 3, 1, a, true);
+  const size_t room = wgrad_slab_room(dtype, false, 3, a);
+  if (pl.slab_bytes() > room) BRATS_FAIL(BRATS_E_ARG, "wgrad_gn_bwd_tiles: the plan's %zu bytes of slabs exceed the workspace size %zu", pl.slab_bytes(), room);
+  gn_bwd_tiles_sums_launch(tile_stats, tiles_per_sample, mean_rstd, red, N, cout, groups, st);
+  const WgradParams p = wgrad_params(a, ws, pl.tiles, pl.nlane, pl.nsplit, pl.ntaps, 1);
+  const WgradGnFold f{dz, y, dzpitch, ypitch, scale_shift, mean_rstd, gamma, red, dgamma, dbeta, act, groups, slope};
+  constexpr int LDS = Wg3b<3, 1>::LDS + WG_GNB_TAB;
+  static std::atomic<uint64_t> attr_done{0};
+  BRATS_ENSURE_LDS_ATTR((conv_wgrad_alltaps2_gnb_kernel<3, 1>), LDS, attr_done);
+  hipLaunchKernelGGL((conv_wgrad_alltaps2_gnb_kernel<3, 1>), dim3(pl.groups * pl.nsplit, pl.cot, pl.cit), dim3(512), LDS, st, p, f);
+  BRATS_CHECK_LAUNCH();
+  wgrad_reduce_launch((const float*)ws, dw, pl.nsplit, cout, c1, pl.ntaps, st);
+  BRATS_CHECK_LAUNCH();
+  return 0;
+}
+
 extern "C" int BRATS_API(brats_conv3d_x3_wgrad)(const void* x1, int c1, int pitch1, const void* x2, int c2, int pitch2, const void* dy,
                                      int dypitch, const float* amax_dy, float* ws, float* dw, float* dbias, int dtype, int dil,
                                      int N, int D, int H, int W, int cout, brats_stream_t s) {
diff --git a/brats21_amd/csrc/conv_wgrad_alltaps2_body.inc b/brats21_amd/csrc/conv_wgrad_alltaps2_body.inc
--- /dev/null
+++ b/brats21_amd/csrc/conv_wgrad_alltaps2_body.inc
@@ -0,0 +1,251 @@
+  typedef bf16_t T;
+  using G = Wg3b<COF, CIF>;
+  static_assert(!GNB || G::YPPV == 6, "the fused piece deal is written for 48-channel dY rows");
+  constexpr int YI = GNB ? G::YI + 1 : G::YI;
+  extern __shared__ __attribute__((aligned(16))) char lds[];
+  char* ldy = lds + 2 * G::XB;
+  const int tid = threadIdx.x, lane = tid & 63;
+  const int wave = __builtin_amdgcn_readfirstlane(tid >> 6);
+  const int q = lane >> 4, v = lane & 15;
+  const int lane8 = blockIdx.x % p.nlane, gsub = blockIdx.x / p.nlane, g8 = gridDim.x / p.nlane;
+  const int split = blockIdx.x;
+  const int tpx = (p.ntiles + p.nlane - 1) / p.nlane;
+  const int tile_end = min(p.ntiles, (lane8 + 1) * tpx);
+  const int co0 = blockIdx.y * G::CO, ci0 = blockIdx.z * G::CI;
+  const T* xsrc;
+  int xpitch;
+  if (ci0 < p.c1) { xsrc = (const T*)p.x1 + ci0; xpitch = p.p1; }
+  else { xsrc = (const T*)p.x2 + (ci0 - p.c1); xpitch = p.p2; }
+  const int xpb = xpitch * 2, ypb = p.dyp * 2;
+
+  int xoffs[G::XI], xcode[G::XI];
+#pragma unroll
+  for (int i = 0; i < G::XI; ++i) {
+    const int P = tid + 512 * i;
+    const int vox = P / G::XPPV, part = P % G::XPPV;
+    const int hx = vox % G::HX, hy = (vox / G::HX) % G::HY, hz = vox / (G::HX * G::HY);
+    const bool ok = P < G::XPIECES && (CIF > 1 || part * 8 < p.c1);
+    xoffs[i] = ok ? ((hz * p.H + hy) * p.W + hx) * xpb + part * 16 : (int)0x80000000;
+    xcode[i] = ok ? (hz | hy << 3 | hx << 6 | 1 << 14) : 0;
+  }
+  const unsigned xsample_bytes = (unsigned)p.D * p.H * p.W * xpitch * 2;
+  const unsigned ysample_bytes = (unsigned)p.D * p.H * p.W * p.dyp * 2;
+
+  int poff[G::PPW];
+#pragma unroll
+  for (int jj = 0; jj < G::PPW; ++jj) {
+    const int pid = wave + 8 * jj;
+    const int t = pid / CIF, nn = pid % CIF;
+    poff[jj] = pid < G::PAIRS ? (((t / 9) * G::HY + (t / 3) % 3) * G::HX + t % 3) * G::SX + nn * 32 : 0;
+  }
+  f32x4 acc[G::PPW][COF];
+#pragma unroll
+  for (int jj = 0; jj < G::PPW; ++jj)
+#pragma unroll
+    for (int m = 0; m < COF; ++m) acc[jj][m] = f32x4{0.f, 0.f, 0.f, 0.f};
+
+  u32x4 ry[YI];
+  WgGnbState<GNB> gs;
+  if constexpr (GNB) {
+    if (blockIdx.x == 0 && blockIdx.y == 0 && blockIdx.z == 0 && f.dgamma) {
+      for (int c = tid; c < p.cout; c += 512) GN_BWD_PARAM_SUMS(f.red, p.N, p.cout, c, f.dbeta[c], f.dgamma[c])
+    }
+  }
+  struct TileLoads {
+    rsrc4_t xrs;
+    __amdgpu_buffer_rsrc_t yrs;
+    int xorg, yorg;
+    unsigned zm, ym, xm, inter;
+    char* xdst;
+    WgGnbLoads<GNB> g;
+  };
+  auto setup_loads = [&](int tile, int buf) {
+    TileLoads L;
+    int bt = tile;
+    const int x0 = (bt % p.tx) * WG_TX; bt /= p.tx;
+    const int y0 = (bt % p.ty) * WG_TY; bt /= p.ty;
+    const int z0 = (bt % p.tz) * WG_TZ;
+    const int n = bt / p.tz;
+    const size_t sample_vox = (size_t)n * p.D * p.H * p.W;
+    L.xrs = make_rsrc4(xsrc + sample_vox * xpitch, xsample_bytes);
+    if constexpr (!GNB)
+      L.yrs = __builtin_amdgcn_make_buffer_rsrc((void*)((const T*)p.dy + sample_vox * p.dyp + co0), (short)0, (int)ysample_bytes, 0x00020000);
+    L.xorg = (((z0 - 1) * p.H + (y0 - 1)) * p.W + (x0 - 1)) * xpb;
+    if constexpr (!GNB) L.yorg = ((z0 * p.H + y0) * p.W + x0) * ypb;
+    if constexpr (GNB) {
+      const unsigned vox = (unsigned)p.D * p.H * p.W;
+      L.yrs = __builtin_amdgcn_make_buffer_rsrc((void*)((const T*)f.y + sample_vox * f.yp + co0), (short)0, (int)(vox * f.yp * 2), 0x00020000);
+      L.g.zrs = __builtin_amdgcn_make_buffer_rsrc((void*)((const T*)f.dz + sample_vox * f.dzp + co0), (short)0, (int)(vox * f.dzp * 2), 0x00020000);
+      L.yorg = ((z0 * p.H + y0) * p.W + x0) * f.yp * 2;
+      L.g.zorg = ((z0 * p.H + y0) * p.W + x0) * f.dzp * 2;
+      L.g.n = n;
+    }
+    L.xdst = lds + buf * G::XB + wave * 1024;
+    auto inside = [](int o, int size, int hn) {
+      const int lo = o >= 1 ? 0 : 1 - o, hi = size - o + 1 < hn ? size - o + 1 : hn;
+      return hi > lo ? ((1u << hi) - 1u) & ~((1u << lo) - 1u) : 0u;
+    };
+    L.zm = inside(z0, p.D, G::HZ); L.ym = inside(y0, p.H, G::HY); L.xm = inside(x0, p.W, G::HX);
+    L.inter = (L.zm == (1u << G::HZ) - 1 && L.ym == (1u << G::HY) - 1 && L.xm == (1u << G::HX) - 1) ? 1u : 0u;
+    return L;
+  };
+  auto issue_x = [&](const TileLoads& L, auto i_) {
+    constexpr int i = i_;
+    const int c = xcode[i];
+    const unsigned ok = (unsigned)(c >> 14) & (L.inter | ((L.zm >> (c & 7)) & (L.ym >> ((c >> 3) & 7)) & (L.xm >> ((c >> 6) & 31)))) & 1u;
+    lds_dma16_async(L.xrs, L.xdst + i * 8192, (L.xorg + xoffs[i]) | ((int)ok - 1));
+  };
+  auto issue_y = [&](const TileLoads& L, auto i_) {
+    constexpr int i = i_;
+    if constexpr (GNB) {
+      if (i < G::YI || tid < G::YPPV) {
+        const int P = wg_gnb_piece(tid, i);
+        const int vox = P / G::YPPV, part = P % G::YPPV;
+        const int z = vox >> 6, y = (vox >> 4) & 3, x = vox & 15;
+        const int vo = (z * p.H + y) * p.W + x;
+        const unsigned ok = wg_gnb_mine(tid, i) ? (L.inter | ((L.zm >> (z + 1)) & (L.ym >> (y + 1)) & (L.xm >> (x + 1)))) & 1u : 0u;
+        gs.rz[i] = __builtin_bit_cast(u32x4, __builtin_amdgcn_raw_buffer_load_b128(L.g.zrs, (L.g.zorg + vo * f.dzp * 2 + part * 16) | ((int)ok - 1), 0, 0));
+        ry[i] = __builtin_bit_cast(u32x4, __builtin_amdgcn_raw_buffer_load_b128(L.yrs, (L.yorg + vo * f.yp * 2 + part * 16) | ((int)ok - 1), 0, 0));
+        gs.yokm = (gs.yokm & ~(1u << i)) | ok << i;
+      }
+      return;
+    }
+    const int P = tid + 512 * i;
+    const int vox = P / G::YPPV, part = P % G::YPPV;
+    const int z = vox >> 6, y = (vox >> 4) & 3, x = vox & 15;
+    const int yo = ((z * p.H + y) * p.W + x) * ypb + part * 16;
+    const unsigned ok = (L.inter | ((L.zm >> (z + 1)) & (L.ym >> (y + 1)) & (L.xm >> (x + 1)))) & 1u;
+    ry[i] = __builtin_bit_cast(u32x4, __builtin_amdgcn_raw_buffer_load_b128(L.yrs, (L.yorg + yo) | ((int)ok - 1), 0, 0));
+  };
+
+  const int tile_first = lane8 * tpx + gsub;
+  const int qq = v >> 2, pp = v & 3;
+  const int ybase = (4 * q + qq) * G::SY + pp * 8;
+  const int xbase = (4 * q + qq) * G::SX + pp * 8;
+  int cur = 0;
+#ifdef BRATS_WGRAD_STAMPS
+  long long tacc[5] = {0, 0, 0, 0, 0}, tlast = __builtin_amdgcn_s_memtime();
+#define WG_STAMP(i) do { const long long t_ = __builtin_amdgcn_s_memtime(); tacc[i] += t_ - tlast; tlast = t_; } while (0)
+#else
+#define WG_STAMP(i) do { } while (0)
+#endif
+  if (tile_first < tile_end) {
+    const TileLoads L = setup_loads(tile_first, 0);
+    static_for<0, G::XI>([&](auto i_) { issue_x(L, i_); });
+    static_for<0, YI>([&](auto i_) { issue_y(L, i_); });
+    if constexpr (GNB) gs.n_pend = L.g.n;
+  }
+  for (int tile = tile_first; tile < tile_end; tile += g8, cur ^= 1) {
+    WG_STAMP(4);
+    if constexpr (GNB) {
+      if (gs.n_pend != gs.n_coef) {
+        float* gtab = (float*)(lds + G::LDS);
+        if (tid < G::CO && co0 + tid < p.cout) {
+          const int n = gs.n_pend, C = p.cout, c = co0 + tid, cpg = C / f.groups, g = c / cpg;
+          const float invM = GN_BWD_INV_COUNT(cpg, p.D * p.H * p.W);
+          const float mean = f.mean_rstd[(n * f.groups + g) * 2], rstd = f.mean_rstd[(n * f.groups + g) * 2 + 1];
+          float m1, m2, ca, cb, ck;
+          GN_BWD_GROUP_MEANS(f.gamma, f.red, n, C, cpg, g, invM, m1, m2)
+          GN_BWD_COEFS(mean, rstd, f.gamma[c], m1, m2, ca, cb, ck)
+          gtab[tid] = f.scale_shift[((size_t)n * C + c) * 2];
+          gtab[G::CO + tid] = f.scale_shift[((size_t)n * C + c) * 2 + 1];
+          gtab[2 * G::CO + tid] = ca;
+          gtab[3 * G::CO + tid] = cb;
+          gtab[4 * G::CO + tid] = ck;
+        }
+        __syncthreads();
+        gtab += (tid % G::YPPV) * 8;
+#pragma unroll
+        for (int j = 0; j < 8; ++j) {
+          gs.sc[j] = gtab[j]; gs.sh[j] = gtab[G::CO + j];
+          gs.ca[j] = gtab[2 * G::CO + j]; gs.cb[j] = gtab[3 * G::CO + j]; gs.ck[j] = gtab[4 * G::CO + j];
+        }
+        gs.n_coef = gs.n_pend;
+      }
+      static_for<0, YI>([&](auto i_) {
+        constexpr int i = i_;
+        if (wg_gnb_mine(tid, i)) {
+          const u32x4 o = gn_bwd_apply_raw8(gs.rz[i], ry[i], gs.sc, gs.sh, gs.ca, gs.cb, gs.ck, f.act, f.slope);
+          const uint32_t keep = 0u - ((gs.yokm >> i) & 1u);
+          ry[i] = u32x4{o[0] & keep, o[1] & keep, o[2] & keep, o[3] & keep};
+        }
+      });
+      __builtin_amdgcn_sched_barrier(0);
+    }
+    asm volatile("s_waitcnt vmcnt(0)" ::: "memory");
+    WG_STAMP(0);
+    __syncthreads();
+    WG_STAMP(1);
+    if constexpr (GNB) {
+      static_for<0, YI>([&](auto i_) {
+        constexpr int i = i_;
+        if (wg_gnb_mine(tid, i)) *(u32x4*)(ldy + wg_gnb_piece(tid, i) * 16) = ry[i];
+      });
+    } else {
+#pragma unroll
+    for (int i = 0; i < G::YI; ++i) *(u32x4*)(ldy + (tid + 512 * i) * 16) = ry[i];
+    }
+    __syncthreads();
+    WG_STAMP(2);
+    const bool more = tile + g8 < tile_end;
+    TileLoads L = setup_loads(more ? tile + g8 : tile, cur ^ 1);
+    if (!more) L.zm = L.inter = 0;
+    __builtin_amdgcn_sched_barrier(0);
+    WG_STAMP(3);
+    const char* ldx = lds + cur * G::XB;
+    constexpr int PD = 3;
+    bf16x8 a[2][COF], b[PD + 1];
+    auto read_a = [&](auto s_) {
+      constexpr int s = s_;
+      const int yoff = ybase + (32 * s) * G::SY;
+#pragma unroll
+      for (int m = 0; m < COF; ++m) a[s & 1][m] = tr_pair(ldy + yoff + m * 32, ldy + yoff + 16 * G::SY + m * 32);
+    };
+    auto read_b = [&](auto u_) {
+      constexpr int u = u_;
+      constexpr int s = u / G::PPW, jj = u % G::PPW;
+      const int xoff = xbase + (((s >> 1) * G::HY + 2 * (s & 1)) * G::HX) * G::SX + poff[jj];
+      b[u % (PD + 1)] = tr_pair(ldx + xoff, ldx + xoff + G::HX * G::SX);
+    };
+    constexpr int NU = 8 * G::PPW;
+    static_for<0, G::XI>([&](auto i_) { issue_x(L, i_); });
+    static_for<0, YI>([&](auto i_) { issue_y(L, i_); });
+    if constexpr (GNB) gs.n_pend = L.g.n;
+    __builtin_amdgcn_sched_barrier(0);
+    read_a(std::integral_constant<int, 0>{});
+    static_for<0, PD>([&](auto u_) { read_b(u_); });
+    static_for<0, NU>([&](auto u_) {
+      constexpr int u = u_;
+      constexpr int s = u / G::PPW, jj = u % G::PPW;
+      if constexpr (u + PD < NU) read_b(std::integral_constant<int, u + PD>{});
+      if constexpr (jj == 0 && s + 1 < 8) read_a(std::integral_constant<int, s + 1>{});
+      __builtin_amdgcn_sched_barrier(0);
+#pragma unroll
+      for (int m = 0; m < COF; ++m)
+        acc[jj][m] = MFMA16_16x16x32(a[s & 1][m], b[u % (PD + 1)], acc[jj][m]);
+      __builtin_amdgcn_sched_barrier(0);
+    });
+  }
+
+#ifdef BRATS_WGRAD_STAMPS
+  WG_STAMP(4);
+  if (lane == 0 && blockIdx.y == 0 && blockIdx.z == 0) {
+    long long* st = (long long*)(p.ws + (size_t)gridDim.x * 27 * p.cout * p.cin) + ((size_t)blockIdx.x * 8 + wave) * 5;
+    for (int i = 0; i < 5; ++i) st[i] = tacc[i];
+  }
+#endif
+#pragma unroll
+  for (int jj = 0; jj < G::PPW; ++jj) {
+    const int pid = wave + 8 * jj;
+    if (pid < G::PAIRS) {
+      const int t = pid / CIF, nn = pid % CIF;
+      float* base = p.ws + ((size_t)split * 27 + t) * p.cout * p.cin;
+      const int ci = ci0 + nn * 16 + v;
+      if (CIF > 1 || ci < p.cin) {
+#pragma unroll
+        for (int m = 0; m < COF; ++m)
+#pragma unroll
+          for (int r = 0; r < 4; ++r) base[(size_t)(co0 + m * 16 + 4 * q + r) * p.cin + ci] = acc[jj][m][r];
+      }
+    }
+  }
diff --git a/brats21_amd/csrc/gen_twin_dispatch.py b/brats21_amd/csrc/gen_twin_dispatch.py
--- a/brats21_amd/csrc/gen_twin_dispatch.py
+++ b/brats21_amd/csrc/gen_twin_dispatch.py
@@ -3,7 +3,7 @@
 import sys
 
 BOTH = {"brats_conv3d_set_vs8", "brats_conv3d_set_kp", "brats_conv3d_set_wgrad_alltaps", "brats_conv3d_set_wgrad_noslab",
-        "brats_conv3d_set_x3_wgrad_fused", "brats_upsample_bwd_set_fused"}
+        "brats_conv3d_set_x3_wgrad_fused", "brats_upsample_bwd_set_fused", "brats_conv3d_set_wgrad_gn_bwd"}
 DATA = {"brats_conv3d_f8_fwd", "brats_conv3d_wgrad_f8", "brats_conv3d_pack_weights_multi"}
 
 txt = re.sub(r"/\*.*?\*/", " ", open(sys.argv[1]).read(), flags=re.S)
diff --git a/brats21_amd/csrc/gn_bwd_apply.hpp b/brats21_amd/csrc/gn_bwd_apply.hpp
--- /dev/null
+++ b/brats21_amd/csrc/gn_bwd_apply.hpp
@@ -0,0 +1,58 @@
+#pragma once
+#include "common.hpp"
+#include "act.hpp"
+
+
+#define GN_BWD_INV_COUNT(cpg, voxels) (1.f / ((float)(cpg) * (float)(voxels)))
+
+#define GN_BWD_GROUP_MEANS(gamma, red, n, C, cpg, g, invM, m1, m2)       \
+  {                                                                      \
+    float t1_ = 0.f, t2_ = 0.f;                                          \
+    for (int j_ = 0; j_ < (cpg); ++j_) {                                 \
+      const int c_ = (g) * (cpg) + j_;                                   \
+      t1_ += (gamma)[c_] * (red)[((size_t)(n) * (C) + c_) * 2];          \
+      t2_ += (gamma)[c_] * (red)[((size_t)(n) * (C) + c_) * 2 + 1];      \
+    }                                                                    \
+    (m1) = t1_ * (invM);                                                 \
+    (m2) = t2_ * (invM);                                                 \
+  }
+
+#define GN_BWD_PARAM_SUMS(red, N, C, c, dbeta_c, dgamma_c)               \
+  {                                                                      \
+    float b_ = 0.f, g_ = 0.f;                                            \
+    for (int m_ = 0; m_ < (N); ++m_) { b_ += (red)[((size_t)m_ * (C) + (c)) * 2]; g_ += (red)[((size_t)m_ * (C) + (c)) * 2 + 1]; } \
+    (dbeta_c) = b_;                                                      \
+    (dgamma_c) = g_;                                                     \
+  }
+
+#define GN_BWD_COEFS(mean, rstd, gamma_c, m1, m2, ca, cb, ck)            \
+  {                                                                      \
+    (ca) = (rstd) * (gamma_c);                                           \
+    (cb) = -(rstd) * (rstd) * (m2);                                      \
+    (ck) = (rstd) * ((mean) * (rstd) * (m2) - (m1));                     \
+  }
+
+#define GN_BWD_APPLY_ELEM(HEAVY, g, y, sc, sh, ca, cb, ck, act, slope, o)                  \
+  {                                                                                        \
+    const float u_ = (g) * act_grad<HEAVY>((y) * (sc) + (sh), act, slope);                 \
+    (o) = u_ * (ca) + ((y) * (cb) + (ck));                                                 \
+  }
+
+DEVI u32x4 gn_bwd_apply_raw8(u32x4 dz, u32x4 y, const float (&sc)[8], const float (&sh)[8], const float (&ca)[8],
+                             const float (&cb)[8], const float (&ck)[8], int act, float slope) {
+  float g[8], yy[8], o[8];
+#pragma unroll
+  for (int i = 0; i < 4; ++i) {
+    unpack2(dz[i], g[2 * i], g[2 * i + 1]);
+    unpack2(y[i], yy[2 * i], yy[2 * i + 1]);
+  }
+#pragma unroll
+  for (int j = 0; j < 8; ++j) GN_BWD_APPLY_ELEM(false, g[j], yy[j], sc[j], sh[j], ca[j], cb[j], ck[j], act, slope, o[j])
+  u32x4 v;
+#pragma unroll
+  for (int i = 0; i < 4; ++i) v[i] = pack2(o[2 * i], o[2 * i + 1]);
+  return v;
+}
+
+void gn_bwd_tiles_sums_launch(const float* tile_stats, int tiles_per_sample, const float* mean_rstd, float* red, int N, int C,
+                              int groups, hipStream_t st);
diff --git a/brats21_amd/csrc/norm.hip b/brats21_amd/csrc/norm.hip
--- a/brats21_amd/csrc/norm.hip
+++ b/brats21_amd/csrc/norm.hip
@@ -2,6 +2,7 @@
 #include "common.hpp"
 
 #include "act.hpp"
+#include "gn_bwd_apply.hpp"
 #include "se.hpp"
 
 constexpr int GN_MAX_SPLITS = 64;
@@ -901,24 +902,10 @@
   float* m12 = sm;
   const int n = blockIdx.y;
   const int cpg = C / groups;
-  const float invM = 1.f / ((float)cpg * (float)voxels);
-  for (int g = threadIdx.x; g < groups; g += blockDim.x) {
-    float t1 = 0.f, t2 = 0.f;
-    for (int j = 0; j < cpg; ++j) {
-      const int c = g * cpg + j;
-      t1 += gamma[c] * red[((size_t)n * C + c) * 2];
-      t2 += gamma[c] * red[((size_t)n * C + c) * 2 + 1];
-    }
-    m12[g * 2] = t1 * invM;
-    m12[g * 2 + 1] = t2 * invM;
-  }
+  const float invM = GN_BWD_INV_COUNT(cpg, voxels);
+  for (int g = threadIdx.x; g < groups; g += blockDim.x) GN_BWD_GROUP_MEANS(gamma, red, n, C, cpg, g, invM, m12[g * 2], m12[g * 2 + 1])
   if (blockIdx.x == 0 && blockIdx.y == 0 && dgamma) {
-    for (int c = threadIdx.x; c < C; c += blockDim.x) {
-      float b = 0.f, g = 0.f;
-      for (int m = 0; m < N; ++m) { b += red[((size_t)m * C + c) * 2]; g += red[((size_t)m * C + c) * 2 + 1]; }
-      dbeta[c] = b;
-      dgamma[c] = g;
-    }
+    for (int c = threadIdx.x; c < C; c += blockDim.x) GN_BWD_PARAM_SUMS(red, N, C, c, dbeta[c], dgamma[c])
   }
   __syncthreads();
   const int cv = C / VW;
@@ -934,9 +921,7 @@
     sh[j] = scale_shift[((size_t)n * C + c) * 2 + 1];
     const float mean = mean_rstd[(n * groups + g) * 2], rstd = mean_rstd[(n * groups + g) * 2 + 1];
     const float m1 = m12[g * 2], m2 = m12[g * 2 + 1];
-    ca[j] = rstd * gamma[c];
-    cb[j] = -rstd * rstd * m2;
-    ck[j] = rstd * (mean * rstd * m2 - m1);
+    GN_BWD_COEFS(mean, rstd, gamma[c], m1, m2, ca[j], cb[j], ck[j])
   }
   const T* dzb = dz + (size_t)n * voxels * dzpitch + c0;
   const T* yb = y + (size_t)n * voxels * ypitch + c0;
@@ -946,10 +931,7 @@
   float mx = 0.f;
   auto body = [&](const float* g, const float* yy, float* o) {
 #pragma unroll
-    for (int j = 0; j < VW; ++j) {
-      const float u = g[j] * act_grad<HEAVY>(yy[j] * sc[j] + sh[j], act, slope);
-      o[j] = u * ca[j] + (yy[j] * cb[j] + ck[j]);
-    }
+    for (int j = 0; j < VW; ++j) GN_BWD_APPLY_ELEM(HEAVY, g[j], yy[j], sc[j], sh[j], ca[j], cb[j], ck[j], act, slope, o[j])
     if (amax) {
 #pragma unroll
       for (int j = 0; j < VW; j += 2) mx = __builtin_fmaxf(__builtin_fmaxf(mx, __builtin_fabsf(o[j])), __builtin_fabsf(o[j + 1]));
@@ -1122,6 +1104,14 @@
   red[(size_t)i * 2 + 1] = (float)(rstd * (s2 - mean * s1));
 }
 
+void gn_bwd_tiles_sums_launch(const float* tile_stats, int tiles_per_sample, const float* mean_rstd, float* red, int N, int C,
+                              int groups, hipStream_t st) {
+  double* part = (double*)(red + (((size_t)N * C * 2 + 1) / 2) * 2);
+  const int splits = gn_splits(tiles_per_sample);
+  hipLaunchKernelGGL(gn_chan_reduce_kernel, dim3((C + 15) / 16, N, splits), dim3(256), 0, st, tile_stats, tiles_per_sample, C, part);
+  hipLaunchKernelGGL(gn_bwd_tiles_finish_kernel, dim3((N * C + 255) / 256), dim3(256), 0, st, part, splits, N, C, groups, mean_rstd, red);
+}
+
 extern "C" int BRATS_API(brats_gn_act_bwd_tiles)(const float* tile_stats, int tiles_per_sample, const void* dz, int dzpitch, const void* y,
                                       int ypitch, const float* scale_shift, const float* mean_rstd, const float* gamma, void* dy,
                                       int dypitch, float* red, float* dgamma, float* dbeta, int dtype, int act, float slope,
@@ -1134,10 +1124,7 @@
   if (C % vw || C % groups || dzpitch % vw || ypitch % vw || dypitch % vw || C / vw > 256)
     BRATS_FAIL(BRATS_E_ARG, "gn_act_bwd_tiles: C=%d / pitches must be multiples of %d", C, vw);
   hipStream_t st = (hipStream_t)s;
-  double* part = (double*)(red + (((size_t)N * C * 2 + 1) / 2) * 2);
-  const int splits = gn_splits(tiles_per_sample);
-  hipLaunchKernelGGL(gn_chan_reduce_kernel, dim3((C + 15) / 16, N, splits), dim3(256), 0, st, tile_stats, tiles_per_sample, C, part);
-  hipLaunchKernelGGL(gn_bwd_tiles_finish_kernel, dim3((N * C + 255) / 256), dim3(256), 0, st, part, splits, N, C, groups, mean_rstd, red);
+  gn_bwd_tiles_sums_launch(tile_stats, tiles_per_sample, mean_rstd, red, N, C, groups, st);
   const bool big = big_tensor(dtype, (size_t)N * voxels * C);
   dim3 g2(voxel_walk(vw, voxels, C).grid(big ? 8192 : 2048), N);
   const size_t lds2 = (size_t)2 * groups * sizeof(float);
diff --git a/brats21_amd/networks/_program.py b/brats21_amd/networks/_program.py
--- a/brats21_amd/networks/_program.py
+++ b/brats21_amd/networks/_program.py
@@ -37,6 +37,7 @@
         self.fold_head_bwd = os.environ.get("BRATS_FOLD_HEAD", "1") != "0"
         self.fold_pool_bwd = os.environ.get("BRATS_FOLD_POOL", "1") != "0"
         self.fold_bwd_stats = os.environ.get("BRATS_FOLD_BWD_STATS", "1") != "0"
+        self.fold_first_bwd = os.environ.get("BRATS_FOLD_FIRST_BWD", "1") != "0"
         self.fold_head_fwd = os.environ.get("BRATS_FOLD_HEAD_FWD", os.environ.get("BRATS_FOLD_HEAD", "1")) != "0"
 
     def _init_dropout(self, p):
diff --git a/brats21_amd/networks/equiunet.py b/brats21_amd/networks/equiunet.py
--- a/brats21_amd/networks/equiunet.py
+++ b/brats21_amd/networks/equiunet.py
@@ -269,7 +269,14 @@
     kact, slope_t = _unit_act(unit, cx.act)
     if slope_t is not None:
         cx.put(unit.prelu.weight, ops.prelu_slope_grad(dz, y, scale_shift))
-    if unit.batch_norm:
+    fused = None
+    if (tiles is not None and not need_dx and cx.m.fold_first_bwd and x2 is None and head is None and pool is None and not unit.bcn
+            and not unit.batch_norm and unit.conv.bias is None and slope_t is None and not all8 and not x3s and cx.drop is None):
+        fused = ops.conv3d_wgrad_gn_bwd_tiles(x, tiles, dz, y, scale_shift, mean_rstd, gamma_c, unit.groups, kact,
+                                              out=cx.dest(unit.conv.weight))
+    if fused is not None:
+        dw, dgamma, dbeta = fused
+    elif unit.batch_norm:
         if mean_rstd is None:
             raise NotImplementedError("--norm batch: backward through an eval-mode forward (running statistics) is not implemented")
         n_, d_, h_, w_, c_ = y.shape
@@ -294,7 +301,9 @@
         dy, dgamma, dbeta = ops.gn_act_bwd(dz, y, scale_shift, mean_rstd, gamma_c, unit.groups, kact, amax=amax,
                                            slope_t=slope_t)
     wdst = cx.dest(unit.conv.weight)
-    if w8 and amax is not None:
+    if fused is not None:
+        pass
+    elif w8 and amax is not None:
         dw = ops.conv3d_wgrad_f8(x, dy, ax, amax, x2=x2, amax2=ax2, out=wdst)
     elif x2 is not None and x.shape[-1] % 16:
         dw, db = ops.conv3d_wgrad(torch.cat([x, x2], -1), dy, 3, unit.dilation, amax_dy=amax if x3s else None, want_dbias=unit.bcn)
diff --git a/brats21_amd/ops.py b/brats21_amd/ops.py
--- a/brats21_amd/ops.py
+++ b/brats21_amd/ops.py
@@ -1739,3 +1739,4 @@
 
 
 from ._attgate import AttGateSaved, attgate_bwd, attgate_fwd
+from ._first_bwd import conv3d_wgrad_gn_bwd_tiles
diff --git a/include/brats_hip.h b/include/brats_hip.h
--- a/include/brats_hip.h
+++ b/include/brats_hip.h
@@ -81,6 +81,13 @@
 int brats_conv3d_set_wgrad_alltaps(int mode);
 int brats_conv3d_set_wgrad_noslab(int mode);
 int brats_conv3d_wgrad_noslab_taken(int dtype, int dil, int N, int D, int H, int W, int c1, int c2, int cout);
+int brats_conv3d_set_wgrad_gn_bwd(int mode);
+int brats_conv3d_wgrad_gn_bwd_taken(int dtype, int N, int D, int H, int W, int c1, int xpitch, int cout, int dzpitch, int ypitch,
+                                    int groups, int act);
+int brats_conv3d_wgrad_gn_bwd_tiles(const void* x, int c1, int xpitch, const float* tile_stats, int tiles_per_sample, const void* dz,
+                                    int dzpitch, const void* y, int ypitch, const float* scale_shift, const float* mean_rstd,
+                                    const float* gamma, float* red, float* dgamma, float* dbeta, float* ws, float* dw, int dtype,
+                                    int act, float slope, int groups, int N, int D, int H, int W, int cout, brats_stream_t s);
 int brats_conv3d_set_x3_wgrad_fused(int mode);
 int brats_conv3d_wgrad(const void* x1, int c1, int pitch1, const void* x2, int c2, int pitch2,
                        const void* dy, int dypitch, float* ws, float* dw, float* dbias,
```
